# Zoe187419/ATE_replication_causalML

Measured on AMD Instinct MI355X. Metric: rows/sec for DML-ATE cross-fit, N=1e7 p=500, 1/2/4/8 MI355X; ATE/SE parity, higher is better.
Workload: dtype bf16; 1 GPU; model=DML-PLR 5-fold cross-fit, CV-LASSO nuisances (100 lambdas, inner 4-fold CV), global_batch=10000000, seq_len=500, N=10000000, p=500, folds=5, parallelism=dp1, dgp=tutorial, n_kept=10000000, layout=blocked64+bytes8

## Files before the change

ate_replication_causalml_amd/_native.py:

```python
from __future__ import annotations

import ctypes
import os
from pathlib import Path

_LIBDIR = Path(__file__).resolve().parent / "_lib"
_hip = None
_cpu = None


class NativeMissing(RuntimeError):
    pass


class NativeError(RuntimeError):

    def __init__(self, name: str, status: int, detail: str):
        self.entry, self.status = name, status
        super().__init__(f"{name} failed with status {status}: {detail}")


HIP_ERRORS = {
    1: "hipErrorInvalidValue", 2: "hipErrorOutOfMemory", 3: "hipErrorNotInitialized",
    4: "hipErrorDeinitialized", 9: "hipErrorInvalidConfiguration",
    13: "hipErrorInvalidSymbol", 17: "hipErrorInvalidDevicePointer",
    21: "hipErrorInvalidMemcpyDirection", 35: "hipErrorInsufficientDriver",
    52: "hipErrorMissingConfiguration", 53: "hipErrorPriorLaunchFailure",
    98: "hipErrorInvalidDeviceFunction", 100: "hipErrorNoDevice", 101: "hipErrorInvalidDevice",
    200: "hipErrorInvalidImage", 201: "hipErrorInvalidContext", 209: "hipErrorNoBinaryForGpu",
    218: "hipErrorInvalidKernelFile", 400: "hipErrorInvalidHandle", 500: "hipErrorNotFound",
    600: "hipErrorNotReady", 700: "hipErrorIllegalAddress", 701: "hipErrorLaunchOutOfResources",
    702: "hipErrorLaunchTimeOut", 710: "hipErrorAssert", 719: "hipErrorLaunchFailure",
    720: "hipErrorCooperativeLaunchTooLarge", 801: "hipErrorNotSupported",
    900: "hipErrorStreamCaptureUnsupported", 901: "hipErrorStreamCaptureInvalidated",
    907: "hipErrorCapturedEvent", 999: "hipErrorUnknown",
}


def describe_status(rc: int) -> str:
    if rc < 0:
        return "rejected by the entry point's own argument check (no kernel launched)"
    return f"{HIP_ERRORS.get(rc, 'hipError?')} ({rc})"


c_void_p = ctypes.c_void_p
c_int = ctypes.c_int
c_int64 = ctypes.c_int64
c_uint64 = ctypes.c_uint64
c_double = ctypes.c_double

_SIGS = {
    "ate_gram_bf16": "pliipipipipppp",
    "ate_gram_bf16_pair": "pllipippipippippiip",
    "ate_gram_bf16_tri": "pllippipippipp",
    "ate_gram_pair_bal": "",
    "ate_last_error": "pi",
    "ate_last_stale_error": "pi",
    "ate_clear_errors": "",
    "ate_debug_bad_launch": "ip",
    "ate_check_kernel_resources": "pi",
    "ate_gram_f32": "plippipipippppp",
    "ate_gram_f64": "plippipipippppp",
    "ate_gram_tile_sizes": "pppp",
    "ate_chol_solve": "pipiipdpppppp",
    "ate_chol_solve_k": "pipipidppppp",
    "ate_spd_solve_batched": "ppiippp",
    "ate_predict": "ipllppiidipp",
    "ate_irls_update": "ipllppiiiiippppipp",
    "ate_irls_check": "piidippp",
    "ate_naive": "ippplpppp",
    "ate_clip_propensity": "pplpp",
    "ate_aipw": "ppppppldpppp",
    "ate_dml_moments": "ppplppp",
    "ate_dml_finalize": "pipp",
    "ate_boot_multinomial": "ppluiipp",
    "ate_boot_poisson": "ppluiilipp",
    "ate_enet_isa_selftest": "pp",
    "ate_enet_prepare": "piipipiipipipppppppp",
    "ate_enet_path": "pipiippppidddipppppippp",
    "ate_enet_coef": "ppiiiipppppppp",
    "ate_enet_cvloss_gauss": "pippiipppiiipp",
    "ate_cv_select": "pppiipippppip",
    "ate_enet_pick": "ppiiipppip",
    "ate_dml_resid_moments": "ipllpipipiiiiiippp",
    "ate_dml_resid_exact": "pllpipipiiiiiiippp",
    "ate_irm_score_moments": "ipllpipiipiiiiidippp",
    "ate_irm_score_moments_multi": "ipllpipiipipiiiiiidippp",
    "ate_irm_score_multi_smax": "",
    "ate_irm_scores": "ipllpipiipiiiiidipp",
    "ate_irm_sens_moments": "ipllpipiipiiiiidippp",
    "ate_irm_target_moments": "ipllpipiipiiiiidippp",
    "ate_iivm_moments": "ipllpipiipiiiiiiidippp",
    "ate_group_boot": "pppliiuippp",
    "ate_group_boot_scratch": "iii",
    "ate_cate_moments": "ppplpiiippp",
    "ate_cate_moments_scratch": "iii",
    "ate_cate_boot": "ppplppiiiuippp",
    "ate_cate_boot_scratch": "iiii",
    "ate_policy_pair_hist": "ppppppliiipp",
    "ate_policy_pair_hist_scratch": "i",
    "ate_policy_search": "ppiilppp",
    "ate_lognet_path": "iplpiipipipdddippippppppppp",
    "ate_lognet_cvloss": "iplpiippipppipp",
    "ate_dgp_fill": "iplllllp" + "uiipppp",
    "ate_sel_block_rows": "",
    "ate_sel_gen_count": "upilllpp",
    "ate_sel_gen_flags": "upillpp",
    "ate_sel_gen_mark": "upiplllpiplp",
    "ate_forest_fit": "pppppi" + "pppppppp" + "ip",
    "ate_forest_predict": "ppiiipppppippip",
    "ate_forest_pack": "pippppppp",
    "ate_forest_scratch_bytes": "ii",
    "ate_forest_exact_scratch_bytes": "iiii",
    "ate_forest_fit_exact": "piiipppippppippppppppp",
    "ate_forest_predict16": "ppiiipppppppippip",
    "ate_bin_matrix": "plipppp",
    "ate_panel_xtv": "iplpipplipp",
    "ate_select_compact": "plppddpppp" + "p",
    "ate_gbdt_run": "ppp",
    "ate_lv_boot": "ppp",
    "ate_lv_classify": "pipiippp",
    "ate_lv_decide": "ppipipipippppp" + "iipip",
    "ate_lv_partition": "ppipippppipp",
    "ate_lv_scatter": "pppppippp",
    "ate_lv_children": "pippppp",
    "ate_lv_transpose": "piipip",
    "ate_gbdt_bin_panel": "pilpipppilpppl" + "p",
    "ate_gbdt_slab_entries": "liii",
    "ate_gbdt_slab2_entries": "li",
    "ate_gbdt_pair_root": "pppplllp",
    "ate_gbdt_apply": "plliipppp" + "p",
    "ate_panel_xv": "iplpipiplpp",
    "ate_col_moments": "pllipppp",
    "ate_standardize": "pllippp",
    "ate_interactions": "pllipl" + "p",
    "ate_scan_parts": "l",
    "ate_gbdt_limits": "p",
    "ate_excl_scan_i32": "plpppp",
    "ate_excl_scan_i64": "plpppp",
}
_RESTYPE = {"ate_forest_scratch_bytes": ctypes.c_int64,
            "ate_forest_exact_scratch_bytes": ctypes.c_int64, "ate_gbdt_slab_entries": ctypes.c_int64,
            "ate_gbdt_slab2_entries": ctypes.c_int64,
            "ate_scan_parts": ctypes.c_int64, "ate_group_boot_scratch": ctypes.c_int64,
            "ate_cate_moments_scratch": ctypes.c_int64,
            "ate_cate_boot_scratch": ctypes.c_int64,
            "ate_policy_pair_hist_scratch": ctypes.c_int64}
_CT = {"p": c_void_p, "i": c_int, "l": c_int64, "u": c_uint64, "d": c_double}


def _load(path: Path, sigs: dict):
    lib = ctypes.CDLL(str(path), mode=ctypes.RTLD_GLOBAL)
    for name, sig in sigs.items():
        if hasattr(lib, name):
            f = getattr(lib, name)
            f.restype = _RESTYPE.get(name, c_int)
            f.argtypes = [_CT[ch] for ch in sig]
    return lib


def hip_available() -> bool:
    return (_LIBDIR / "libatehip.so").exists()


def hip_library_path() -> Path:
    debug = os.environ.get("ATE_DEBUG", "0") not in ("", "0")
    return Path(os.environ["ATE_HIP_LIB"]) if os.environ.get("ATE_HIP_LIB") else \
        _LIBDIR / ("libatehip_debug.so" if debug else "libatehip.so")


def hip():
    global _hip
    if _hip is None:
        import torch
        debug = os.environ.get("ATE_DEBUG", "0") not in ("", "0")
        p = hip_library_path()
        if not p.exists():
            raise NativeMissing(
                f"{p} not found: build it with `python -m ate_replication_causalml_amd._build` "
                "(hipcc --offload-arch=gfx950). GPU ops have no fallback.")
        _hip = _load(p, _SIGS)
        if debug:
            _check_kernel_resources(_hip)
    return _hip


_resource_report = None


def _check_kernel_resources(lib):
    global _resource_report
    buf = ctypes.create_string_buffer(1 << 14)
    bad = lib.ate_check_kernel_resources(buf, len(buf))
    _resource_report = buf.value.decode(errors="replace")
    if bad > 0:
        raise NativeError("ate_check_kernel_resources", bad,
                          "kernels that cannot launch as registered:\n" + "\n".join(
                              l for l in _resource_report.splitlines() if "FAIL" in l))


def kernel_resource_report() -> str | None:
    return _resource_report


def _native_message(lib, fn: str) -> tuple[int, str]:
    buf = ctypes.create_string_buffer(512)
    code = getattr(lib, fn)(buf, len(buf))
    return code, buf.value.decode(errors="replace")


def cpu():
    global _cpu
    if _cpu is None:
        p = _LIBDIR / "libatecpu.so"
        if not p.exists():
            from ._build import build_cpu
            build_cpu()
        _cpu = _load(p, {})
    return _cpu


def check(rc: int, name: str = "native call"):
    if rc != 0:
        raise RuntimeError(f"{name} failed with code {rc}")


def call(name: str, *args):
    lib = hip()
    rc = getattr(lib, name)(*args)
    if rc != 0:
        raise NativeError(name, rc, status_detail(lib, rc))
    return rc


def status_detail(lib, rc: int) -> str:
    detail = describe_status(rc)
    if rc > 0 and hasattr(lib, "ate_last_error"):
        code, msg = _native_message(lib, "ate_last_error")
        if code == rc and msg:
            detail = msg
        scode, smsg = _native_message(lib, "ate_last_stale_error")
        if scode and smsg:
            detail += f" [stale, cleared before the launch: {smsg}]"
        lib.ate_clear_errors()
    return detail


def loaded_libraries():
    out = []
    try:
        with open(f"/proc/{os.getpid()}/maps") as f:
            for line in f:
                if str(_LIBDIR) in line:
                    out.append(line.split()[-1])
    except OSError:
        pass
    return sorted(set(out))
```

ate_replication_causalml_amd/estimators/lasso.py:

```python
from __future__ import annotations

import numpy as np
import torch

from .. import _native
from ..ops import stats as S
from ..ops.devconst import const
from ..ops.enet import cv_enet_gaussian
from ..ops.gram import gram
from ..ops.linalg import chol_solve, chol_solve_active
from ..ops.panel import build_panel, dtype_code
from ..parallel import rng
from ..reference.estimators import lambda_interp
from ..result import AteResult
from ..utils.graphs import estimator_graphs
from .common import as_np, read_result, resolve_device


def _fold_ids(n, K, seed, stream, dist):
    return dist.fold_ids(K, seed, stream) if dist is not None else rng.fold_ids(n, K, seed, stream)


def _sharded_gram(pan, dist):
    G = gram(pan)
    if dist is None:
        return G, None
    dist.sum_(G)
    return G, global_seg_counts(pan, dist.comm)


def _lasso_w_panel(Y, W, X, seed, nfolds, fold_stream, device, dtype, dist=None):
    dev = resolve_device(device)
    Xn = np.column_stack([as_np(X), as_np(W)])
    fid = _fold_ids(Xn.shape[0], nfolds, seed, fold_stream, dist)
    return build_panel(Xn, None, as_np(Y), folds=fid, dtype=dtype, device=dev)


def _lasso_w_cv(pan, pf_w, G, counts=None):
    pf = np.r_[np.ones(len(pan.xcols) - 1), pf_w]
    return cv_enet_gaussian(G, pan, pan.xcols, [pan.cols["Y"]], penalty_factor=pf,
                            seg_counts=counts)


def _lasso_w_body(pan, pf_w, dist=None, counts=None):
    G = gram(pan)
    if dist is not None:
        dist.sum_(G)
    cv = _lasso_w_cv(pan, pf_w, G, None if counts is None else np.asarray(counts))
    lam = cv.lambdas[0].gather(0, cv.sel[0, 1:2].long())
    fnp = cv.fold_npass.min().double().reshape(1) if cv.fold_npass is not None else \
        torch.zeros(1, dtype=torch.float64, device=lam.device)
    return torch.cat([cv.coef_1se[0, -1:].double(), lam.double(), fnp])


def _lasso_w(Y, W, X, pf_w, seed, nfolds, fold_stream, method, device, dtype, dist, graph):
    pan = _lasso_w_panel(Y, W, X, seed, nfolds, fold_stream, device, dtype, dist)
    if graph and (dist is None or dist.capturable) and pan.data.is_cuda:
        counts = None if dist is None else tuple(global_seg_counts(pan, dist.comm).tolist())
        out, g = estimator_graphs.run("lasso_w", _lasso_w_body, (pan,), float(pf_w), dist,
                                      counts)
        v = out.cpu().numpy()
        if v[2] < 0:
            from ..utils.guards import NumericalError
            raise NumericalError("CV fold path timed out waiting for its full-data lambda "
                                 "sequence; selection is invalid")
        return AteResult.make(method, float(v[0]), None, lambda_1se=float(v[1]), hipgraph=g)
    G, counts = _sharded_gram(pan, dist)
    cv = _lasso_w_cv(pan, pf_w, G, counts).check()
    return AteResult.make(method, float(cv.coef_1se[0, -1]), None,
                          lambda_1se=float(cv.lambdas[0, int(cv.sel[0, 1])]))


def lasso_single(Y, W, X, seed=1991, nfolds=10, fold_stream=5, method="Single-equation LASSO",
                 device=None, dtype="f64", dist=None, graph=True):
    return _lasso_w(Y, W, X, 0.0, seed, nfolds, fold_stream, method, device, dtype, dist, graph)


def lasso_usual(Y, W, X, seed=1991, nfolds=10, fold_stream=6, method="Usual LASSO", device=None,
                dtype="f64", dist=None, graph=True):
    return _lasso_w(Y, W, X, 1.0, seed, nfolds, fold_stream, method, device, dtype, dist, graph)


def interaction_expand(x: torch.Tensor) -> torch.Tensor:
    from ..ops.prep import interactions
    return interactions(x)


def _interp_at(lams: torch.Tensor, nlam: torch.Tensor, path: torch.Tensor, s: torch.Tensor):
    L = lams.numel()
    k = nlam.long().clamp(min=1)
    ar = torch.arange(L, device=lams.device)
    valid = ar < k
    lam0 = lams[0]
    lamk = lams.gather(0, (k - 1).reshape(1))[0]
    den = lam0 - lamk
    single = den == 0
    dsafe = torch.where(single, torch.ones_like(den), den)
    sfrac = ((lam0 - s) / dsafe).clamp(0.0, 1.0)
    ln = torch.where(valid, (lam0 - lams) / dsafe, torch.full_like(lams, 2.0))
    left = ((ln <= sfrac) & valid).sum().clamp(min=1) - 1
    ln_l = ln.gather(0, left.reshape(1))[0]
    exact = (ln_l == sfrac) | single | (left + 1 >= k)
    right = torch.where(exact, left, left + 1)
    ln_r = ln.gather(0, right.reshape(1))[0]
    gap = ln_l - ln_r
    frac = torch.where(exact | (gap.abs() < np.finfo(float).eps), torch.ones_like(sfrac),
                       (sfrac - ln_r) / torch.where(gap == 0, torch.ones_like(gap), gap))
    return (path.index_select(0, left.reshape(1))[0] * frac
            + path.index_select(0, right.reshape(1))[0] * (1 - frac))


def _belloni_body(panw, pany, panpost, compat):
    cws = cv_enet_gaussian(gram(panw), panw, panw.xcols, [panw.cols["Y"]])
    cys = cv_enet_gaussian(gram(pany), pany, pany.xcols, [pany.cols["Y"]])
    q = len(panw.xcols)
    s = cws.lambdas[0].gather(0, cws.sel[0, 0:1].long())[0]
    bw = _interp_at(cws.lambdas[0], cws.nlam[0], cws.coef_path[0].double(), s)[1:]
    if compat == "reference":
        by = _interp_at(cys.lambdas[0], cys.nlam[0], cys.coef_path[0].double(), s)[1:]
        pos = (bw > 0) | (by > 0)
        keep = torch.cat([pos[1:], torch.zeros(1, dtype=torch.bool, device=pos.device)])
    else:
        sy = cys.lambdas[0].gather(0, cys.sel[0, 0:1].long())[0]
        by = _interp_at(cys.lambdas[0], cys.nlam[0], cys.coef_path[0].double(), sy)[1:]
        keep = (bw != 0) | (by != 0)
    G = gram(panpost)[0]
    dev = G.device
    xc = const(panpost.xcols[:q], torch.int32, dev)
    ki = keep.long()
    nsel = ki.sum()
    pos = torch.where(keep, ki.cumsum(0), 1 + nsel + (1 - ki).cumsum(0))
    wpos = (1 + nsel).reshape(1)
    dest = torch.cat([const([0], torch.int64, dev), pos, wpos])
    src = torch.cat([const([panpost.cols["one"]], torch.int32, dev), xc,
                     const([panpost.xcols[q]], torch.int32, dev)])
    cols = torch.empty(q + 2, dtype=torch.int32, device=dev).index_copy(0, dest, src)
    kact = (2 + nsel).to(torch.int32)
    r = chol_solve_active(G, cols, kact, panpost.cols["Y"])
    b_w = r.beta.gather(0, wpos)[0]
    se = torch.sqrt(r.aux[1] / (panpost.n - r.aux[0]) * r.invdiag.gather(0, wpos)[0])
    fnp = torch.stack([cws.fold_npass.min(), cys.fold_npass.min()]).min().double() \
        if cws.fold_npass is not None else torch.zeros((), dtype=torch.float64, device=dev)
    return torch.stack([b_w.double(), se.double(), nsel.double(), r.aux[0].double(), fnp])


def belloni(Y, W, X, seed=1991, nfolds=10, compat="reference", method="Belloni et.al",
            device=None, dtype="f64", dist=None, graph=True):
    dev = resolve_device(device)
    Yn, Wn = as_np(Y), as_np(W)
    xint = interaction_expand(torch.as_tensor(as_np(X), device=dev))
    n, q = xint.shape
    if graph and dist is None and dev.type == "cuda":
        panw = build_panel(xint, None, Wn, folds=_fold_ids(n, nfolds, seed, 8, None), dtype=dtype,
                           device=dev)
        pany = build_panel(xint, None, Yn, folds=_fold_ids(n, nfolds, seed, 9, None), dtype=dtype,
                           device=dev)
        post = torch.cat([xint, torch.as_tensor(Wn, dtype=torch.float64, device=dev)[:, None]], 1)
        panpost = build_panel(post, None, Yn, dtype=dtype, device=dev)
        out, g = estimator_graphs.run("belloni", _belloni_body, (panw, pany, panpost), compat)
        v = out.cpu().numpy()
        if v[4] < 0:
            from ..utils.guards import NumericalError
            raise NumericalError("CV fold path timed out waiting for its full-data lambda "
                                 "sequence; selection is invalid")
        return AteResult.make(method, float(v[0]), float(v[1]), n_selected=int(round(v[2])),
                              rank=int(round(v[3])), hipgraph=g)
    fits = []
    for target, stream in ((Wn, 8), (Yn, 9)):
        fid = _fold_ids(n, nfolds, seed, stream, dist)
        pan = build_panel(xint, None, target, folds=fid, dtype=dtype, device=dev)
        G, counts = _sharded_gram(pan, dist)
        fits.append((pan, G, cv_enet_gaussian(G, pan, pan.xcols, [pan.cols["Y"]],
                                              seg_counts=counts).check()))
    (_, _, cw), (_, _, cy) = fits
    s = float(cw.lambdas[0, int(cw.sel[0, 0])])
    lw = cw.lambdas[0, :int(cw.nlam[0])].cpu().numpy()
    ly = cy.lambdas[0, :int(cy.nlam[0])].cpu().numpy()
    pw = cw.coef_path[0, :len(lw)].cpu().numpy()
    py = cy.coef_path[0, :len(ly)].cpu().numpy()

    def coef_at(lams, path, s_):
        l, r, f = lambda_interp(lams, s_)
        return path[l] * f + path[r] * (1 - f)

    bw = coef_at(lw, pw, s)[1:]
    by = coef_at(ly, py, s if compat == "reference" else float(cy.lambdas[0, int(cy.sel[0, 0])]))[1:]
    if compat == "reference":
        union = []
        for v in np.concatenate([np.flatnonzero(bw > 0) + 1, np.flatnonzero(by > 0) + 1]):
            if int(v) not in union:
                union.append(int(v))
        cols = [v - 2 for v in union if v - 1 >= 1]
    else:
        cols = sorted(set(np.flatnonzero(bw != 0)) | set(np.flatnonzero(by != 0)))
    sel_x = torch.cat([xint[:, torch.as_tensor(cols, dtype=torch.long, device=xint.device)],
                       torch.as_tensor(Wn, dtype=torch.float64, device=xint.device)[:, None]], 1)
    pan = build_panel(sel_x, None, Yn, dtype=dtype, device=dev)
    G = gram(pan)[0]
    if dist is not None:
        dist.sum_(G)
    dcols = [pan.cols["one"], *pan.xcols]
    r = chol_solve(G, dcols, pan.cols["Y"])
    n_all = dist.n_total if dist is not None else pan.n
    se = torch.sqrt(r.aux[1] / (n_all - r.aux[0]) * r.invdiag[-1])
    return read_result(torch.stack([r.beta[-1], se]), method, n_selected=len(cols),
                       rank=int(r.aux[0]))


def global_seg_counts(pan, comm):
    c = torch.as_tensor(np.asarray(pan.seg_nreal, dtype=np.float64))
    if comm is not None and comm.world_size > 1:
        dev = pan.device
        t = c.to(dev)
        comm.all_reduce_(t)
        c = t.cpu()
    return c.numpy()


EXACT_BLOCK = 16384


def dml_residual_terms(pan, coef: torch.Tensor, rows: int = 1 << 20) -> torch.Tensor:
    K = coef.shape[0]
    Xc = pan.colmajor()
    dev = Xc.device
    bf = pan.dtype == torch.bfloat16
    xc = torch.as_tensor(pan.xcols, dtype=torch.long, device=dev)
    out = []
    for k in range(K):
        r0, r1 = (int(v) for v in pan.seg_bounds[k])
        for a in range(r0, r1, rows):
            b = min(r1, a + rows)
            blk = Xc[:, a:b]
            valid = (blk[pan.cols["one"]] != 0).double()
            xs = blk.index_select(0, xc).double()
            y = blk[pan.cols["Y_hi"]].double() + blk[pan.cols["Y_lo"]].double() if bf else \
                blk[pan.cols["Y"]].double()
            w = blk[pan.cols["W_hi"]].double() + blk[pan.cols["W_lo"]].double() if bf else \
                blk[pan.cols["W"]].double()
            yr = y - (coef[k, 0, 0] + coef[k, 0, 1:].double() @ xs)
            wr = w - (coef[k, 1, 0] + coef[k, 1, 1:].double() @ xs)
            yr, wr = yr * valid, wr * valid
            w2 = wr * wr
            out.append(torch.stack([wr * yr, w2, yr * yr * w2, yr * w2 * wr, w2 * w2,
                                    valid, yr * yr], 1))
    return torch.cat(out)


_TRI: dict = {}


def _tri_index(P: int, device):
    key = (P, str(device))
    t = _TRI.get(key)
    if t is None:
        i, j = np.triu_indices(P)
        t = (torch.as_tensor(i * P + j, dtype=torch.int64).to(device),
             torch.as_tensor(j * P + i, dtype=torch.int64).to(device))
        _TRI[key] = t
    return t


def allreduce_sym_(comm, t: torch.Tensor) -> torch.Tensor:
    P = t.shape[-1]
    up, lo = _tri_index(P, t.device)
    v = t.view(-1, P * P)
    buf = v.index_select(1, up)
    comm.all_reduce_(buf)
    v.index_copy_(1, up, buf)
    v.index_copy_(1, lo, buf)
    return t


def dml_phases(pan, folds: int, lambda_rule="min", comm=None, seg_counts=None, G=None,
               shard_paths=True, exact=False):
    from ..utils.graphs import Collective
    dist = comm is not None and comm.world_size > 1
    if dist and seg_counts is None:
        seg_counts = global_seg_counts(pan, comm)
    K = folds
    full_sets = [[s for s in range(K) if s != k] for k in range(K)]
    ycols = [pan.cols["Y"], pan.cols["W"]]
    sharded = dist and shard_paths
    mine = [k for k in range(K) if k % comm.world_size == comm.rank] if sharded else list(range(K))
    p1 = len(pan.xcols) + 1

    n_rows = int(np.asarray(seg_counts if seg_counts is not None else pan.seg_nreal).sum())
    if exact:
        from ..ops.gram import check_exact_range
        check_exact_range(pan, n_rows, comm=comm if dist else None)

    def phase_gram(_):
        if exact:
            return {"GX": gram(pan, stage="tiles", exact=True, n_total=n_rows, checked=True)}
        return {"G": gram(pan, stage="tiles") if G is None else G}

    def phase_gram_reduce(st):
        if exact:
            return {"GX": gram(pan, stage="reduce", exact=True)}
        return st if G is not None else {"G": gram(pan, stage="reduce", out=st["G"])}

    def phase_from_limbs(st):
        from ..ops.exact import from_limbs
        return {**st, "G": from_limbs(st["GX"])}

    native_exact = pan.data.is_cuda and pan.dtype == torch.bfloat16

    def phase_terms(st):
        from ..ops.exact import column_amax
        if native_exact:
            part = _exact_resid(pan, st["coef"], 1, None)
            return {**st, "amax": part.view(-1, 7).amax(0)}
        terms = dml_residual_terms(pan, st["coef"])
        return {**st, "terms": terms, "amax": column_amax(terms)}

    def phase_limbs(st):
        from ..ops.exact import _scale_exp, sum_limbs
        if native_exact:
            sh = _scale_exp(st["amax"], n_rows).contiguous()
            part = _exact_resid(pan, st["coef"], 2, sh).view(torch.int64).view(-1, 14).sum(0)
            return {**st, "limbs": torch.stack([part[:7], part[7:]])}
        return {**st, "limbs": sum_limbs(st["terms"], st["amax"], n_rows)}

    def phase_mom_exact(st):
        from ..ops.exact import finish_limbs
        return {**st, "mom": finish_limbs(st["limbs"], st["amax"], n_rows)}

    def fit(st):
        if not mine:
            return None
        cv = cv_enet_gaussian(st["G"], pan, pan.xcols, ycols,
                              full_sets=[full_sets[k] for k in mine], seg_counts=seg_counts)
        return cv

    def pick(cv):
        return (cv.coef_min if lambda_rule == "min" else cv.coef_1se).reshape(
            len(mine), 2, -1).contiguous()

    def phase_fit(st):
        cv = fit(st)
        coef = pick(cv)
        return {**st, "cv": cv, "mom": dml_residual_moments(pan, coef)}

    def phase_fit_sharded(st):
        cv = fit(st)
        coef = torch.zeros((K, 2, p1), dtype=torch.float64, device=pan.device)
        if cv is not None:
            coef.index_copy_(0, const(mine, torch.int64, pan.device), pick(cv).double())
        return {**st, "cv": cv, "coef": coef}

    def phase_resid(st):
        return {**st, "mom": dml_residual_moments(pan, st["coef"])}

    def phase_final(st):
        return {**st, "res": S.dml_finalize(st["mom"], "plr")}

    cap = bool(getattr(comm, "capturable", False))

    def reduce(name, op="sum"):
        def f(st):
            (comm.all_reduce_ if op == "sum" else comm.all_reduce_max_)(st[name])
            return st
        return Collective(f, capturable=cap)

    def reduce_sym(name):
        _tri_index(pan.P, pan.device)

        def f(st):
            allreduce_sym_(comm, st[name])
            return st
        return Collective(f, capturable=cap)

    if exact:
        phases = [phase_gram, phase_gram_reduce]
        if dist:
            phases.append(reduce("GX"))
        phases.append(phase_from_limbs)
        if sharded:
            phases += [phase_fit_sharded, reduce("coef")]
        else:
            def phase_fit_coef(st):
                cv = fit(st)
                return {**st, "cv": cv, "coef": pick(cv).double()}
            phases.append(phase_fit_coef)
        phases.append(phase_terms)
        if dist:
            phases.append(reduce("amax", "max"))
        phases.append(phase_limbs)
        if dist:
            phases.append(reduce("limbs"))
        phases += [phase_mom_exact, phase_final]
        return phases
    phases = [phase_gram, phase_gram_reduce]
    if dist:
        phases.append(reduce_sym("G"))
    if sharded:
        phases += [phase_fit_sharded, reduce("coef"), phase_resid]
    else:
        phases.append(phase_fit)
    if dist:
        phases.append(reduce("mom"))
    phases.append(phase_final)
    return phases


def dml_crossfit_panel(pan, folds: int, lambda_rule="min", G=None, comm=None, seg_counts=None,
                       exact=False):
    st = None
    for ph in dml_phases(pan, folds, lambda_rule, comm, seg_counts, G, exact=exact):
        st = ph(st)
    return st["res"], st["mom"], st.get("cv")


def micro_fold_map(K: int, s: int) -> np.ndarray:
    a, b = np.divmod(np.arange(K * K), K)
    return (a + s * b) % K


def median_aggregate(theta: torch.Tensor, se: torch.Tensor, how: str = "median"):
    def med(v):
        v = torch.sort(v).values
        n = v.shape[0]
        return v[n // 2] if n % 2 else 0.5 * (v[n // 2 - 1] + v[n // 2])
    if how == "mean":
        t = theta.mean()
        return torch.stack([t, torch.sqrt((se * se + (theta - t) ** 2).mean())])
    t = med(theta)
    return torch.stack([t, torch.sqrt(med(se * se + (theta - t) ** 2))])


def dml_repeated_phases(pan, folds: int, repeats: int, lambda_rule="min", comm=None,
                        seg_counts=None, aggregate="median"):
    from ..utils.graphs import Collective
    K, Sn = folds, repeats
    if pan.nseg != K * K:
        raise ValueError(f"repeated cross-fitting needs K*K = {K * K} micro-segments, the panel "
                         f"has {pan.nseg}")
    if not 1 <= Sn <= K:
        raise ValueError(f"repeats must be in 1..{K} (distinct partitions of K*K micro-segments)")
    dist = comm is not None and comm.world_size > 1
    if seg_counts is None:
        seg_counts = global_seg_counts(pan, comm) if dist else np.asarray(pan.seg_nreal)
    counts = np.asarray(seg_counts, dtype=np.float64)
    dev = pan.device
    maps = [micro_fold_map(K, s) for s in range(Sn)]
    M = [const(np.eye(K)[m].T.copy(), torch.float64, dev) for m in maps]
    fold_counts = [np.bincount(m, weights=counts, minlength=K) for m in maps]
    mi = [const(m, torch.int64, dev) for m in maps]
    full_sets = [[j for j in range(K) if j != k] for k in range(K)]
    ycols = [pan.cols["Y"], pan.cols["W"]]
    P = pan.P
    cap = bool(getattr(comm, "capturable", False))

    def phase_gram(_):
        return {"G": gram(pan, stage="tiles")}

    def phase_gram_reduce(st):
        return {"G": gram(pan, stage="reduce", out=st["G"])}

    Mall = torch.cat(M)
    sets_all = [[s * K + j for j in fs] for s in range(Sn) for fs in full_sets]
    counts_all = np.concatenate(fold_counts)

    def phase_paths(st):
        Gs = (Mall @ st["G"].view(K * K, P * P)).view(Sn * K, P, P)
        cv = cv_enet_gaussian(Gs, pan, pan.xcols, ycols, full_sets=sets_all,
                              seg_counts=counts_all)
        coef = (cv.coef_min if lambda_rule == "min" else cv.coef_1se).reshape(Sn, K, 2, -1)
        return {**st, "coef": coef}

    def phase_split(s):
        def f(st):
            coef_m = st["coef"][s].double().index_select(0, mi[s]).contiguous()
            return {**st, f"mom{s}": dml_residual_moments(pan, coef_m)}
        return f

    def phase_final(st):
        res = torch.stack([S.dml_finalize(st[f"mom{s}"], "plr") for s in range(Sn)])
        return {**st, "splits": res, "res": median_aggregate(res[:, 0], res[:, 1], aggregate)}

    def reduce(name):
        def f(st):
            comm.all_reduce_(st[name])
            return st
        return Collective(f, capturable=cap)

    def reduce_sym(name):
        _tri_index(P, dev)

        def f(st):
            allreduce_sym_(comm, st[name])
            return st
        return Collective(f, capturable=cap)

    phases = [phase_gram, phase_gram_reduce]
    if dist:
        phases.append(reduce_sym("G"))
    phases.append(phase_paths)
    for s in range(Sn):
        phases.append(phase_split(s))
        if dist:
            phases.append(reduce(f"mom{s}"))
    phases.append(phase_final)
    return phases


def dml_repeated_panel(pan, folds: int, repeats: int, lambda_rule="min", comm=None,
                       seg_counts=None, aggregate="median"):
    st = None
    for ph in dml_repeated_phases(pan, folds, repeats, lambda_rule, comm, seg_counts, aggregate):
        st = ph(st)
    return st["res"], st["splits"]


def _exact_resid(pan, coef: torch.Tensor, mode: int, sh) -> torch.Tensor:
    K = coef.shape[0]
    dev = pan.device
    xc = const(pan.xcols, torch.int32, dev)
    segs = const(np.asarray(pan.seg_bounds[:K], dtype=np.int64), torch.int64, dev)
    nbx = 512
    part = torch.empty(K * nbx * (7 if mode == 1 else 14), dtype=torch.float64, device=dev)
    cs, bs = pan.strides()
    c = coef.double().contiguous()
    _native.call("ate_dml_resid_exact", pan.data.data_ptr(), cs, bs, xc.data_ptr(), len(pan.xcols),
                 segs.data_ptr(), K, c.data_ptr(), pan.cols["Y_hi"], pan.cols["Y_lo"],
                 pan.cols["W_hi"], pan.cols["W_lo"], pan.cols["one"], nbx, mode,
                 None if sh is None else sh.data_ptr(), part.data_ptr(),
                 torch.cuda.current_stream().cuda_stream)
    return part


def dml_residual_moments(pan, coef: torch.Tensor) -> torch.Tensor:
    K = coef.shape[0]
    p = len(pan.xcols)
    if not pan.data.is_cuda:
        X = pan.colmajor().double()
        moms = torch.zeros(7, dtype=torch.float64)
        for k in range(K):
            r0, r1 = pan.seg_bounds[k]
            Xs = X[:, r0:r1]
            v = Xs[pan.cols["one"]] != 0
            xs = Xs[pan.xcols]
            yv, wv = Xs[pan.cols["Y"]], Xs[pan.cols["W"]]
            yr = yv - (coef[k, 0, 0] + coef[k, 0, 1:] @ xs)
            wr = wv - (coef[k, 1, 0] + coef[k, 1, 1:] @ xs)
            moms += S.dml_moments(yr[v], wr[v])
        return moms
    dev = pan.device
    xc = const(pan.xcols, torch.int32, dev)
    segs = const(np.asarray(pan.seg_bounds[:K], dtype=np.int64), torch.int64, dev)
    bf = pan.dtype == torch.bfloat16
    nbx = 512 if bf else 256
    part = torch.empty(K * nbx * 7, dtype=torch.float64, device=dev)
    mom = torch.empty(7, dtype=torch.float64, device=dev)
    bf = pan.dtype == torch.bfloat16
    y0, y1 = (pan.cols["Y_hi"], pan.cols["Y_lo"]) if bf else (pan.cols["Y"], -1)
    w0, w1 = (pan.cols["W_hi"], pan.cols["W_lo"]) if bf else (pan.cols["W"], -1)
    cs, bs = pan.strides()
    _native.call("ate_dml_resid_moments", dtype_code(pan.data), pan.data.data_ptr(), cs, bs,
                 xc.data_ptr(), p, segs.data_ptr(), K, coef.data_ptr(), y0, y1, w0, w1,
                 pan.cols["one"], nbx, part.data_ptr(), mom.data_ptr(),
                 torch.cuda.current_stream().cuda_stream)
    return mom


def _dml_body(pan, folds, lambda_rule, dist=None, counts=None):
    comm = dist.comm if dist is not None else None
    return dml_crossfit_panel(pan, folds, lambda_rule, comm=comm,
                              seg_counts=None if counts is None else np.asarray(counts))[0]


def _dml_graphed(pan, folds, lambda_rule, dist=None):
    counts = None
    if dist is not None and dist.world > 1:
        counts = tuple(global_seg_counts(pan, dist.comm).tolist())
    return estimator_graphs.run("dml_plr", _dml_body, (pan,), folds, lambda_rule, dist, counts)


def _dml_repeated_body(pan, folds, repeats, lambda_rule, aggregate):
    st = None
    for ph in dml_repeated_phases(pan, folds, repeats, lambda_rule, aggregate=aggregate):
        st = ph(st)
    return torch.cat([st["res"], st["splits"].reshape(-1)])


def dml_plr_lasso_repeated(Y, W, X, folds=5, repeats=3, seed=1991, lambda_rule="min",
                           aggregate="median", method="DML cross-fit (LASSO, repeated)",
                           device=None, dtype="f64", graph=True):
    dev = resolve_device(device)
    Yn, Wn, Xn = as_np(Y), as_np(W), as_np(X)
    micro = rng.fold_ids(len(Yn), folds * folds, seed, 0)
    pan = build_panel(Xn, Wn, Yn, folds=micro, dtype=dtype, device=dev)
    if graph and pan.data.is_cuda:
        out, g = estimator_graphs.run("dml_repeated", _dml_repeated_body, (pan,), folds, repeats,
                                      lambda_rule, aggregate)
    else:
        out, g = _dml_repeated_body(pan, folds, repeats, lambda_rule, aggregate), False
    v = out.detach().double().cpu().numpy()
    return AteResult.make(method, v[0], v[1], n=len(Yn), repeats=repeats, aggregate=aggregate,
                          splits=v[2:].reshape(repeats, 2).tolist(), hipgraph=g)


def dml_plr_lasso(Y, W, X, folds=5, seed=1991, lambda_rule="min", method="DML cross-fit (LASSO)",
                  device=None, dtype="f64", dist=None, graph=True):
    dev = resolve_device(device)
    Yn, Wn, Xn = as_np(Y), as_np(W), as_np(X)
    fid = _fold_ids(len(Yn), folds, seed, 0, dist)
    pan = build_panel(Xn, Wn, Yn, folds=fid, dtype=dtype, device=dev)
    if graph and (dist is None or dist.capturable) and pan.data.is_cuda:
        res, g = _dml_graphed(pan, folds, lambda_rule, dist)
        return read_result(res, method, n=dist.n_total if dist is not None else len(Yn),
                           hipgraph=g)
    res, mom, _ = dml_crossfit_panel(pan, folds, lambda_rule,
                                     comm=dist.comm if dist is not None else None)
    return read_result(res, method, n=dist.n_total if dist is not None else len(Yn))
```

ate_replication_causalml_amd/ops/enet.py:

```python
from __future__ import annotations

from dataclasses import dataclass

import numpy as np
import torch

from .. import _native
from ..reference import glmnet as ref
from .devconst import const, const_bytes


def _stream():
    return torch.cuda.current_stream().cuda_stream


@dataclass
class EnetCvResult:
    lambdas: torch.Tensor
    nlam: torch.Tensor
    cvm: torch.Tensor
    cvsd: torch.Tensor
    sel: torch.Tensor
    coef_path: torch.Tensor
    coef_min: torch.Tensor
    coef_1se: torch.Tensor
    full_keys: list
    npass: torch.Tensor
    fold_npass: torch.Tensor | None = None
    fold_nlam: torch.Tensor | None = None

    def check(self):
        bad = [] if self.fold_npass is None else \
            np.flatnonzero(self.fold_npass.cpu().numpy() < 0).tolist()
        if bad:
            from ..utils.guards import NumericalError
            raise NumericalError(f"CV fold path(s) {bad} timed out waiting for their "
                                 "full-data lambda sequence; selection is invalid")
        return self


def poison_if_truncated(fold_npass: torch.Tensor, *ts):
    bad = (fold_npass < 0).any()
    nan = torch.full((), float("nan"), dtype=torch.float64, device=fold_npass.device)
    return [torch.where(bad, nan, t) for t in ts]


def _zeroed(dev, *specs):
    sizes = [int(np.prod(sh)) * torch.empty((), dtype=dt).element_size() for sh, dt in specs]
    offs = np.concatenate([[0], np.cumsum([(b + 255) // 256 * 256 for b in sizes])])
    buf = torch.zeros(int(offs[-1]), dtype=torch.uint8, device=dev)
    return [buf[int(o):int(o) + b].view(dt).view(sh)
            for (sh, dt), o, b in zip(specs, offs[:-1], sizes)]


def _rescale_vp(vp, p):
    vp = np.ones(p) if vp is None else np.maximum(np.asarray(vp, float), 0)
    return vp * p / vp.sum()


def _cv_tables(nseg, full_sets, ycols, nreal, nlambda, full_y):
    ny = len(ycols)
    if full_sets is None:
        full_sets = [list(range(nseg))]
    tsets, tindex = [], {}

    def tid(segs):
        key = tuple(sorted(segs))
        if key not in tindex:
            tindex[key] = len(tsets)
            tsets.append(key)
        return tindex[key]

    full_t = [tid(fs) for fs in full_sets]
    fold_t, fold_hold = [], []
    for fs in full_sets:
        for s in fs:
            fold_t.append(tid([q for q in fs if q != s]))
            fold_hold.append(s)
    K = len(full_sets[0])
    assert all(len(fs) == K for fs in full_sets), "full sets must have equal fold counts"
    masks = np.zeros((len(tsets), nseg), dtype=np.uint8)
    for i, ts in enumerate(tsets):
        masks[i, list(ts)] = 1
    if full_y is None:
        ys_of = [list(range(ny))] * len(full_sets)
    else:
        if len(full_y) != len(full_sets) or any(not 0 <= int(y) < ny for y in full_y):
            raise ValueError("full_y needs one index into ycols per full set")
        ys_of = [[int(y)] for y in full_y]
    full_keys = [(f, y) for f in range(len(full_sets)) for y in ys_of[f]]
    full_probs = [(full_t[f], y, -1, nlambda) for f, y in full_keys]
    src_of = {key: i for i, key in enumerate(full_keys)}
    fold_probs, fold_ycol, fold_holds = [], [], []
    fold_index = np.zeros((len(full_probs), K), dtype=np.int32)
    nfold = np.zeros((len(full_probs), K))
    for f in range(len(full_sets)):
        for k in range(K):
            for y in ys_of[f]:
                src = src_of[(f, y)]
                fold_index[src, k] = len(fold_probs)
                nfold[src, k] = nreal[fold_hold[f * K + k]]
                fold_probs.append((fold_t[f * K + k], y, src, 0))
                fold_ycol.append(ycols[y])
                fold_holds.append(fold_hold[f * K + k])
    perm = np.argsort([fp[0] for fp in fold_probs], kind="stable")
    inv = np.empty_like(perm)
    inv[perm] = np.arange(len(perm))
    fold_probs = [fold_probs[i] for i in perm]
    fold_ycol = [fold_ycol[i] for i in perm]
    fold_holds = [fold_holds[i] for i in perm]
    fold_index = inv[fold_index].astype(np.int32)
    return (full_sets, masks, full_keys, full_probs, fold_probs, fold_ycol, fold_holds,
            fold_index, nfold)


def cv_problem_count(nseg, full_sets=None, ny=1, full_y=None) -> int:
    t = _cv_tables(nseg, full_sets, list(range(ny)), np.ones(nseg), 1, full_y)
    return len(t[3]) + len(t[4])


MAX_PATH_PROBLEMS = 256


def default_lambda_min_ratio(n_train_min, p) -> float:
    return 1e-4 if n_train_min > p else 1e-2


def cv_enet_gaussian(G: torch.Tensor, panel, xcols, ycols, full_sets=None, penalty_factor=None,
                     alpha=1.0, nlambda=100, lambda_min_ratio=None, thresh=1e-7,
                     maxit=100000, seg_counts=None, full_y=None) -> EnetCvResult:
    nseg = G.shape[0]
    P = G.shape[1]
    p = len(xcols)
    ny = len(ycols)
    nreal = np.asarray(panel.seg_nreal if seg_counts is None else seg_counts, dtype=np.float64)
    (full_sets, masks, full_keys, full_probs, fold_probs, fold_ycol, fold_holds, fold_index,
     nfold) = _cv_tables(nseg, full_sets, ycols, nreal, nlambda, full_y)
    n_full = [nreal[list(fs)].sum() for fs in full_sets]
    if lambda_min_ratio is None:
        lambda_min_ratio = default_lambda_min_ratio(min(n_full), p)
    vp = _rescale_vp(penalty_factor, p)
    L = nlambda
    if G.is_cuda:
        return _cv_gpu(G, P, nseg, masks, xcols, ycols, p, ny, vp, panel.cols["one"], full_probs,
                       fold_probs, fold_ycol, fold_holds, fold_index, nfold, alpha,
                       lambda_min_ratio, thresh, maxit, L, full_keys, panel.dtype)
    return _cv_cpu(G, masks, xcols, ycols, p, ny, vp, panel.cols["one"], full_probs, fold_probs,
                   fold_ycol, fold_holds, fold_index, nfold, alpha, lambda_min_ratio, thresh, maxit,
                   L, full_keys)


_PROB_DT = np.dtype([("train", "<i4"), ("y", "<i4"), ("src", "<i4"), ("nlam", "<i4")])


def _probs_tensor(probs, dev):
    return const_bytes(np.array(probs, dtype=_PROB_DT), dev)


def _cv_gpu(G, P, nseg, masks, xcols, ycols, p, ny, vp, one, full_probs, fold_probs, fold_ycol,
            fold_holds, fold_index, nfold, alpha, flmin, thresh, maxit, L, full_keys,
            panel_dtype):
    dev = G.device
    s = _stream()
    f64 = dict(dtype=torch.float64, device=dev)
    nt = masks.shape[0]
    masks_t = const(masks, torch.uint8, dev)
    xc = const(xcols, torch.int32, dev)
    yc = const(ycols, torch.int32, dev)
    c_f32 = int(panel_dtype != torch.float64)
    ldc = (p + 63) // 64 * 64
    nf = len(full_probs)
    probs_all = list(full_probs) + list(fold_probs)
    nq = len(probs_all)
    i32 = torch.int32
    C, apath, rsq, nlam, npass, progress = _zeroed(
        dev, ((nt, p, ldc), torch.float32 if c_f32 else torch.float64), ((nq, L, p), torch.float64),
        ((nq, L), torch.float64), ((nq,), i32), ((nq,), i32), ((nq,), i32))
    g = torch.empty((nt, ny, p), **f64)
    xm = torch.empty((nt, p), **f64)
    xs = torch.empty((nt, p), **f64)
    ju = torch.empty((nt, p), dtype=torch.uint8, device=dev)
    ym = torch.empty((nt, ny), **f64)
    ys = torch.empty((nt, ny), **f64)
    nobs = torch.empty(nt, **f64)
    _native.call("ate_enet_prepare", G.data_ptr(), nseg, P, masks_t.data_ptr(), nt, xc.data_ptr(),
                 p, one, yc.data_ptr(), ny, C.data_ptr(), c_f32, g.data_ptr(), xm.data_ptr(),
                 xs.data_ptr(), ju.data_ptr(), ym.data_ptr(), ys.data_ptr(), nobs.data_ptr(), s)
    vp_t = const(np.asarray(vp, dtype=np.float64), torch.float64, dev)
    pr = _probs_tensor(probs_all, dev)
    lams = torch.full((nq, L), float("nan"), **f64)
    lampub = torch.empty((nq, L), **f64)
    _native.call("ate_enet_path", C.data_ptr(), c_f32, g.data_ptr(), p, ny, ju.data_ptr(),
                 ys.data_ptr(), vp_t.data_ptr(), pr.data_ptr(), nq, alpha, flmin, thresh,
                 maxit, apath.data_ptr(), lams.data_ptr(), rsq.data_ptr(), nlam.data_ptr(),
                 npass.data_ptr(), L, progress.data_ptr(), lampub.data_ptr(), s)
    coef = torch.empty((nq, L, p + 1), **f64)
    _native.call("ate_enet_coef", apath.data_ptr(), pr.data_ptr(), nq, p, ny, L,
                 nlam.data_ptr(), xm.data_ptr(), xs.data_ptr(), ju.data_ptr(), ym.data_ptr(),
                 ys.data_ptr(), coef.data_ptr(), s)
    hold = const([0] * nf + list(fold_holds), torch.int32, dev)
    ycol_p = const([0] * nf + list(fold_ycol), torch.int32, dev)
    cvraw = torch.empty((nq, L), **f64)
    _native.call("ate_enet_cvloss_gauss", G.data_ptr(), P, hold.data_ptr(), xc.data_ptr(), p, one,
                 ycol_p.data_ptr(), coef.data_ptr(), nlam.data_ptr(), L, nf, nq - nf,
                 cvraw.data_ptr(), s)
    fidx = const(fold_index + nf, torch.int32, dev)
    nfold_t = const(nfold, torch.float64, dev)
    cvm = torch.empty((nf, L), **f64)
    cvsd = torch.empty((nf, L), **f64)
    sel = torch.empty((nf, 2), dtype=torch.int32, device=dev)
    K = fold_index.shape[1]
    fold_npass = npass[nf:]
    _native.call("ate_cv_select", cvraw.data_ptr(), fidx.data_ptr(), nfold_t.data_ptr(), K, nf,
                 nlam.data_ptr(), L, cvm.data_ptr(), cvsd.data_ptr(), sel.data_ptr(),
                 fold_npass.data_ptr(), nq - nf, s)
    cmin = torch.empty((nf, p + 1), **f64)
    c1se = torch.empty((nf, p + 1), **f64)
    _native.call("ate_enet_pick", coef.data_ptr(), sel.data_ptr(), p, L, nf, cmin.data_ptr(),
                 c1se.data_ptr(), fold_npass.data_ptr(), nq - nf, s)
    return EnetCvResult(lams[:nf], nlam[:nf], cvm, cvsd, sel, coef[:nf], cmin, c1se, full_keys,
                        npass[:nf], fold_npass, nlam[nf:])


def _cv_cpu(G, masks, xcols, ycols, p, ny, vp, one, full_probs, fold_probs, fold_ycol, fold_holds,
            fold_index, nfold, alpha, flmin, thresh, maxit, L, full_keys):
    Gn = G.double().cpu().numpy()
    nt = masks.shape[0]
    stats = []
    for t in range(nt):
        Gt = np.tensordot(masks[t].astype(float), Gn, axes=1)
        n = Gt[one, one]
        sx = Gt[one, xcols] / n
        vx = np.diag(Gt)[xcols] / n - sx * sx
        ju = vx > 0
        xs = np.where(ju, np.sqrt(np.maximum(vx, 0)), 1.0)
        Cm = (Gt[np.ix_(xcols, xcols)] / n - np.outer(sx, sx)) / np.outer(xs, xs)
        Cm[~ju, :] = 0
        Cm[:, ~ju] = 0
        Cm[np.flatnonzero(~ju), np.flatnonzero(~ju)] = 1.0
        gs, ymv, ysv = [], [], []
        for yc in ycols:
            my = Gt[one, yc] / n
            vy = Gt[yc, yc] / n - my * my
            sy = np.sqrt(vy) if vy > 0 else 1.0
            gj = np.where(ju, (Gt[xcols, yc] / n - sx * my) / (xs * sy), 0.0)
            gs.append(gj)
            ymv.append(my)
            ysv.append(sy)
        stats.append(dict(C=Cm, g=gs, xm=sx, xs=xs, ju=ju, ym=ymv, ys=ysv, n=n))

    def run(probs, src_paths):
        res = []
        for (t, y, src, nlam_req) in probs:
            st = stats[t]
            lam = None if src < 0 else src_paths[src].lambdas
            path = ref._elnet_core(st["C"], st["g"][y], np.ones(p), st["xm"], st["xs"], st["ym"][y],
                                   st["ys"][y], st["ju"], alpha, vp, lam, nlam_req or L, flmin,
                                   thresh, maxit)
            res.append(path)
        return res

    full = run(full_probs, None)
    folds = run(fold_probs, full)
    nf = len(full_probs)
    K = fold_index.shape[1]
    lams = np.full((nf, L), np.nan)
    nlam = np.zeros(nf, dtype=np.int32)
    coef = np.full((nf, L, p + 1), np.nan)
    for f, path in enumerate(full):
        m = len(path.lambdas)
        lams[f, :m] = path.lambdas
        nlam[f] = m
        coef[f, :m, 0] = path.a0
        coef[f, :m, 1:] = path.beta
    cvraw = np.full((len(fold_probs), L), np.nan)
    for q, path in enumerate(folds):
        Gh = Gn[fold_holds[q]]
        yc = fold_ycol[q]
        n = Gh[one, one]
        for m in range(len(path.lambdas)):
            a0, b = path.a0[m], path.beta[m]
            Gxx = Gh[np.ix_(xcols, xcols)]
            sse = (Gh[yc, yc] - 2 * a0 * Gh[one, yc] - 2 * b @ Gh[xcols, yc] + n * a0 * a0
                   + 2 * a0 * b @ Gh[xcols, one] + b @ Gxx @ b)
            cvraw[q, m] = sse / n
    cvm = np.full((nf, L), np.nan)
    cvsd = np.full((nf, L), np.nan)
    sel = np.zeros((nf, 2), dtype=np.int32)
    for f in range(nf):
        m = nlam[f]
        raw = cvraw[fold_index[f]][:, :m]
        cm, cs, i0, i1 = ref.cv_select(lams[f, :m], raw, nfold[f])
        cvm[f, :m], cvsd[f, :m] = cm, cs
        sel[f] = (i0, i1)
    cmin = np.stack([coef[f, sel[f, 0]] for f in range(nf)])
    c1se = np.stack([coef[f, sel[f, 1]] for f in range(nf)])
    t = torch.from_numpy
    return EnetCvResult(t(lams), t(nlam), t(cvm), t(cvsd), t(sel), t(coef), t(cmin), t(c1se),
                        full_keys, t(np.array([pth.npasses for pth in full])),
                        fold_nlam=t(np.array([len(pth.lambdas) for pth in folds], dtype=np.int32)))
```

csrc/common.hpp:

```cpp
#pragma once
#include <hip/hip_runtime.h>
#include <stdint.h>
#include <stdio.h>

#include <vector>

#define ATE_API extern "C" __attribute__((visibility("default")))

namespace ate {

constexpr int WAVE = 64;

typedef __attribute__((ext_vector_type(8))) __bf16 bf16x8;
typedef __attribute__((ext_vector_type(4))) float f32x4;
typedef __attribute__((ext_vector_type(16))) float f32x16;
typedef unsigned short bf16_t;

__device__ __forceinline__ float bf16_to_f32(bf16_t h) {
  return __uint_as_float(((uint32_t)h) << 16);
}
__host__ __device__ inline bf16_t f32_to_bf16_rne(float f) {
#ifdef __HIP_DEVICE_COMPILE__
  uint32_t u = __float_as_uint(f);
#else
  uint32_t u; __builtin_memcpy(&u, &f, 4);
#endif
  u += 0x7FFFu + ((u >> 16) & 1u);
  return (bf16_t)(u >> 16);
}

struct u32x4 { uint32_t x, y, z, w; };

__host__ __device__ inline u32x4 philox4x32(uint32_t c0, uint32_t c1, uint32_t c2, uint32_t c3,
                                            uint32_t k0, uint32_t k1) {
  for (int r = 0; r < 10; ++r) {
    uint64_t p0 = (uint64_t)0xD2511F53u * c0;
    uint64_t p1 = (uint64_t)0xCD9E8D57u * c2;
    uint32_t hi0 = (uint32_t)(p0 >> 32), lo0 = (uint32_t)p0;
    uint32_t hi1 = (uint32_t)(p1 >> 32), lo1 = (uint32_t)p1;
    uint32_t n0 = hi1 ^ c1 ^ k0;
    uint32_t n2 = hi0 ^ c3 ^ k1;
    c0 = n0; c1 = lo1; c2 = n2; c3 = lo0;
    k0 += 0x9E3779B9u; k1 += 0xBB67AE85u;
  }
  return {c0, c1, c2, c3};
}

enum : uint32_t { P_FOLD = 1, P_BOOT = 2, P_RF_BOOT = 3, P_RF_MTRY = 4, P_DGP = 5,
                  P_SUBSAMPLE = 6, P_GBDT = 7, P_SAMPLE_ROWS = 8, P_MULT = 9 };

__host__ __device__ inline u32x4 rand4(uint64_t seed, uint32_t purpose, uint32_t stream,
                                       uint64_t index) {
  return philox4x32((uint32_t)index, (uint32_t)(index >> 32), purpose, stream,
                    (uint32_t)seed, (uint32_t)(seed >> 32));
}
__host__ __device__ inline uint32_t rand_below(uint64_t seed, uint32_t purpose, uint32_t stream,
                                               uint64_t index, uint32_t n) {
  u32x4 r = rand4(seed, purpose, stream, index);
  return (uint32_t)(((uint64_t)r.x * (uint64_t)n) >> 32);
}
__host__ __device__ inline float rand_uniform(uint64_t seed, uint32_t purpose, uint32_t stream,
                                              uint64_t index) {
  u32x4 r = rand4(seed, purpose, stream, index);
  return (float)(r.x >> 8) * (1.0f / 16777216.0f);
}

template <typename T>
__device__ __forceinline__ T wave_sum(T v) {
#pragma unroll
  for (int o = 32; o > 0; o >>= 1) v += __shfl_xor(v, o, 64);
  return v;
}
template <typename T>
__device__ __forceinline__ T wave_max(T v) {
#pragma unroll
  for (int o = 32; o > 0; o >>= 1) { T u = __shfl_xor(v, o, 64); v = v > u ? v : u; }
  return v;
}

template <int NV>
__device__ inline void block_sum(double (&v)[NV], double* smem ) {
  const int lane = threadIdx.x & 63, wid = threadIdx.x >> 6, nw = blockDim.x >> 6;
#pragma unroll
  for (int k = 0; k < NV; ++k) v[k] = wave_sum(v[k]);
  if (lane == 0)
#pragma unroll
    for (int k = 0; k < NV; ++k) smem[wid * NV + k] = v[k];
  __syncthreads();
  if (threadIdx.x == 0) {
#pragma unroll
    for (int k = 0; k < NV; ++k) {
      double s = 0.0;
      for (int w = 0; w < nw; ++w) s += smem[w * NV + k];
      v[k] = s;
    }
  }
  __syncthreads();
}

inline int grid_for(int64_t n, int block, int cap = 2048) {
  int64_t g = (n + block - 1) / block;
  if (g < 1) g = 1;
  return (int)(g > cap ? cap : g);
}

}

#ifdef ATE_DEVICE_ASSERT
#define ATE_DASSERT(cond)                                                          \
  do {                                                                             \
    if (!(cond)) {                                                                 \
      printf("ATE_DASSERT failed %s:%d: %s\n", __FILE__, __LINE__, #cond);         \
      __builtin_trap();                                                            \
    }                                                                              \
  } while (0)
#else
#define ATE_DASSERT(cond) do { } while (0)
#endif

namespace ate {
struct LaunchError {
  int code = 0;
  bool pending = false;
  char msg[512] = {0};
};
inline thread_local LaunchError g_launch_error, g_stale_error;

inline void record_error(LaunchError& slot, hipError_t e, const char* what, const char* func,
                         const char* file, int line) {
  slot.code = (int)e;
  snprintf(slot.msg, sizeof(slot.msg), "%s (%d): %s; %s in %s at %s:%d", hipGetErrorName(e),
           (int)e, hipGetErrorString(e), what, func, file, line);
}
inline void launch_pre(const char* func, const char* file, int line) {
  const hipError_t e = hipGetLastError();
  if (e != hipSuccess)
    record_error(g_stale_error, e, "pending before a launch (an earlier HIP call's)", func,
                 file, line);
}
inline void launch_post(const char* func, const char* file, int line) {
  const hipError_t e = hipGetLastError();
  if (e != hipSuccess && !g_launch_error.pending) {
    record_error(g_launch_error, e, "kernel launch failed", func, file, line);
    g_launch_error.pending = true;
  }
}
inline int take_launch_error() {
  if (!g_launch_error.pending) return 0;
  g_launch_error.pending = false;
  return g_launch_error.code;
}
}

namespace ate {
struct KernelShape {
  const void* fn;
  const char* name;
  int threads, dyn_lds;
};
inline std::vector<KernelShape>& kernel_shapes() {
  static std::vector<KernelShape> v;
  return v;
}
struct KernelShapeReg {
  KernelShapeReg(const void* f, const char* n, int t, int d) { kernel_shapes().push_back({f, n, t, d}); }
};
}
#define ATE_CAT2(a, b) a##b
#define ATE_CAT(a, b) ATE_CAT2(a, b)
#define ATE_KERNEL_SHAPE(name, threads, dyn_lds, ...)                                   \
  static ate::KernelShapeReg ATE_CAT(ate_kshape_, __LINE__)((const void*)(__VA_ARGS__), \
                                                              name, threads, dyn_lds);

#define ATE_LAUNCH(...)                                   \
  do {                                                    \
    ate::launch_pre(__func__, __FILE__, __LINE__);        \
    hipLaunchKernelGGL(__VA_ARGS__);                      \
    ate::launch_post(__func__, __FILE__, __LINE__);       \
  } while (0)

#define ATE_CHECK_LAUNCH()                                \
  do {                                                    \
    const int e_ = ate::take_launch_error();              \
    if (e_ != 0) return e_;                               \
  } while (0)
```

csrc/dml.hip:

```cpp
#include "common.hpp"

using namespace ate;

template <typename T>
__device__ __forceinline__ double ld_col(const T* X, int64_t ld, int c, int64_t i) {
  return (double)X[(int64_t)c * ld + i];
}
template <>
__device__ __forceinline__ double ld_col<bf16_t>(const bf16_t* X, int64_t ld, int c, int64_t i) {
  return (double)bf16_to_f32(X[(int64_t)c * ld + i]);
}

struct Seg { int64_t r0, r1; };

template <typename C>
__device__ int compact_support(C* cy, C* cw, int* xc, int p, int* wcnt ) {
  const int lane = threadIdx.x & 63, wid = threadIdx.x >> 6, nw = blockDim.x >> 6;
  int base = 0;
  for (int j0 = 0; j0 < p; j0 += blockDim.x) {
    const int j = j0 + threadIdx.x;
    const bool keep = j < p && (cy[1 + j] != C(0) || cw[1 + j] != C(0));
    C vy = j < p ? cy[1 + j] : C(0), vw = j < p ? cw[1 + j] : C(0);
    const int c = j < p ? xc[j] : 0;
    const uint64_t m = __ballot(keep);
    if (lane == 0) wcnt[wid] = __popcll(m);
    __syncthreads();
    int off = base;
    for (int w = 0; w < wid; ++w) off += wcnt[w];
    int tot = base;
    for (int w = 0; w < nw; ++w) tot += wcnt[w];
    const int pos = off + __popcll(m & ((1ull << lane) - 1ull));
    __syncthreads();
    if (keep) { cy[1 + pos] = vy; cw[1 + pos] = vw; xc[pos] = c; }
    __syncthreads();
    base = tot;
  }
  return base;
}

template <typename T, int RPT>
__global__ __launch_bounds__(256) void dml_resid_kernel(
    const T* __restrict__ X, int64_t ld, const int* __restrict__ xcols, int p,
    const Seg* __restrict__ segs, int nseg, const double* __restrict__ coef ,
    int y0, int y1, int w0, int w1, int vcol, double* __restrict__ partial) {
  extern __shared__ __attribute__((aligned(16))) double sh[];
  double* cy = sh;
  double* cw = sh + (p + 1);
  int* xc = (int*)(sh + 2 * (p + 1));
  __shared__ double red[16 * 7];
  __shared__ int wcnt[16];
  double v[7] = {0, 0, 0, 0, 0, 0, 0};
  for (int j = threadIdx.x; j < p; j += blockDim.x) xc[j] = xcols[j];
  const int k = blockIdx.y;
  ATE_DASSERT(k < nseg && y0 >= 0 && w0 >= 0 && vcol >= 0);
  for (int j = threadIdx.x; j <= p; j += blockDim.x) {
    cy[j] = coef[((int64_t)k * 2 + 0) * (p + 1) + j];
    cw[j] = coef[((int64_t)k * 2 + 1) * (p + 1) + j];
  }
  __syncthreads();
  p = compact_support(cy, cw, xc, p, wcnt);
  const Seg sg = segs[k];
  ATE_DASSERT(sg.r0 >= 0 && sg.r0 <= sg.r1 && sg.r1 <= ld);
  for (int64_t base = sg.r0 + (int64_t)blockIdx.x * 256 * RPT; base < sg.r1;
       base += (int64_t)gridDim.x * 256 * RPT) {
    double py[RPT], pw[RPT];
    int64_t ii[RPT];
#pragma unroll
    for (int r = 0; r < RPT; ++r) {
      ii[r] = base + r * 256 + threadIdx.x;
      py[r] = cy[0];
      pw[r] = cw[0];
    }
    for (int j = 0; j < p; ++j) {
      const double by = cy[1 + j], bw = cw[1 + j];
      const int c = xc[j];
#pragma unroll
      for (int r = 0; r < RPT; ++r) {
        double x = ii[r] < sg.r1 ? ld_col(X, ld, c, ii[r]) : 0.0;
        py[r] += by * x;
        pw[r] += bw * x;
      }
    }
#pragma unroll
    for (int r = 0; r < RPT; ++r) {
      if (ii[r] >= sg.r1) continue;
      if (ld_col(X, ld, vcol, ii[r]) == 0.0) continue;
      double y = ld_col(X, ld, y0, ii[r]) + (y1 >= 0 ? ld_col(X, ld, y1, ii[r]) : 0.0);
      double w = ld_col(X, ld, w0, ii[r]) + (w1 >= 0 ? ld_col(X, ld, w1, ii[r]) : 0.0);
      double yr = y - py[r], wr = w - pw[r], w2 = wr * wr;
      v[0] += wr * yr; v[1] += w2; v[2] += yr * yr * w2; v[3] += yr * w2 * wr; v[4] += w2 * w2;
      v[5] += 1.0; v[6] += yr * yr;
    }
  }
  block_sum<7>(v, red);
  if (threadIdx.x == 0) {
    double* out = partial + ((int64_t)blockIdx.y * gridDim.x + blockIdx.x) * 7;
#pragma unroll
    for (int q = 0; q < 7; ++q) out[q] = v[q];
  }
}

__global__ __launch_bounds__(256) void sum7_kernel(const double* __restrict__ partial, int nb,
                                                   double* __restrict__ out) {
  __shared__ double red[16 * 7];
  double v[7] = {0, 0, 0, 0, 0, 0, 0};
  for (int b = threadIdx.x; b < nb; b += 256)
#pragma unroll
    for (int q = 0; q < 7; ++q) v[q] += partial[(int64_t)b * 7 + q];
  block_sum<7>(v, red);
  if (threadIdx.x == 0)
#pragma unroll
    for (int q = 0; q < 7; ++q) out[q] = v[q];
}

template <typename T>
static int dml_resid_t(const void* X, int64_t ld, const void* xcols, int p, const void* segs,
                       int nseg, const void* coef, int y0, int y1, int w0, int w1, int vcol,
                       int nbx, void* partial, void* moments, hipStream_t s) {
  size_t sh = (size_t)2 * (p + 1) * sizeof(double) + (size_t)p * sizeof(int);
  dim3 grid(nbx, nseg);
  ATE_LAUNCH((dml_resid_kernel<T, 4>), grid, dim3(256), sh, s, (const T*)X, ld,
                     (const int*)xcols, p, (const Seg*)segs, nseg, (const double*)coef, y0, y1,
                     w0, w1, vcol, (double*)partial);
  ATE_CHECK_LAUNCH();
  ATE_LAUNCH(sum7_kernel, dim3(1), dim3(256), 0, s, (const double*)partial, nbx * nseg,
                     (double*)moments);
  ATE_CHECK_LAUNCH();
  return 0;
}

__global__ __launch_bounds__(256) void dml_resid_bf16_kernel(
    const bf16_t* __restrict__ X, int64_t cs, int64_t bs, const int* __restrict__ xcols, int p,
    const Seg* __restrict__ segs, int nseg, const double* __restrict__ coef,
    int y0, int y1, int w0, int w1, int vcol, double* __restrict__ partial, int mode,
    const int64_t* __restrict__ sh) {
  extern __shared__ __attribute__((aligned(16))) float shf[];
  float* cy = shf;
  float* cw = shf + (p + 1);
  int* xc = (int*)(shf + 2 * (p + 1));
  __shared__ double red[16 * 7];
  __shared__ int wcnt[16];
  const int k = blockIdx.y;
  for (int j = threadIdx.x; j < p; j += blockDim.x) xc[j] = xcols[j];
  for (int j = threadIdx.x; j <= p; j += blockDim.x) {
    cy[j] = (float)coef[((int64_t)k * 2 + 0) * (p + 1) + j];
    cw[j] = (float)coef[((int64_t)k * 2 + 1) * (p + 1) + j];
  }
  __syncthreads();
  p = compact_support(cy, cw, xc, p, wcnt);
  double v[7] = {0, 0, 0, 0, 0, 0, 0};
  long long lh[7] = {0, 0, 0, 0, 0, 0, 0}, ll[7] = {0, 0, 0, 0, 0, 0, 0};
  double scale[7];
#pragma unroll
  for (int q = 0; q < 7; ++q) scale[q] = mode == 2 ? ldexp(1.0, (int)sh[q]) : 1.0;
  const Seg sg = segs[k];
  ATE_DASSERT(k < nseg && sg.r0 >= 0 && sg.r0 <= sg.r1 && (sg.r0 & 7) == 0 && mode >= 0 &&
              mode <= 2 && y0 >= 0 && w0 >= 0 && vcol >= 0);
  auto ld8 = [&](int c, int64_t i, float (&o)[8]) {
    ATE_DASSERT((i & 7) == 0 && c >= 0);
    const uint4 u = *reinterpret_cast<const uint4*>(X + (int64_t)c * cs + (i >> 6) * bs + (i & 63));
    const uint32_t w[4] = {u.x, u.y, u.z, u.w};
#pragma unroll
    for (int q = 0; q < 4; ++q) {
      o[2 * q] = __uint_as_float(w[q] << 16);
      o[2 * q + 1] = __uint_as_float(w[q] & 0xFFFF0000u);
    }
  };
  for (int64_t i = sg.r0 + ((int64_t)blockIdx.x * 256 + threadIdx.x) * 8; i < sg.r1;
       i += (int64_t)gridDim.x * 256 * 8) {
    float py[8], pw[8];
#pragma unroll
    for (int r = 0; r < 8; ++r) { py[r] = cy[0]; pw[r] = cw[0]; }
#pragma unroll 4
    for (int j = 0; j < p; ++j) {
      float x[8];
      ld8(xc[j], i, x);
      const float by = cy[1 + j], bw = cw[1 + j];
#pragma unroll
      for (int r = 0; r < 8; ++r) { py[r] += by * x[r]; pw[r] += bw * x[r]; }
    }
    float vv[8], ya[8], yb[8], wa[8], wb[8];
    ld8(vcol, i, vv);
    ld8(y0, i, ya);
    ld8(w0, i, wa);
    if (y1 >= 0) ld8(y1, i, yb); else { for (int r = 0; r < 8; ++r) yb[r] = 0.f; }
    if (w1 >= 0) ld8(w1, i, wb); else { for (int r = 0; r < 8; ++r) wb[r] = 0.f; }
#pragma unroll
    for (int r = 0; r < 8; ++r) {
      if (vv[r] == 0.f) continue;
      const double yr = ((double)ya[r] + (double)yb[r]) - (double)py[r];
      const double wr = ((double)wa[r] + (double)wb[r]) - (double)pw[r];
      const double w2 = wr * wr;
      if (mode == 0) {
        v[0] += wr * yr; v[1] += w2; v[2] += yr * yr * w2; v[3] += yr * w2 * wr; v[4] += w2 * w2;
        v[5] += 1.0; v[6] += yr * yr;
        continue;
      }
      const double t[7] = {wr * yr, w2, yr * yr * w2, yr * w2 * wr, w2 * w2, 1.0, yr * yr};
#pragma unroll
      for (int q = 0; q < 7; ++q) {
        if (mode == 1) {
          v[q] = fmax(v[q], fabs(t[q]));
        } else {
          const double x = t[q] * scale[q];
          const double h = floor(x);
          lh[q] += (long long)h;
          ll[q] += (long long)rint((x - h) * 4294967296.0);
        }
      }
    }
  }
  const int64_t blk = (int64_t)blockIdx.y * gridDim.x + blockIdx.x;
  if (mode == 0) {
    block_sum<7>(v, red);
    if (threadIdx.x == 0) {
      double* out = partial + blk * 7;
#pragma unroll
      for (int q = 0; q < 7; ++q) out[q] = v[q];
    }
    return;
  }
  __shared__ long long xr[4][14];
  const int lane = threadIdx.x & 63, wid = threadIdx.x >> 6;
#pragma unroll
  for (int q = 0; q < 7; ++q) {
    for (int o = 32; o > 0; o >>= 1) {
      if (mode == 1) {
        v[q] = fmax(v[q], __shfl_xor(v[q], o, 64));
      } else {
        lh[q] += __shfl_xor(lh[q], o, 64);
        ll[q] += __shfl_xor(ll[q], o, 64);
      }
    }
  }
  if (lane == 0) {
#pragma unroll
    for (int q = 0; q < 7; ++q) {
      xr[wid][q] = mode == 1 ? __double_as_longlong(v[q]) : lh[q];
      xr[wid][7 + q] = ll[q];
    }
  }
  __syncthreads();
  if (threadIdx.x < 14) {
    const int q = threadIdx.x;
    if (mode == 1) {
      if (q < 7) {
        double m = 0.0;
        for (int w = 0; w < 4; ++w) m = fmax(m, __longlong_as_double(xr[w][q]));
        partial[blk * 7 + q] = m;
      }
    } else {
      long long a = 0;
      for (int w = 0; w < 4; ++w) a += xr[w][q];
      reinterpret_cast<long long*>(partial)[blk * 14 + q] = a;
    }
  }
}

ATE_API int ate_dml_resid_moments(int dtype, const void* X, int64_t cs, int64_t bs,
                                  const void* xcols, int p,
                                  const void* segs, int nseg, const void* coef, int y0, int y1,
                                  int w0, int w1, int vcol, int nbx, void* partial, void* moments,
                                  void* stream) {
  hipStream_t s = (hipStream_t)stream;
  if (dtype != 3 && bs != 64) return -1;
  const int64_t ld = cs;
  if (dtype == 1)
    return dml_resid_t<float>(X, ld, xcols, p, segs, nseg, coef, y0, y1, w0, w1, vcol, nbx,
                              partial, moments, s);
  if (dtype == 2)
    return dml_resid_t<double>(X, ld, xcols, p, segs, nseg, coef, y0, y1, w0, w1, vcol, nbx,
                               partial, moments, s);
  if (dtype == 3) {
    size_t sh = (size_t)2 * (p + 1) * sizeof(float) + (size_t)p * sizeof(int);
    dim3 grid(nbx, nseg);
    ATE_LAUNCH(dml_resid_bf16_kernel, grid, dim3(256), sh, s, (const bf16_t*)X, cs, bs,
                       (const int*)xcols, p, (const Seg*)segs, nseg, (const double*)coef, y0, y1,
                       w0, w1, vcol, (double*)partial, 0, (const int64_t*)nullptr);
    ATE_CHECK_LAUNCH();
    ATE_LAUNCH(sum7_kernel, dim3(1), dim3(256), 0, s, (const double*)partial, nbx * nseg,
                       (double*)moments);
    ATE_CHECK_LAUNCH();
    return 0;
  }
  return -1;
}

ATE_API int ate_dml_resid_exact(const void* X, int64_t cs, int64_t bs, const void* xcols, int p,
                                const void* segs, int nseg, const void* coef, int y0, int y1,
                                int w0, int w1, int vcol, int nbx, int mode, const void* sh,
                                void* partial, void* stream) {
  if (mode < 1 || mode > 2) return -1;
  size_t shm = (size_t)2 * (p + 1) * sizeof(float) + (size_t)p * sizeof(int);
  dim3 grid(nbx, nseg);
  ATE_LAUNCH(dml_resid_bf16_kernel, grid, dim3(256), shm, (hipStream_t)stream,
                     (const bf16_t*)X, cs, bs, (const int*)xcols, p, (const Seg*)segs, nseg,
                     (const double*)coef, y0, y1, w0, w1, vcol, (double*)partial, mode,
                     (const int64_t*)sh);
  ATE_CHECK_LAUNCH();
  return 0;
}
```

csrc/enet.hip:

```cpp
#include <cstdlib>

#include <utility>

#include "common.hpp"

#include <type_traits>

using namespace ate;

__device__ __forceinline__ double seg_sum(const double* __restrict__ G, int nseg, int P,
                                          const unsigned char* __restrict__ mk, int a, int b) {
  double acc = 0.0;
  for (int q = 0; q < nseg; ++q)
    if (mk[q]) acc += G[((int64_t)q * P + a) * P + b];
  return acc;
}

__global__ __launch_bounds__(256) void enet_prep_stats_kernel(
    const double* __restrict__ G, int nseg, int P, const unsigned char* __restrict__ masks,
    const int* __restrict__ xcols, int p, int ones_col, const int* __restrict__ ycols, int ny,
    double* __restrict__ xm, double* __restrict__ xs, unsigned char* __restrict__ ju,
    double* __restrict__ ym, double* __restrict__ ys, double* __restrict__ nobs) {
  const int s = blockIdx.y;
  const unsigned char* mk = masks + (int64_t)s * nseg;
  const double n = seg_sum(G, nseg, P, mk, ones_col, ones_col);
  const int e = blockIdx.x * blockDim.x + threadIdx.x;
  if (e < p) {
    const int j = e;
    const double mj = seg_sum(G, nseg, P, mk, ones_col, xcols[j]) / n;
    const double vj = seg_sum(G, nseg, P, mk, xcols[j], xcols[j]) / n - mj * mj;
    xm[(int64_t)s * p + j] = mj;
    xs[(int64_t)s * p + j] = vj > 0 ? sqrt(vj) : 1.0;
    ju[(int64_t)s * p + j] = vj > 0 ? 1 : 0;
    if (j == 0) nobs[s] = n;
  } else if (e < p + ny) {
    const int y = e - p;
    const double my = seg_sum(G, nseg, P, mk, ones_col, ycols[y]) / n;
    const double vy = seg_sum(G, nseg, P, mk, ycols[y], ycols[y]) / n - my * my;
    ym[(int64_t)s * ny + y] = my;
    ys[(int64_t)s * ny + y] = vy > 0 ? sqrt(vy) : 1.0;
  }
}

template <typename CT>
__global__ __launch_bounds__(256) void enet_prepare_kernel(
    const double* __restrict__ G, int nseg, int P, const unsigned char* __restrict__ masks,
    const int* __restrict__ xcols, int p, int ldc, const int* __restrict__ ycols, int ny,
    const double* __restrict__ xm, const double* __restrict__ xs,
    const unsigned char* __restrict__ ju, const double* __restrict__ ym,
    const double* __restrict__ ys, const double* __restrict__ nobs, CT* __restrict__ C,
    double* __restrict__ g) {
  const int s = blockIdx.y;
  const unsigned char* mk = masks + (int64_t)s * nseg;
  const double n = nobs[s];
  const int64_t total = (int64_t)p * p + (int64_t)ny * p;
  for (int64_t e = blockIdx.x * (int64_t)blockDim.x + threadIdx.x; e < total;
       e += (int64_t)gridDim.x * blockDim.x) {
    if (e < (int64_t)p * p) {
      const int j = (int)(e / p), k = (int)(e % p);
      const bool okj = ju[(int64_t)s * p + j], okk = ju[(int64_t)s * p + k];
      double cjk;
      if (!okj || !okk) {
        cjk = (j == k) ? 1.0 : 0.0;
      } else {
        const double mj = xm[(int64_t)s * p + j], mk2 = xm[(int64_t)s * p + k];
        cjk = (seg_sum(G, nseg, P, mk, xcols[j], xcols[k]) / n - mj * mk2) /
              (xs[(int64_t)s * p + j] * xs[(int64_t)s * p + k]);
      }
      C[((int64_t)s * p + j) * ldc + k] = (CT)cjk;
    } else {
      const int64_t r = e - (int64_t)p * p;
      const int y = (int)(r / p), j = (int)(r % p);
      double gj = 0.0;
      if (ju[(int64_t)s * p + j]) {
        const double mj = xm[(int64_t)s * p + j], my = ym[(int64_t)s * ny + y];
        gj = (seg_sum(G, nseg, P, mk, xcols[j], ycols[y]) / n - mj * my) /
             (xs[(int64_t)s * p + j] * ys[(int64_t)s * ny + y]);
      }
      g[((int64_t)s * ny + y) * p + j] = gj;
    }
  }
}

ATE_API int ate_enet_prepare(const void* G, int nseg, int P, const void* masks, int ntrain,
                             const void* xcols, int p, int ones_col, const void* ycols, int ny,
                             void* C, int c_f32, void* g, void* xm, void* xs, void* ju, void* ym,
                             void* ys, void* nobs, void* stream) {
  hipStream_t st = (hipStream_t)stream;
  ATE_LAUNCH(enet_prep_stats_kernel, dim3((p + ny + 255) / 256, ntrain), dim3(256), 0, st,
                     (const double*)G, nseg, P, (const unsigned char*)masks, (const int*)xcols,
                     p, ones_col, (const int*)ycols, ny, (double*)xm, (double*)xs,
                     (unsigned char*)ju, (double*)ym, (double*)ys, (double*)nobs);
  ATE_CHECK_LAUNCH();
  const int64_t total = (int64_t)p * p + (int64_t)ny * p;
  dim3 grid(grid_for(total, 256, 512), ntrain);
  const int ldc = (p + 63) / 64 * 64;
  if (c_f32)
    ATE_LAUNCH(enet_prepare_kernel<float>, grid, dim3(256), 0, st, (const double*)G, nseg,
                       P, (const unsigned char*)masks, (const int*)xcols, p, ldc,
                       (const int*)ycols, ny, (const double*)xm, (const double*)xs,
                       (const unsigned char*)ju, (const double*)ym, (const double*)ys,
                       (const double*)nobs, (float*)C, (double*)g);
  else
    ATE_LAUNCH(enet_prepare_kernel<double>, grid, dim3(256), 0, st, (const double*)G, nseg,
                       P, (const unsigned char*)masks, (const int*)xcols, p, ldc,
                       (const int*)ycols, ny, (const double*)xm, (const double*)xs,
                       (const unsigned char*)ju, (const double*)ym, (const double*)ys,
                       (const double*)nobs, (double*)C, (double*)g);
  ATE_CHECK_LAUNCH();
  return 0;
}

struct EnetProblem {
  int train;
  int y;
  int ulam_src;
  int nlam_req;
};

constexpr double BIGL = 9.9e35;
constexpr int PMAX = 512;

#ifdef ENET_PROF
__device__ unsigned long long enet_prof[256][32];
#define PROF_T(var) const unsigned long long var = wall_clock64()
#define PROF_ADD(k, v) do { if (tid == 0) sprof[0][k] += (unsigned long long)(v); } while (0)
#else
#define PROF_T(var)
#define PROF_ADD(k, v) do { } while (0)
#endif

template <typename CT> struct VecT;
template <> struct VecT<float> { typedef float4 type; };
template <> struct VecT<double> { typedef double2 type; };
__device__ __forceinline__ float vdot(float4 a, float4 b) {
  return a.x * b.x + a.y * b.y + a.z * b.z + a.w * b.w;
}
__device__ __forceinline__ double vdot(double2 a, double2 b) { return a.x * b.x + a.y * b.y; }

__device__ __forceinline__ void glds16f(const float* src, float* dst) {
  __builtin_amdgcn_global_load_lds(src, (__attribute__((address_space(3))) void*)dst, 16, 0, 0);
}
__device__ __forceinline__ void glds16f(const double*, float*) {}

__device__ __forceinline__ double readlane_d(double v, int i) {
  int lo = __builtin_amdgcn_readlane(__double2loint(v), i);
  int hi = __builtin_amdgcn_readlane(__double2hiint(v), i);
  return __hiloint2double(hi, lo);
}

__device__ __forceinline__ void select_lane(int i, int lane, double& a, double b, double& c, double d) {
  int a0 = __double2loint(a), a1 = __double2hiint(a), c0 = __double2loint(c), c1 = __double2hiint(c);
  asm volatile(
      "v_cmp_eq_u32_e32 vcc, %4, %5\n\t"
      "v_cndmask_b32_e32 %0, %0, %6, vcc\n\t"
      "v_cndmask_b32_e32 %1, %1, %7, vcc\n\t"
      "v_cndmask_b32_e32 %2, %2, %8, vcc\n\t"
      "v_cndmask_b32_e32 %3, %3, %9, vcc"
      : "+v"(a0), "+v"(a1), "+v"(c0), "+v"(c1)
      : "i"(i), "v"(lane), "v"(__double2loint(b)), "v"(__double2hiint(b)), "v"(__double2loint(d)),
        "v"(__double2hiint(d))
      : "vcc");
  a = __hiloint2double(a1, a0);
  c = __hiloint2double(c1, c0);
}

__device__ __forceinline__ void select_lane1(int i, int lane, double& a, double b) {
  int a0 = __double2loint(a), a1 = __double2hiint(a);
  asm volatile(
      "v_cmp_eq_u32_e32 vcc, %2, %3\n\t"
      "v_cndmask_b32_e32 %0, %0, %4, vcc\n\t"
      "v_cndmask_b32_e32 %1, %1, %5, vcc"
      : "+v"(a0), "+v"(a1)
      : "i"(i), "v"(lane), "v"(__double2loint(b)), "v"(__double2hiint(b))
      : "vcc");
  a = __hiloint2double(a1, a0);
}

template <int C>
__device__ __forceinline__ void fmac_bcast(double& u, double d, double nc) {
  asm volatile("s_nop 1\n\tv_fmac_f64_dpp %0, %1, %2 row_newbcast:%3 row_mask:0xf bank_mask:0xf"
               : "+v"(u)
               : "v"(d), "v"(nc), "i"(C));
}
template <int R>
__device__ __forceinline__ double row_replicate(double x) {
  unsigned w[2] = {(unsigned)__double2loint(x), (unsigned)__double2hiint(x)};
#pragma unroll
  for (int h = 0; h < 2; ++h) {
    const auto p = __builtin_amdgcn_permlane32_swap(w[h], w[h], false, false);
    const unsigned a = R < 2 ? p[0] : p[1];
    const auto q = __builtin_amdgcn_permlane16_swap(a, a, false, false);
    w[h] = (R & 1) ? q[1] : q[0];
  }
  return __hiloint2double((int)w[1], (int)w[0]);
}

__device__ __forceinline__ double clamp_hw(double u, double lo, double hi) {
  double r;
  asm("v_max_f64 %0, %1, %2\n\tv_min_f64 %0, %0, %3" : "=&v"(r) : "v"(u), "v"(lo), "v"(hi));
  return r;
}

__device__ __forceinline__ double lasso_step_hw(double u, double a, double lo, double hi) {
  double t, c;
  asm("v_add_f64 %0, %2, -%3\n\t"
      "v_max_f64 %1, %2, %4\n\t"
      "v_min_f64 %1, %1, %5\n\t"
      "v_add_f64 %1, %0, -%1"
      : "=&v"(t), "=&v"(c)
      : "v"(u), "v"(a), "v"(lo), "v"(hi));
  return c;
}

template <class F, int... C>
__device__ __forceinline__ void static_for_impl(F&& f, std::integer_sequence<int, C...>) {
  (f(std::integral_constant<int, C>{}), ...);
}
template <int N, class F>
__device__ __forceinline__ void static_for(F&& f) {
  static_for_impl(f, std::make_integer_sequence<int, N>{});
}

__global__ void enet_isa_selftest_kernel(double* out) {
  const int l = threadIdx.x;
  const double x = (double)l;
  out[l] = row_replicate<0>(x);
  out[64 + l] = row_replicate<1>(x);
  out[128 + l] = row_replicate<2>(x);
  out[192 + l] = row_replicate<3>(x);
  double u = 1.0;
  fmac_bcast<5>(u, x, 2.0);
  out[256 + l] = u;
}

ATE_API int ate_enet_isa_selftest(void* out, void* stream) {
  ATE_LAUNCH(enet_isa_selftest_kernel, dim3(1), dim3(64), 0, (hipStream_t)stream,
                     (double*)out);
  ATE_CHECK_LAUNCH();
  return 0;
}

#ifndef ENET_NW
#define ENET_NW 8
#endif
constexpr int NW = ENET_NW, NTH = NW * 64, NP = NW - 1;
static_assert(NW >= 3, "phase B uses wave 1 for block tn and waves 2.. for snapshots");
static_assert(NW >= PMAX / 64, "one pull wave per 64-column block: NW >= PMAX / 64");
#ifndef ENET_SETPRIO
#define ENET_SETPRIO 0
#endif
#ifndef ENET_BALLOT_ONLY
#define ENET_BALLOT_ONLY 0
#endif
#ifndef ENET_PULL_DENSE
#define ENET_PULL_DENSE 12
#endif
#ifndef ENET_ROWWALK
#define ENET_ROWWALK 0
#endif
#ifndef ENET_MODE_S
#define ENET_MODE_S 1
#endif
#ifndef ENET_S_ENTER
#define ENET_S_ENTER 40
#endif
#ifndef ENET_S_FETCH
#define ENET_S_FETCH 8
#endif
constexpr int S_UNION = 112 * 1024;
constexpr int S_CAP = S_UNION / (PMAX * 4);
#ifndef ENET_DENSE_MIN
#define ENET_DENSE_MIN 28
#endif

#define LDS_AS __attribute__((address_space(3)))
struct PassS {
  double dlx, rsq;
};
__device__ __noinline__ PassS enet_pass_s(bool full, int T, int ldc, double ab, double dem,
                                          const float* __restrict__ Cf, LDS_AS double* sg,
                                          LDS_AS double* sa, const LDS_AS double* svp,
                                          LDS_AS int* sflag, LDS_AS int* sslot,
                                          LDS_AS float* sccache, LDS_AS int* sever_n,
                                          LDS_AS int* sncache,
                                          LDS_AS unsigned long long* sprof_row) {
  const int lane = threadIdx.x & 63;
#ifdef ENET_PROF
  const long long tps0_ = clock64();
  unsigned long long nit_ = 0, nfetch_ = 0;
#endif
  double gS[8], aS[8], tS[8];
  int slS[8];
  int flb = 0;
#pragma unroll
  for (int s8 = 0; s8 < 8; ++s8) {
    const int k = s8 * 64 + lane;
    const bool in = s8 < T;
    gS[s8] = in ? sg[k] : 0.0;
    aS[s8] = in ? sa[k] : 0.0;
    tS[s8] = in ? svp[k] * ab : 0.0;
    slS[s8] = in ? sslot[k] : -1;
    const int f = in ? sflag[k] : 0;
    if ((f & 1) && (full || (f & 2))) flb |= 1 << s8;
    if (f & 2) flb |= 1 << (8 + s8);
  }
  int ncache = __builtin_amdgcn_readfirstlane(*sncache);
  int ever_n = __builtin_amdgcn_readfirstlane(*sever_n);
  double dlx = 0.0, rsq_add = 0.0;
#ifdef ENET_PROF
  const long long tpl0_ = clock64();
#endif
  static_for<8>([&](auto s_tag) __attribute__((always_inline)) {
    constexpr int SJ = decltype(s_tag)::value;
    if (SJ >= T) return;
    uint64_t live = ~0ull;
    for (;;) {
      const bool c = ((flb >> SJ) & 1) & ((aS[SJ] != 0.0) | (fabs(gS[SJ] + aS[SJ]) > tS[SJ]));
      const uint64_t cm = __builtin_amdgcn_ballot_w64(c) & live;
      if (!cm) break;
      const int lj = __ffsll((unsigned long long)cm) - 1;
      live = lj == 63 ? 0ull : (~0ull << (lj + 1));
#ifdef ENET_PROF
      ++nit_;
#endif
      const int j = SJ * 64 + lj;
      const double gj = readlane_d(gS[SJ], lj);
      const double aj = readlane_d(aS[SJ], lj);
      const double tj = readlane_d(tS[SJ], lj);
      int slj = __builtin_amdgcn_readlane(slS[SJ], lj);
      const double uj = gj + aj;
      double an = copysign(fmax(fabs(uj) - tj, 0.0), uj);
      if (dem != 0.0) an = an / (1.0 + svp[j] * dem);
      const double d = an - aj;
      if (__builtin_amdgcn_readfirstlane((int)(d == 0.0))) continue;
      float cv[8];
      if (slj < 0 && ncache < S_CAP) {
#ifdef ENET_PROF
        ++nfetch_;
#endif
        slj = ncache++;
        const float* Cj = Cf + (int64_t)j * ldc;
        LDS_AS float* dst = sccache + slj * PMAX;
#pragma unroll
        for (int s8 = 0; s8 < 8; ++s8) {
          const int k = s8 * 64 + lane;
          const float v = k < ldc ? Cj[k] : 0.f;
          cv[s8] = v;
          dst[(s8 >> 2) * 256 + lane * 4 + (s8 & 3)] = v;
        }
        if (lane == 0) sslot[j] = slj;
        if (lane == lj) slS[SJ] = slj;
      } else if (slj >= 0) {
        const LDS_AS float* src = sccache + slj * PMAX + lane * 4;
#pragma unroll
        for (int e = 0; e < 4; ++e) {
          cv[e] = src[e];
          cv[4 + e] = src[256 + e];
        }
      } else {
        const float* Cj = Cf + (int64_t)j * ldc;
#pragma unroll
        for (int s8 = 0; s8 < 8; ++s8) cv[s8] = s8 * 64 + lane < ldc ? Cj[s8 * 64 + lane] : 0.f;
      }
#pragma unroll
      for (int s8 = 0; s8 < 8; ++s8) gS[s8] = __builtin_fma(-(double)cv[s8], d, gS[s8]);
      const int evj = __builtin_amdgcn_readlane(flb, lj);
      if (!((evj >> (8 + SJ)) & 1)) ++ever_n;
      if (lane == lj) {
        flb |= 1 << (8 + SJ);
        aS[SJ] = an;
      }
      rsq_add += d * (2.0 * gj - d);
      dlx = fmax(dlx, d * d);
    }
  });
#ifdef ENET_PROF
  if (lane == 0) sprof_row[23] += (unsigned long long)(clock64() - tpl0_);
#endif
#pragma unroll
  for (int s8 = 0; s8 < 8; ++s8) {
    if (s8 < T) {
      const int k = s8 * 64 + lane;
      sg[k] = gS[s8];
      sa[k] = aS[s8];
      if ((flb >> (8 + s8)) & 1) sflag[k] |= 2;
    }
  }
  if (lane == 0) {
    *sever_n = ever_n;
    *sncache = ncache;
  }
#ifdef ENET_PROF
  if (lane == 0) {
    sprof_row[19] += 1ull;
    sprof_row[20] += nit_;
    sprof_row[21] += (unsigned long long)(clock64() - tps0_);
    sprof_row[22] += nfetch_;
  }
#endif
  return PassS{dlx, rsq_add};
}

constexpr int FOLD_LEAD = 2;

__device__ __noinline__ double lambda0_extrap(double l1, double l2) {
#pragma clang fp contract(off)
  return exp(2.0 * log(l1) - log(l2));
}

template <typename CT, bool LASSO>
__global__ __launch_bounds__(NTH) void enet_path_kernel(
    const CT* __restrict__ C, const double* __restrict__ gin, int p, int ny,
    const unsigned char* __restrict__ ju_s, const double* __restrict__ ys_s,
    const double* __restrict__ vp_in, const EnetProblem* __restrict__ probs, int nprob,
    double alpha, double flmin, double thr, int maxit,
    double* __restrict__ apath, double* __restrict__ lams, double* __restrict__ rsqs,
    int* __restrict__ nlam_out, int* __restrict__ npass_out, int L, int* __restrict__ progress,
    long spin_max, double* __restrict__ lampub) {
  constexpr int TMAX = PMAX / 64;
  __shared__ double sg[PMAX], sa[PMAX], svp[PMAX], sdc[PMAX];
  __shared__ __attribute__((aligned(16))) unsigned char s_union[S_UNION];
  double(&sds)[TMAX][PMAX] = *reinterpret_cast<double(*)[TMAX][PMAX]>(s_union);
  float(&sCn2)[2][64 * 64] = *reinterpret_cast<float(*)[2][64 * 64]>(s_union + 32768);
  float(&sCorr)[64 * 64] = *reinterpret_cast<float(*)[64 * 64]>(s_union + 65536);
  float* const sccache = reinterpret_cast<float*>(s_union);
  __shared__ int sslot[PMAX];
  __shared__ int sever_n;
  __shared__ int sncache;
  __shared__ int spub, sarr;
  __shared__ int sfetch0;
  __shared__ int sflag[PMAX];
  __shared__ double spart2[2][NW][64];
  __shared__ __attribute__((aligned(16))) float sred[NW][256];
  __shared__ __attribute__((aligned(16))) float sdw[NW][64];
  __shared__ int srow[NW][64];
  __shared__ float scorr2[2][NP][64];
  __shared__ int scorr_ok[2];
#ifdef ENET_PROF
  __shared__ unsigned long long sprof[NW][32];
  for (int e = threadIdx.x; e < NW * 32; e += blockDim.x) (&sprof[0][0])[e] = 0ull;
#endif
  __shared__ __attribute__((aligned(16))) CT sdelta[PMAX];
  __shared__ int slist[PMAX];
  constexpr int PER = (PMAX + NP - 1) / NP + 1;
  __shared__ int slist2[NP * PER];
  __shared__ __attribute__((aligned(16))) CT sdelta2[NP * PER];
  __shared__ int scl[64];
  __shared__ CT scd[64];
  __shared__ __attribute__((aligned(16))) float sdall[64];
  __shared__ int svis[8], snv, sblk_any[8], svis_id[8];
  __shared__ double sdl;
  __shared__ double srsq;
  __shared__ int snl_final;
  __shared__ int sany;
  __shared__ int schg;
  __shared__ double slam;
  __shared__ int savail;
  __shared__ int snpass_ring[4];
  int q;
  {
    int bid = blockIdx.x, nwg = gridDim.x;
    int xcd = bid & 7, qq = nwg >> 3, r = nwg & 7;
    q = ((xcd < r) ? xcd * (qq + 1) : r * (qq + 1) + (xcd - r) * qq) + (bid >> 3);
  }
  if (q >= nprob) return;
  const EnetProblem pr = probs[q];
  if (pr.ulam_src < -1) return;
  const int tid = threadIdx.x, lane = tid & 63, wid = tid >> 6;
#if ENET_SETPRIO
  if (ENET_SETPRIO == 2 || wid == 0) __builtin_amdgcn_s_setprio(3);
#endif
  const int T = (p + 63) >> 6;
  const int ldc = T * 64;
  const int cw = ldc / NW;
  const CT* Cq = C + (int64_t)pr.train * p * ldc;
  const double ysq = ys_s[(int64_t)pr.train * ny + pr.y];
  for (int k = tid; k < T * 64; k += NTH) {
    bool in = k < p;
    sg[k] = in ? gin[((int64_t)pr.train * ny + pr.y) * p + k] : 0.0;
    sa[k] = 0.0;
    svp[k] = in ? vp_in[k] : 0.0;
    sdc[k] = 0.0;
    sflag[k] = (in && ju_s[(int64_t)pr.train * p + k]) ? 1 : 0;
  }
  for (int e = tid; e < TMAX * PMAX; e += NTH) (&sds[0][0])[e] = 0.0;
  for (int k = tid; k < PMAX; k += NTH) sslot[k] = -1;
  if (tid < 8) svis_id[tid] = tid;
  if (tid == 0) { sever_n = 0; sncache = 0; spub = 0; sarr = 0; sfetch0 = 0; }
  __syncthreads();
  const int nlam = pr.ulam_src >= 0 ? L : pr.nlam_req;
  const double alf = pr.ulam_src >= 0 ? 1.0 : pow(flmin, 1.0 / (double)(nlam - 1));
  double alm = 0.0, rsq = 0.0, rsq_prev = 0.0;
  int npass = 0, m_out = 0;
  double ab = 0.0, dem = 0.0;
  double rsq_l = 0.0;
  typedef typename VecT<CT>::type V;
  constexpr int W = sizeof(V) / sizeof(CT);
  float dg_lo[32], dg_hi[32];
  int cpar = 0;

  auto pull_block = [&](int jb, int tb) __attribute__((always_inline)) -> float {
    ATE_DASSERT(jb >= 0 && jb < T && tb >= 0 && tb < T && jb != tb);
    const int grp = lane >> 4, c4 = (lane & 15) * 4;
    const int j = jb * 64 + lane;
    const double ddj = sdc[j] - sds[tb][j];
    const uint64_t nzb = __builtin_amdgcn_ballot_w64(ddj != 0.0);
    if (!nzb) return 0.f;
    const int n = __popcll(nzb);
    const float* Cf = reinterpret_cast<const float*>(Cq) + tb * 64 + c4;
    float* dw = sdw[wid];
    float4 a = make_float4(0.f, 0.f, 0.f, 0.f);
    auto fma4 = [&](float4 w, float d) __attribute__((always_inline)) {
      a.x += w.x * d;
      a.y += w.y * d;
      a.z += w.z * d;
      a.w += w.w * d;
    };
    if (n >= ENET_PULL_DENSE) {
      const int r0 = jb * 64 + grp * 16;
      float4 v[16];
#pragma unroll
      for (int u = 0; u < 16; ++u) {
        const int r = min(r0 + u, p - 1);
        v[u] = *reinterpret_cast<const float4*>(Cf + (int64_t)r * ldc);
      }
      dw[lane] = (float)ddj;
      __builtin_amdgcn_fence(__ATOMIC_RELEASE, "wavefront");
      __builtin_amdgcn_wave_barrier();
      __builtin_amdgcn_fence(__ATOMIC_ACQUIRE, "wavefront");
#pragma unroll
      for (int k = 0; k < 4; ++k) {
        const float4 d4 = *reinterpret_cast<const float4*>(dw + grp * 16 + 4 * k);
        fma4(v[4 * k + 0], d4.x);
        fma4(v[4 * k + 1], d4.y);
        fma4(v[4 * k + 2], d4.z);
        fma4(v[4 * k + 3], d4.w);
      }
    } else {
      int* rw = srow[wid];
      const int pos = __popcll(nzb & ((1ull << lane) - 1ull));
      if (ddj != 0.0) {
        rw[pos] = j;
        dw[pos] = (float)ddj;
      }
      __builtin_amdgcn_fence(__ATOMIC_RELEASE, "wavefront");
      __builtin_amdgcn_wave_barrier();
      __builtin_amdgcn_fence(__ATOMIC_ACQUIRE, "wavefront");
      constexpr int NS = (ENET_PULL_DENSE + 3) / 4;
      float4 v[NS];
      float dv[NS];
#pragma unroll
      for (int u = 0; u < NS; ++u) {
        if (4 * u < n) {
          const int idx = 4 * u + grp;
          const bool ok = idx < n;
          const int ix = ok ? idx : 0;
          v[u] = *reinterpret_cast<const float4*>(Cf + (int64_t)rw[ix] * ldc);
          dv[u] = ok ? dw[ix] : 0.f;
        }
      }
#pragma unroll
      for (int u = 0; u < NS; ++u)
        if (4 * u < n) fma4(v[u], dv[u]);
    }
    float* red = sred[wid];
    *reinterpret_cast<float4*>(red + grp * 64 + c4) = a;
    __builtin_amdgcn_fence(__ATOMIC_RELEASE, "wavefront");
    __builtin_amdgcn_wave_barrier();
    __builtin_amdgcn_fence(__ATOMIC_ACQUIRE, "wavefront");
    return (red[lane] + red[64 + lane]) + (red[128 + lane] + red[192 + lane]);
  };

  auto pull = [&](int t) __attribute__((always_inline)) {
    const int c0 = wid * cw;
    int cnt = 0;
    if constexpr (sizeof(CT) != 4) {
      for (int base = c0; base < c0 + cw; base += 64) {
        const int j = base + lane;
        const bool inq = j < c0 + cw;
        const double dj = inq ? sdc[j] - sds[t][j] : 0.0;
        const bool nz = dj != 0.0;
        const uint64_t bal = __ballot(nz);
        const int pos = cnt + __popcll(bal & ((1ull << lane) - 1ull));
        if (nz) { slist[c0 + pos] = j; sdelta[c0 + pos] = (CT)dj; }
        cnt += __popcll(bal);
      }
    }
    CT acc = 0;
    if constexpr (sizeof(CT) == 4) {
      const int jb = wid + (wid >= t ? 1 : 0);
      if (jb < T) acc = pull_block(jb, t);
    } else {
      const CT* colt = Cq + t * 64 + lane;
      int e = 0;
      for (; e + 16 <= cnt; e += 16) {
        CT v[16];
#pragma unroll
        for (int u = 0; u < 16; ++u) v[u] = colt[(int64_t)slist[c0 + e + u] * ldc];
#pragma unroll
        for (int u = 0; u < 16; ++u) acc += v[u] * sdelta[c0 + e + u];
      }
      for (; e < cnt; ++e) acc += colt[(int64_t)slist[c0 + e] * ldc] * sdelta[c0 + e];
    }
#ifdef ENET_PROF
    if (sizeof(CT) != 4 && lane == 0) sprof[wid][5] += (unsigned long long)cnt;
#endif
    if constexpr (sizeof(CT) == 4) {
      for (int pc = wid; pc < 16; pc += NW) {
        const int i = pc * 4 + (lane >> 4);
        const int r = min(t * 64 + i, p - 1);
        glds16f(Cq + (int64_t)r * ldc + t * 64 + (lane & 15) * 4, &sCn2[cpar][0] + pc * 256);
      }
    } else {
      for (int i = wid; i < 64; i += NW) {
        const int r = t * 64 + i;
        sCn2[cpar][i * 64 + lane] = r < p ? (float)Cq[(int64_t)r * ldc + t * 64 + lane] : 0.f;
      }
    }
    spart2[0][wid][lane] = (double)acc;
    __syncthreads();
    if (tid < 64) {
      const int k = t * 64 + tid;
      double sp = 0.0;
#pragma unroll
      for (int w = 0; w < NW; ++w) sp += spart2[0][w][tid];
      sg[k] -= sp;
    }
    for (int j = tid; j < ldc; j += NTH) sds[t][j] = sdc[j];
    __syncthreads();
  };

  auto pull_rest = [&](int t, int tn, int vpar) __attribute__((always_inline)) {
    ATE_DASSERT(t >= 0 && t < T && tn >= 0 && tn < T);
    const int my = wid - 1;
    CT acc = 0;
    if constexpr (sizeof(CT) == 4) {
      for (int pc = my; pc < 32; pc += NP) {
        const int blk = pc < 16 ? tn : t;
        const int i = (pc & 15) * 4 + (lane >> 4);
        const int r = min(blk * 64 + i, p - 1);
        const CT* src = Cq + (int64_t)r * ldc + tn * 64 + (lane & 15) * 4;
        float* dst = (pc < 16 ? &sCn2[cpar ^ 1][0] : sCorr) + (pc & 15) * 256;
        glds16f(src, dst);
      }
      const int jb = my + (my >= tn ? 1 : 0);
      if (jb < T) acc = pull_block(jb, tn);
    } else {
      const int base0 = my * PER;
      double dvv[TMAX];
#pragma unroll
      for (int c = 0; c < TMAX; ++c) {
        const int j = c * 64 + lane;
        dvv[c] = c < T ? sdc[j] - sds[tn][j] : 0.0;
      }
      uint64_t bals[TMAX];
      int pref[TMAX];
      int tot = 0;
#pragma unroll
      for (int c = 0; c < TMAX; ++c) {
        bals[c] = __builtin_amdgcn_ballot_w64(dvv[c] != 0.0);
        pref[c] = tot;
        tot += __popcll(bals[c]);
      }
      const int share = (tot + NP - 1) / NP;
      const int lo = my * share, hi = min(tot, lo + share);
      ATE_DASSERT(hi - lo <= PER);
      const uint64_t ltmask = (1ull << lane) - 1ull;
#pragma unroll
      for (int c = 0; c < TMAX; ++c) {
        const int pos = pref[c] + __popcll(bals[c] & ltmask);
        if (((bals[c] >> lane) & 1ull) && pos >= lo && pos < hi) {
          slist2[base0 + pos - lo] = c * 64 + lane;
          sdelta2[base0 + pos - lo] = (CT)dvv[c];
        }
      }
      const int cnt = max(0, hi - lo);
      const CT* colt = Cq + tn * 64 + lane;
      int e = 0;
      for (; e + 16 <= cnt; e += 16) {
        CT v[16];
#pragma unroll
        for (int u = 0; u < 16; ++u) v[u] = colt[(int64_t)slist2[base0 + e + u] * ldc];
#pragma unroll
        for (int u = 0; u < 16; ++u) acc += v[u] * sdelta2[base0 + e + u];
      }
      for (; e < cnt; ++e) acc += colt[(int64_t)slist2[base0 + e] * ldc] * sdelta2[base0 + e];
    }
    spart2[vpar][wid][lane] = (double)acc;
    if constexpr (sizeof(CT) == 4) return;
    constexpr int NR = (64 + NP - 1) / NP;
    float dr[NR];
#pragma unroll
    for (int ii = 0; ii < NR; ++ii) {
      const int i = my + NP * ii;
      const int r = tn * 64 + i;
      dr[ii] = (i < 64 && r < p) ? (float)Cq[(int64_t)r * ldc + tn * 64 + lane] : 0.f;
    }
#pragma unroll
    for (int ii = 0; ii < NR; ++ii) {
      const int i = my + NP * ii;
      if (i < 64) sCn2[cpar ^ 1][i * 64 + lane] = dr[ii];
    }
  };

  int ready = -1;
  int nvis = 0;
  int narr = 0;
  auto wait_ge = [&](int* c, int target) __attribute__((always_inline)) {
    while (__hip_atomic_load(c, __ATOMIC_RELAXED, __HIP_MEMORY_SCOPE_WORKGROUP) < target)
      __builtin_amdgcn_s_sleep(1);
    __builtin_amdgcn_fence(__ATOMIC_ACQUIRE, "workgroup");
  };
  auto pending_sum = [&](int par) __attribute__((always_inline)) -> double {
    double c0 = spart2[par][0][lane];
    if constexpr (sizeof(CT) == 4) {
      float cs = 0.f;
      if (scorr_ok[par]) {
#pragma unroll
        for (int w = 0; w < NP; ++w) cs += scorr2[par][w][lane];
      }
      c0 = (double)cs;
    }
    double sp = c0;
#pragma unroll
    for (int w = 1; w < NW; ++w) sp += spart2[par][w][lane];
    return sp;
  };
  bool modeS = sizeof(CT) == 4 && ENET_MODE_S != 0;
  auto pass = [&](bool full) __attribute__((always_inline)) -> double {
    if (modeS) {
      if (wid == 0) {
        const PassS r = enet_pass_s(
            full, T, ldc, ab, dem, reinterpret_cast<const float*>(Cq), (LDS_AS double*)sg,
            (LDS_AS double*)sa, (const LDS_AS double*)svp, (LDS_AS int*)sflag,
            (LDS_AS int*)sslot, (LDS_AS float*)sccache, (LDS_AS int*)&sever_n,
            (LDS_AS int*)&sncache,
#ifdef ENET_PROF
            (LDS_AS unsigned long long*)&sprof[0][0]
#else
            nullptr
#endif
        );
        if (lane == 0) {
          sdl = r.dlx;
          rsq_l += r.rsq;
        }
      }
      __syncthreads();
      const double r = sdl;
      __syncthreads();
      return r;
    }
    double dlx_l = 0.0;
    int nv = T;
    if (!full) {
      for (int t = wid; t < T; t += NW) {
        const bool a = (sflag[t * 64 + lane] & 3) == 3;
        const uint64_t b = __builtin_amdgcn_ballot_w64(a);
        if (lane == 0) sblk_any[t] = b != 0;
      }
      __syncthreads();
      if (tid == 0) {
        int c = 0;
        for (int t = 0; t < T; ++t)
          if (sblk_any[t]) svis[c++] = t;
        snv = c;
      }
      __syncthreads();
      nv = snv;
    }
    const int* vl = full ? svis_id : svis;
    if (nv == 0) {
      PROF_ADD(13, 1ull);
      return 0.0;
    }
    PROF_T(tp0_);
    PROF_ADD(12, 1ull);
    if (ready != vl[0]) pull(vl[0]);
    ready = -1;
    PROF_T(tp1_);
    PROF_ADD(0, tp1_ - tp0_);
    PROF_ADD(8, tp1_ - tp0_);
    for (int v = 0; v < nv; ++v) {
      const int t = vl[v];
      const int vpar = v & 1;
      const int tn = v + 1 < nv ? vl[v + 1] : (t != 0 ? 0 : -1);
      if (v + 1 == nv) ready = tn;
      const int k = t * 64 + lane;
      PROF_T(ta_);
      double gt = 0.0, at = 0.0, dblk = 0.0;
      CT corr = 0;
      int nc = 0;
      uint64_t chm = 0;
      int fl = 0;
      double dc0 = 0.0, ds0 = 0.0;
      if (wid == 0) {
#ifdef ENET_PROF
        const long long tv0_ = clock64();
#endif
#pragma unroll
        for (int i = 0; i < 32; ++i) {
          dg_lo[i] = sCn2[cpar][i * 64 + lane];
          dg_hi[i] = sCn2[cpar][(i + 32) * 64 + lane];
        }
        dc0 = sdc[k];
        gt = sg[k];
        at = sa[k];
        const double vpt = svp[k];
        fl = sflag[k];
        const int par = vpar ^ 1;
        double pend[NW];
#pragma unroll
        for (int w = 0; w < NW; ++w) pend[w] = spart2[par][w][lane];
        const bool cok = sizeof(CT) == 4 && scorr_ok[par];
        const bool elig = (fl & 1) && (full || (fl & 2));
        const double thr_l = vpt * ab;
        const double rden = (LASSO || dem == 0.0) ? 1.0 : 1.0 / (1.0 + vpt * dem);
#ifdef ENET_PROF
        const long long tw0_ = clock64();
#endif
        if (v > 0) wait_ge(&sarr, NP * narr);
#ifdef ENET_PROF
        const long long tw1_ = clock64();
        if (lane == 0) {
          sprof[wid][24] += (unsigned long long)(tw0_ - tv0_);
          sprof[wid][25] += (unsigned long long)(tw1_ - tw0_);
        }
#endif
        ds0 = sds[t][k];
        if (v > 0) {
          double c0 = pend[0];
          if constexpr (sizeof(CT) == 4) {
            float cs = 0.f;
            if (cok) {
#pragma unroll
              for (int w = 0; w < NP; ++w) cs += scorr2[par][w][lane];
            }
            c0 = (double)cs;
          }
          double sp = c0;
#pragma unroll
          for (int w = 1; w < NW; ++w) sp += pend[w];
          gt = gt - sp;
        }
        double gbef = 0.0;
        const double thr0 = elig ? (at != 0.0 ? -1.0 : thr_l) : __builtin_inf();
        uint64_t live = ~0ull, moved = 0ull;
        double anv = at;
        double u = gt + at;
#ifdef ENET_PROF
        unsigned long long nupd_ = 0;
#endif
        __builtin_amdgcn_s_waitcnt(0x0F70);
#ifdef ENET_PROF
        const long long tloop0_ = clock64();
        if (lane == 0) sprof[wid][17] += (unsigned long long)(tloop0_ - tv0_);
        if (lane == 0) sprof[wid][26] += (unsigned long long)(tloop0_ - tw1_);
#endif
        auto step = [&]() __attribute__((always_inline)) -> bool {
#pragma clang fp contract(off)
          const double au = fabs(u);
          const uint64_t msk = __builtin_amdgcn_ballot_w64(au > thr0) & live;
          const double an = __dmul_rn(copysign(fmax(au - thr_l, 0.0), u), rden);
          const double dd = an - at;
          asm volatile("" : : "v"(dd));
          if (!msk) return false;
          const int i = __ffsll((unsigned long long)msk) - 1;
          const float clo = dg_lo[i & 31], chi = dg_hi[i & 31];
          const float ci = i < 32 ? clo : chi;
          const double d = readlane_d(dd, i);
          const bool me = lane == i;
          gbef = me ? gt : gbef;
          const double cd = (double)ci * d;
          u -= cd;
          gt -= cd;
          __builtin_amdgcn_sched_barrier(0);
          live = i == 63 ? 0ull : (~0ull << (i + 1));
          moved |= 1ull << i;
          anv = me ? an : anv;
#ifdef ENET_PROF
          if (lane == 0) ++nupd_;
#endif
          return true;
        };
        auto step_known = [&](int i) __attribute__((always_inline)) {
#pragma clang fp contract(off)
          const double au = fabs(u);
          const double an = __dmul_rn(copysign(fmax(au - thr_l, 0.0), u), rden);
          const double dd = an - at;
          const float clo = dg_lo[i & 31], chi = dg_hi[i & 31];
          const float ci = i < 32 ? clo : chi;
          const double d = readlane_d(dd, i);
          const bool me = lane == i;
          gbef = me ? gt : gbef;
          const double cd = (double)ci * d;
          u -= cd;
          gt -= cd;
          __builtin_amdgcn_sched_barrier(0);
          anv = me ? an : anv;
#ifdef ENET_PROF
          if (lane == 0) ++nupd_;
#endif
        };
        const uint64_t em = __builtin_amdgcn_ballot_w64(elig);
        const uint64_t nzm = __builtin_amdgcn_ballot_w64(elig && at != 0.0);
        const int ncand = full ? __popcll(nzm) : __popcll(em);
        auto dense_walk = [&](auto lasso_tag) __attribute__((always_inline)) {
          constexpr bool LW = decltype(lasso_tag)::value;
          const double thr_e = elig ? thr_l : __builtin_inf();
          if constexpr (LW) {
            const double a0v = at;
            double usnap = u;
#if ENET_ROWWALK
            const int row = lane >> 4;
            auto row_pass = [&](auto r_tag) __attribute__((always_inline)) {
              constexpr int R = decltype(r_tag)::value;
              if (row == R) {
                asm volatile("s_nop 4");
                static_for<16>([&](auto c_tag) __attribute__((always_inline)) {
                  constexpr int C = decltype(c_tag)::value, I = R * 16 + C;
                  const double dd = lasso_step_hw(u, a0v, -thr_e, thr_e);
                  const float ci = I < 32 ? dg_lo[I] : dg_hi[I - 32];
                  select_lane1(I, lane, usnap, u);
                  fmac_bcast<C>(u, dd, -(double)ci);
                });
              }
              const double cls = fmin(fmax(usnap, -thr_e), thr_e);
              const double rep = row_replicate<R>((usnap - a0v) - cls);
              if (row != R) {
                asm volatile("s_nop 4");
                static_for<16>([&](auto c_tag) __attribute__((always_inline)) {
                  constexpr int C = decltype(c_tag)::value, I = R * 16 + C;
                  const float ci = I < 32 ? dg_lo[I] : dg_hi[I - 32];
                  fmac_bcast<C>(u, rep, -(double)ci);
                });
              }
            };
            row_pass(std::integral_constant<int, 0>{});
            row_pass(std::integral_constant<int, 1>{});
            row_pass(std::integral_constant<int, 2>{});
            row_pass(std::integral_constant<int, 3>{});
#else
#pragma unroll
            for (int i = 0; i < 64; ++i) {
              const double cl = fmin(fmax(u, -thr_e), thr_e);
              const double dd = (u - a0v) - cl;
              const float ci = i < 32 ? dg_lo[i] : dg_hi[i - 32];
              const double d = readlane_d(dd, i);
              select_lane1(i, lane, usnap, u);
              u = __builtin_fma(-(double)ci, d, u);
            }
#endif
            {
              const double cl = fmin(fmax(usnap, -thr_e), thr_e);
              gbef = usnap - a0v;
              anv = usnap - cl;
            }
            gt = u - a0v;
          } else {
#pragma unroll
            for (int i = 0; i < 64; ++i) {
#pragma clang fp contract(off)
              const double au = fabs(u);
              const double sv = copysign(fmax(au - thr_e, 0.0), u);
              const double an = __dmul_rn(sv, rden);
              const double dd = an - at;
              const float ci = i < 32 ? dg_lo[i] : dg_hi[i - 32];
              const double d = readlane_d(dd, i);
              select_lane(i, lane, gbef, gt, anv, an);
              const double cd = (double)ci * d;
              u -= cd;
              gt -= cd;
            }
          }
#ifdef ENET_PROF
          if (lane == 0) nupd_ += 64;
#endif
        };
        if (!ENET_BALLOT_ONLY && ncand >= ENET_DENSE_MIN) {
          moved = ~0ull;
          if (LASSO || dem == 0.0) dense_walk(std::true_type{});
          else if constexpr (!LASSO) dense_walk(std::false_type{});
        } else if (full || ENET_BALLOT_ONLY) {
          while (step() && step()) {
          }
        } else {
          uint64_t rem = em;
          moved = rem;
          while (rem) {
            const int i = __ffsll((unsigned long long)rem) - 1;
            rem &= rem - 1ull;
            step_known(i);
            if (!rem) break;
            const int i2 = __ffsll((unsigned long long)rem) - 1;
            rem &= rem - 1ull;
            step_known(i2);
          }
        }
#ifdef ENET_PROF
        if (lane == 0) sprof[wid][15] += (unsigned long long)(clock64() - tloop0_);
        const long long tpost0_ = clock64();
#endif
        if ((moved >> lane) & 1ull) {
          const double dn = anv - at;
          if (dn != 0.0) {
            dblk = dn;
            at = anv;
          }
        }
#ifdef ENET_PROF
        if (lane == 0) {
          const unsigned long long tl_ = wall_clock64() - ta_;
          sprof[wid][6] += tl_;
          sprof[wid][7] += nupd_;

          sprof[wid][14] += 1ull;
        }
#endif
        if (dblk != 0.0) {
          rsq_l += dblk * (2.0 * gbef - dblk);
          dlx_l = fmax(dlx_l, dblk * dblk);
          fl |= 2;
        }
        if (sizeof(CT) != 4 && tn >= 0) {
          const bool ch = dblk != 0.0;
          const uint64_t bal = __builtin_amdgcn_ballot_w64(ch);
          const int pos = __popcll(bal & ((1ull << lane) - 1ull));
          if (ch) { scl[pos] = k; scd[pos] = (CT)dblk; }
          nc = __popcll(bal);
          chm = bal;
          const CT* colt = Cq + tn * 64 + lane;
          int e = 0;
          for (; e + 16 <= nc; e += 16) {
            CT w[16];
#pragma unroll
            for (int u = 0; u < 16; ++u) w[u] = colt[(int64_t)scl[e + u] * ldc];
#pragma unroll
            for (int u = 0; u < 16; ++u) corr += w[u] * scd[e + u];
          }
          for (; e < nc; ++e) corr += colt[(int64_t)scl[e] * ldc] * scd[e];
        }
        if constexpr (sizeof(CT) != 4) {
          spart2[vpar][0][lane] = (double)corr;
        } else if (tn >= 0) {
          sdall[lane] = (float)dblk;
          const uint64_t chg = __builtin_amdgcn_ballot_w64(dblk != 0.0);
          if (lane == 0) schg = chg != 0ull;
        }
#ifdef ENET_PROF
        if (lane == 0) sprof[wid][2] += (unsigned long long)(wall_clock64() - ta_);
        if (lane == 0) sprof[wid][28] += (unsigned long long)(clock64() - tpost0_);
#endif
      } else if (tn >= 0) {
        wait_ge(&spub, nvis);
        wait_ge(&sarr, NP * narr);
        pull_rest(t, tn, vpar);
#ifdef ENET_PROF
        if (wid == 1 && lane == 0)
          sprof[wid][4] += (unsigned long long)(wall_clock64() - ta_);
        if (wid == NW - 1 && lane == 0)
          sprof[wid][18] += (unsigned long long)(wall_clock64() - ta_);
#endif
      }
#ifdef ENET_PROF
      const long long tsb_ = clock64();
#endif
      __syncthreads();
#ifdef ENET_PROF
      if (wid == 0 && lane == 0) sprof[0][27] += (unsigned long long)(clock64() - tsb_);
#endif
      PROF_T(tb_);
      PROF_ADD(1, tb_ - ta_);
      PROF_ADD(3, 1);
      const double dnew = dc0 + dblk;
      if (wid == 0) {
        sg[k] = gt;
        sa[k] = at;
        sflag[k] = fl;
        sdc[k] = dnew;
        sds[t][k] = ds0 + dblk;
        if (tn >= 0) {
          sds[tn][k] = dnew;
          if constexpr (sizeof(CT) == 4) {
            if (lane == 0) scorr_ok[vpar] = schg;
          }
        }
        __builtin_amdgcn_fence(__ATOMIC_RELEASE, "workgroup");
        if (lane == 0) __hip_atomic_store(&spub, nvis + 1, __ATOMIC_RELAXED, __HIP_MEMORY_SCOPE_WORKGROUP);
#ifdef ENET_PROF
        if (lane == 0) sprof[wid][9] += (unsigned long long)(wall_clock64() - tb_);
#endif
      } else if (tn >= 0) {
        const int my = wid - 1;
        if (sizeof(CT) == 4 && schg) {
          constexpr int RPW = (64 + NP - 1) / NP;
          float cv[RPW], dv[RPW];
#pragma unroll
          for (int j = 0; j < RPW; ++j) {
            const int r = my + NP * j;
            cv[j] = r < 64 ? sCorr[r * 64 + lane] : 0.f;
            dv[j] = r < 64 ? sdall[r] : 0.f;
          }
          float a = 0.f;
#pragma unroll
          for (int j = 0; j < RPW; ++j) a = __builtin_fmaf(cv[j], dv[j], a);
          scorr2[vpar][my][lane] = a;
        }
        for (int j = my * 64 + lane; j < ldc; j += NP * 64)
          if ((j >> 6) != t) sds[tn][j] = sdc[j];
        __builtin_amdgcn_fence(__ATOMIC_RELEASE, "workgroup");
        if (lane == 0) __hip_atomic_fetch_add(&sarr, 1, __ATOMIC_RELAXED, __HIP_MEMORY_SCOPE_WORKGROUP);
#ifdef ENET_PROF
        if (wid == 1 && lane == 0) sprof[wid][16] += (unsigned long long)(wall_clock64() - tb_);
#endif
      }
      if (tn >= 0) {
        cpar ^= 1;
        ++narr;
      }
      ++nvis;
      PROF_T(tc_);
      PROF_ADD(0, tc_ - tb_);
    }
    if (ready >= 0) {
      if (wid == 0) {
        wait_ge(&sarr, NP * narr);
        const int kr = ready * 64 + lane;
        sg[kr] = sg[kr] - pending_sum((nv - 1) & 1);
      }
    }
    __syncthreads();
    const double dlx = wave_max(dlx_l);
    if (tid == 0) sdl = dlx;
    __syncthreads();
    return sdl;
  };

  auto publish = [&](int v) {
    asm volatile("s_waitcnt vmcnt(0)" ::: "memory");
    __builtin_amdgcn_fence(__ATOMIC_RELEASE, "agent");
    asm volatile("s_waitcnt vmcnt(0)" ::: "memory");
    __hip_atomic_store(progress + q, v, __ATOMIC_RELAXED, __HIP_MEMORY_SCOPE_AGENT);
  };
#ifdef ENET_PROF
  const long long kc0_ = clock64();
  const unsigned long long kw0_ = wall_clock64();
#endif
  const bool is_fold = pr.ulam_src >= 0;
  bool timed_out = false;
  int vseen = 0;
  double lam_lo = 0.0, lam_hi = 0.0;
  bool lam_reg = false;
  for (int m = 0; m < nlam; ++m) {
#ifdef ENET_PROF
    const unsigned long long tlam0_ = wall_clock64();
#endif
    if (is_fold) {
      if (wid == 0) {
        const int need = m <= FOLD_LEAD + 1 ? 2 : m - FOLD_LEAD + 1;
        int v = vseen;
        if (v < need) {
          if (lane == 0) {
            for (long spin = 0;; ++spin) {
              v = __hip_atomic_load(progress + pr.ulam_src, __ATOMIC_RELAXED, __HIP_MEMORY_SCOPE_AGENT);
              if (v >= need) break;
              if (spin > spin_max) { v = -1; break; }
              __builtin_amdgcn_s_sleep(2);
            }
          }
          v = __builtin_amdgcn_readfirstlane(v);
          __builtin_amdgcn_fence(__ATOMIC_ACQUIRE, "agent");
          asm volatile("s_waitcnt vmcnt(0)" ::: "memory");
          if (v > 0) vseen = v;
          if (v >= 2 && v < (1 << 30) && !lam_reg && L <= 128) {
            const double* lp = lampub + (int64_t)pr.ulam_src * L;
            lam_lo = lane < L ? lp[lane] : 0.0;
            lam_hi = 64 + lane < L ? lp[64 + lane] : 0.0;
            lam_reg = true;
          }
        }
        int avail = 0;
        double lv = 0.0;
        if (v < 0) {
          timed_out = true;
        } else if (v >= (1 << 30)) {
          if (lane == 0) {
            int nl = __hip_atomic_load(nlam_out + pr.ulam_src, __ATOMIC_RELAXED, __HIP_MEMORY_SCOPE_AGENT);
            avail = m < nl;
            if (avail) lv = __hip_atomic_load(lams + (int64_t)pr.ulam_src * L + m, __ATOMIC_RELAXED,
                                              __HIP_MEMORY_SCOPE_AGENT);
          }
        } else if (lam_reg) {
          avail = 1;
          lv = readlane_d(m < 64 ? lam_lo : lam_hi, m & 63);
        } else {
          avail = 1;
          if (lane == 0)
            lv = __hip_atomic_load(lampub + (int64_t)pr.ulam_src * L + m, __ATOMIC_RELAXED,
                                   __HIP_MEMORY_SCOPE_AGENT);
        }
        if (lane == 0) {
          savail = avail;
          slam = lv;
        }
      }
      __syncthreads();
      const int avail = savail;
      alm = slam / ysq;
      if (!avail) break;
    } else if (m == 0) {
      alm = BIGL;
    } else if (m == 1) {
      if (!modeS) {
        for (int t = 0; t < T; ++t) pull(t);
        ready = -1;
      }
      double mx = 0.0;
      for (int k = lane; k < p; k += 64)
        if ((sflag[k] & 1) && svp[k] > 0.0) mx = fmax(mx, fabs(sg[k]) / svp[k]);
      mx = wave_max(mx);
      alm = alf * mx / fmax(alpha, 1e-3);
      if (tid == 0 && L >= 3) {
        double* lp = lampub + (int64_t)q * L;
        double x = alm, x2 = alm;
        lp[1] = x * ysq;
        for (int mm = 2; mm < L; ++mm) {
          x *= alf;
          lp[mm] = x * ysq;
          if (mm == 2) x2 = x;
        }
        lp[0] = lambda0_extrap(lp[1], x2 * ysq);
        publish(2);
      }
    } else {
      alm *= alf;
    }
    ab = alm * alpha;
    dem = LASSO ? 0.0 : alm * (1.0 - alpha);
    const int fetched = sncache - sfetch0;
    __syncthreads();
    if (tid == 0) sfetch0 = sncache;
    if (modeS && (sever_n > ENET_S_ENTER || fetched > ENET_S_FETCH)) {
      modeS = false;
      for (int e = tid; e < TMAX * PMAX; e += NTH) (&sds[0][0])[e] = 0.0;
      ready = -1;
      __syncthreads();
    }
#ifdef ENET_PROF
    const unsigned long long tpass0_ = wall_clock64();
    if (tid == 0) sprof[0][29] += tpass0_ - tlam0_;
#endif
    while (npass < maxit) {
      ++npass;
      double dl = pass(true);
      if (dl < thr) break;
      while (npass < maxit) {
        ++npass;
        dl = pass(false);
        if (dl < thr) break;
      }
    }
#ifdef ENET_PROF
    const unsigned long long tpend_ = wall_clock64();
    if (tid == 0) sprof[0][5] += tpend_ - tpass0_;
#endif
    double* ap = apath + ((int64_t)q * L + m) * p;
    for (int k = tid; k < p; k += NTH) ap[k] = sa[k];
    rsq = wave_sum(rsq_l);
    if (tid == 0) srsq = rsq;
    __syncthreads();
    const double rsq_all = srsq;
    if (tid == 0) {
      lams[(int64_t)q * L + m] = alm * ysq;
      rsqs[(int64_t)q * L + m] = rsq_all;
      if (!is_fold && m == 2)
        lams[(int64_t)q * L] = lambda0_extrap(lams[(int64_t)q * L + 1], alm * ysq);
      if (!is_fold && m >= 2)
        __hip_atomic_store(progress + q, m + 1, __ATOMIC_RELAXED, __HIP_MEMORY_SCOPE_AGENT);
    }
    m_out = m + 1;
    if (tid == 0) snpass_ring[m & 3] = npass;
    if (pr.ulam_src < 0 && m >= 4 && m > 0) {
      if (rsq_all - rsq_prev < 1e-5 * rsq_all || rsq_all > 0.999) break;
    }
    rsq_prev = rsq_all;
#ifdef ENET_PROF
    if (tid == 0) sprof[0][30] += wall_clock64() - tpend_;
#endif
  }
  if (is_fold) {
    if (tid == 0) {
      int v = 0;
      for (long spin = 0;; ++spin) {
        v = __hip_atomic_load(progress + pr.ulam_src, __ATOMIC_RELAXED, __HIP_MEMORY_SCOPE_AGENT);
        if (v >= (1 << 30)) break;
        if (spin > spin_max) { v = -1; break; }
        __builtin_amdgcn_s_sleep(2);
      }
      __builtin_amdgcn_fence(__ATOMIC_ACQUIRE, "agent");
      asm volatile("s_waitcnt vmcnt(0)" ::: "memory");
      if (v < 0) timed_out = true;
      snl_final = v < 0 ? m_out
                     : __hip_atomic_load(nlam_out + pr.ulam_src, __ATOMIC_RELAXED, __HIP_MEMORY_SCOPE_AGENT);
    }
    __syncthreads();
    const int nl = snl_final;
    if (m_out > nl) {
      ATE_DASSERT(m_out - nl <= FOLD_LEAD + 1);
      for (int mm = nl; mm < m_out; ++mm) {
        double* ap = apath + ((int64_t)q * L + mm) * p;
        for (int k = tid; k < p; k += NTH) ap[k] = 0.0;
        if (tid == 0) {
          lams[(int64_t)q * L + mm] = __builtin_nan("");
          rsqs[(int64_t)q * L + mm] = 0.0;
        }
      }
      npass = nl > 0 ? snpass_ring[(nl - 1) & 3] : 0;
      m_out = nl;
    }
  }
#ifdef ENET_PROF
  __syncthreads();
  if (tid < 32) {
    unsigned long long acc = 0;
    for (int w = 0; w < NW; ++w) acc += sprof[w][tid];
    if (tid == 10) acc = (unsigned long long)(clock64() - kc0_);
    if (tid == 11) acc = wall_clock64() - kw0_;
    atomicAdd(&enet_prof[q][tid], acc);
  }
#endif
  if (tid == 0) {
    nlam_out[q] = m_out;
    npass_out[q] = timed_out ? -1 : npass;
    if (!is_fold) publish(1 << 30);
  }
}

#ifdef ENET_PROF
extern "C" __attribute__((visibility("default"))) int ate_enet_prof_read(void* host) {
  return (int)hipMemcpyFromSymbol(host, HIP_SYMBOL(enet_prof), sizeof(enet_prof));
}
extern "C" __attribute__((visibility("default"))) int ate_enet_prof_reset() {
  static unsigned long long z[256][32];
  return (int)hipMemcpyToSymbol(HIP_SYMBOL(enet_prof), z, sizeof(z));
}
#endif

ATE_KERNEL_SHAPE("enet_path_kernel<float, lasso>", NTH, 0, enet_path_kernel<float, true>)
ATE_KERNEL_SHAPE("enet_path_kernel<float, enet>", NTH, 0, enet_path_kernel<float, false>)
ATE_KERNEL_SHAPE("enet_path_kernel<double, lasso>", NTH, 0, enet_path_kernel<double, true>)
ATE_KERNEL_SHAPE("enet_path_kernel<double, enet>", NTH, 0, enet_path_kernel<double, false>)

ATE_API int ate_enet_path(const void* C, int c_f32, const void* g, int p, int ny, const void* ju,
                          const void* ys, const void* vp, const void* probs, int nprob,
                          double alpha, double flmin, double thr, int maxit, void* apath,
                          void* lams, void* rsqs, void* nlam_out, void* npass_out, int L,
                          void* progress, void* lampub, void* stream) {
  if (p > PMAX) return -2;
  if (nprob > 256) return -3;
  hipStream_t s = (hipStream_t)stream;
  const int nwg = (nprob + 7) / 8 * 8;
  const char* sm = getenv("ATE_ENET_SPIN_MAX");
  const long spin_max = sm ? atol(sm) : (1l << 26);
#define LAUNCH_C(CTT, LS)                                                                      \
  ATE_LAUNCH((enet_path_kernel<CTT, LS>), dim3(nwg), dim3(NTH), 0, s, (const CTT*)C,   \
                     (const double*)g, p, ny, (const unsigned char*)ju, (const double*)ys,     \
                     (const double*)vp, (const EnetProblem*)probs, nprob, alpha, flmin, thr,   \
                     maxit, (double*)apath, (double*)lams, (double*)rsqs, (int*)nlam_out,     \
                     (int*)npass_out, L, (int*)progress, spin_max, (double*)lampub)
  const bool lasso = alpha == 1.0;
  if (c_f32 && lasso) LAUNCH_C(float, true);
  else if (c_f32) LAUNCH_C(float, false);
  else if (lasso) LAUNCH_C(double, true);
  else LAUNCH_C(double, false);
#undef LAUNCH_C
  ATE_CHECK_LAUNCH();
  return 0;
}

__global__ void enet_coef_kernel(const double* __restrict__ apath, const EnetProblem* __restrict__ probs,
                                 int nprob, int p, int ny, int L, const int* __restrict__ nlam_out,
                                 const double* __restrict__ xm, const double* __restrict__ xs,
                                 const unsigned char* __restrict__ ju, const double* __restrict__ ym,
                                 const double* __restrict__ ys, double* __restrict__ coef) {
  const int q = blockIdx.y, m = blockIdx.x;
  if (q >= nprob || m >= L) return;
  const EnetProblem pr = probs[q];
  double* out = coef + ((int64_t)q * L + m) * (p + 1);
  if (m >= nlam_out[q]) {
    for (int j = threadIdx.x; j <= p; j += blockDim.x) out[j] = NAN;
    return;
  }
  const double* a = apath + ((int64_t)q * L + m) * p;
  const double ysq = ys[(int64_t)pr.train * ny + pr.y], ymq = ym[(int64_t)pr.train * ny + pr.y];
  __shared__ double smem[16];
  double acc[1] = {0.0};
  for (int j = threadIdx.x; j < p; j += blockDim.x) {
    int64_t sj = (int64_t)pr.train * p + j;
    double b = ju[sj] ? a[j] * ysq / xs[sj] : 0.0;
    out[1 + j] = b;
    acc[0] += b * xm[sj];
  }
  block_sum<1>(acc, smem);
  if (threadIdx.x == 0) out[0] = ymq - acc[0];
}

ATE_API int ate_enet_coef(const void* apath, const void* probs, int nprob, int p, int ny, int L,
                          const void* nlam_out, const void* xm, const void* xs, const void* ju,
                          const void* ym, const void* ys, void* coef, void* stream) {
  ATE_LAUNCH(enet_coef_kernel, dim3(L, nprob), dim3(128), 0, (hipStream_t)stream,
                     (const double*)apath, (const EnetProblem*)probs, nprob, p, ny, L,
                     (const int*)nlam_out, (const double*)xm, (const double*)xs,
                     (const unsigned char*)ju, (const double*)ym, (const double*)ys,
                     (double*)coef);
  ATE_CHECK_LAUNCH();
  return 0;
}

constexpr int CVL = 8;
constexpr int CVK = PMAX / 64;

__global__ __launch_bounds__(256) void enet_cvloss_gauss_kernel(
    const double* __restrict__ G, int P, const int* __restrict__ hold,
    const int* __restrict__ xcols, int p, int ones_col, const int* __restrict__ ycol_of_prob,
    const double* __restrict__ coef, const int* __restrict__ nlam_out, int L, int q0,
    double* __restrict__ cvraw) {
  const int q = q0 + blockIdx.x, m0 = (gridDim.y - 1 - blockIdx.y) * CVL;
  const int nl = nlam_out[q];
  const int tid = threadIdx.x, lane = tid & 63, wid = tid >> 6;
  if (m0 >= nl) {
    if (tid < CVL && m0 + tid < L) cvraw[(int64_t)q * L + m0 + tid] = NAN;
    return;
  }
  const double* Gh = G + (int64_t)hold[q] * P * P;
  const int yc = ycol_of_prob[q];
  __shared__ double sbeta[CVL][PMAX];
  __shared__ int sxc[PMAX];
  __shared__ unsigned char snz[PMAX];
  __shared__ double sred[4][3 * CVL];
  for (int e = tid; e < CVL * PMAX; e += 256) {
    const int m = e / PMAX, j = e % PMAX;
    const bool ok = j < p && m0 + m < nl;
    sbeta[m][j] = ok ? coef[((int64_t)q * L + m0 + m) * (p + 1) + 1 + j] : 0.0;
  }
  for (int j = tid; j < PMAX; j += 256) sxc[j] = j < p ? xcols[j] : xcols[0];
  __syncthreads();
  for (int j = tid; j < PMAX; j += 256) {
    bool any = false;
#pragma unroll
    for (int m = 0; m < CVL; ++m) any |= sbeta[m][j] != 0.0;
    snz[j] = any;
  }
  __syncthreads();
  double bl[CVK][CVL];
#pragma unroll
  for (int k = 0; k < CVK; ++k)
#pragma unroll
    for (int m = 0; m < CVL; ++m) bl[k][m] = sbeta[m][k * 64 + lane];
  int cl[CVK];
#pragma unroll
  for (int k = 0; k < CVK; ++k) cl[k] = sxc[k * 64 + lane];
  double quad[CVL], lin[CVL], sx[CVL];
#pragma unroll
  for (int m = 0; m < CVL; ++m) { quad[m] = 0.0; lin[m] = 0.0; sx[m] = 0.0; }
  if (wid == 0) {
#pragma unroll
    for (int k = 0; k < CVK; ++k) {
      if (k * 64 + lane >= p) continue;
      const double gy = Gh[(int64_t)cl[k] * P + yc], g1 = Gh[(int64_t)cl[k] * P + ones_col];
#pragma unroll
      for (int m = 0; m < CVL; ++m) {
        lin[m] = fma(bl[k][m], gy, lin[m]);
        sx[m] = fma(bl[k][m], g1, sx[m]);
      }
    }
  }
  auto next_row = [&](int a) {
    while (a < p && !snz[a]) a += 4;
    return a;
  };
  auto load_row = [&](int a, double* g) {
    const double* Gr = Gh + (int64_t)sxc[a] * P;
#pragma unroll
    for (int k = 0; k < CVK; ++k) g[k] = (k * 64 + lane < p) ? Gr[cl[k]] : 0.0;
  };
  double gn[CVK];
  int a = next_row(wid);
  if (a < p) load_row(a, gn);
  while (a < p) {
    double g[CVK];
#pragma unroll
    for (int k = 0; k < CVK; ++k) g[k] = gn[k];
    const int an = next_row(a + 4);
    if (an < p) load_row(an, gn);
#pragma unroll
    for (int m = 0; m < CVL; ++m) {
      double t = 0.0;
#pragma unroll
      for (int k = 0; k < CVK; ++k) t = fma(g[k], bl[k][m], t);
      quad[m] = fma(sbeta[m][a], t, quad[m]);
    }
    a = an;
  }
#pragma unroll
  for (int m = 0; m < CVL; ++m) {
    quad[m] = wave_sum(quad[m]);
    lin[m] = wave_sum(lin[m]);
    sx[m] = wave_sum(sx[m]);
  }
  if (lane == 0)
#pragma unroll
    for (int m = 0; m < CVL; ++m) {
      sred[wid][m] = quad[m];
      sred[wid][CVL + m] = lin[m];
      sred[wid][2 * CVL + m] = sx[m];
    }
  __syncthreads();
  if (tid < CVL && m0 + tid < L) {
    const int m = tid;
    if (m0 + m >= nl) {
      cvraw[(int64_t)q * L + m0 + m] = NAN;
    } else {
      const double qd = sred[0][m] + sred[1][m] + sred[2][m] + sred[3][m];
      const double ln = sred[0][CVL + m], s1 = sred[0][2 * CVL + m];
      const double a0 = coef[((int64_t)q * L + m0 + m) * (p + 1)];
      const double n = Gh[(int64_t)ones_col * P + ones_col];
      const double yy = Gh[(int64_t)yc * P + yc], sy = Gh[(int64_t)ones_col * P + yc];
      const double sse = yy - 2.0 * a0 * sy - 2.0 * ln + n * a0 * a0 + 2.0 * a0 * s1 + qd;
      cvraw[(int64_t)q * L + m0 + m] = sse / n;
    }
  }
}

ATE_API int ate_enet_cvloss_gauss(const void* G, int P, const void* hold, const void* xcols, int p,
                                  int ones_col, const void* ycol_of_prob, const void* coef,
                                  const void* nlam_out, int L, int q0, int nprob, void* cvraw,
                                  void* stream) {
  if (p > PMAX) return -1;
  if (nprob <= 0) return 0;
  ATE_LAUNCH(enet_cvloss_gauss_kernel, dim3(nprob, (L + CVL - 1) / CVL), dim3(256), 0,
                     (hipStream_t)stream, (const double*)G, P, (const int*)hold,
                     (const int*)xcols, p, ones_col, (const int*)ycol_of_prob,
                     (const double*)coef, (const int*)nlam_out, L, q0, (double*)cvraw);
  ATE_CHECK_LAUNCH();
  return 0;
}

__device__ __forceinline__ bool any_truncated(const int* fnp, int nfp) {
  bool bad = false;
  if (fnp)
    for (int i = threadIdx.x; i < nfp; i += blockDim.x) bad |= fnp[i] < 0;
  return __syncthreads_or(bad) != 0;
}

__global__ __launch_bounds__(64) void cv_select_kernel(
    const double* __restrict__ cvraw, const int* __restrict__ fold_probs,
    const double* __restrict__ nfold, int K, int nfull, const int* __restrict__ nlam_full, int L,
    double* __restrict__ cvm, double* __restrict__ cvsd, int* __restrict__ sel,
    const int* __restrict__ fnp, int nfp) {
  const int f = blockIdx.x;
  const int lane = threadIdx.x;
  if (f >= nfull) return;
  if (any_truncated(fnp, nfp)) {
    for (int m = lane; m < L; m += 64) {
      cvm[(int64_t)f * L + m] = NAN;
      cvsd[(int64_t)f * L + m] = NAN;
    }
    if (lane == 0) { sel[2 * f] = 0; sel[2 * f + 1] = 0; }
    return;
  }
  const int nl = nlam_full[f];
  double wsum = 0.0;
  for (int k = 0; k < K; ++k) wsum += nfold[f * K + k];
  double mus[4], sds[4];
  double best = INFINITY;
  int imin = 0x7fffffff;
#pragma unroll
  for (int c = 0; c < 4; ++c) {
    const int m = c * 64 + lane;
    mus[c] = INFINITY;
    sds[c] = 0.0;
    if (m >= nl) {
      if (m < L) {
        cvm[(int64_t)f * L + m] = NAN;
        cvsd[(int64_t)f * L + m] = NAN;
      }
      continue;
    }
    double mu = 0.0;
    for (int k = 0; k < K; ++k) mu += nfold[f * K + k] * cvraw[(int64_t)fold_probs[f * K + k] * L + m];
    mu /= wsum;
    double var = 0.0;
    for (int k = 0; k < K; ++k) {
      double d = cvraw[(int64_t)fold_probs[f * K + k] * L + m] - mu;
      var += nfold[f * K + k] * d * d;
    }
    const double sd = sqrt(var / wsum / (double)(K - 1));
    cvm[(int64_t)f * L + m] = mu;
    cvsd[(int64_t)f * L + m] = sd;
    mus[c] = mu;
    sds[c] = sd;
    if (mu < best) { best = mu; imin = m; }
  }
#pragma unroll
  for (int o = 32; o > 0; o >>= 1) {
    const double ob = __shfl_xor(best, o, 64);
    const int oi = __shfl_xor(imin, o, 64);
    if (ob < best || (ob == best && oi < imin)) { best = ob; imin = oi; }
  }
  if (imin == 0x7fffffff) imin = 0;
  const int oc = imin >> 6, ol = imin & 63;
  double mine = 0.0;
#pragma unroll
  for (int c = 0; c < 4; ++c)
    if (c == oc) mine = mus[c] + sds[c];
  const double thr1 = __shfl(mine, ol, 64);
  int i1 = imin;
#pragma unroll
  for (int c = 0; c < 4; ++c) {
    const uint64_t b = __ballot(c * 64 + lane < nl && mus[c] <= thr1);
    if (b) { i1 = c * 64 + __ffsll((unsigned long long)b) - 1; break; }
  }
  if (lane == 0) {
    sel[2 * f] = imin;
    sel[2 * f + 1] = i1;
  }
}

ATE_API int ate_cv_select(const void* cvraw, const void* fold_probs, const void* nfold, int K,
                          int nfull, const void* nlam_full, int L, void* cvm, void* cvsd, void* sel,
                          const void* fold_npass, int nfp, void* stream) {
  if (L > 256) return -1;
  ATE_LAUNCH(cv_select_kernel, dim3(nfull), dim3(64), 0, (hipStream_t)stream,
                     (const double*)cvraw, (const int*)fold_probs, (const double*)nfold, K, nfull,
                     (const int*)nlam_full, L, (double*)cvm, (double*)cvsd, (int*)sel,
                     (const int*)fold_npass, nfp);
  ATE_CHECK_LAUNCH();
  return 0;
}

__global__ void enet_pick_kernel(const double* __restrict__ coef, const int* __restrict__ sel,
                                 int p, int L, int nfull, double* __restrict__ out_min,
                                 double* __restrict__ out_1se, const int* __restrict__ fnp,
                                 int nfp) {
  const int f = blockIdx.x, which = blockIdx.y;
  double* out = which ? out_1se : out_min;
  const bool bad = any_truncated(fnp, nfp);
  const int m = sel[2 * f + which];
  for (int j = threadIdx.x; j <= p; j += blockDim.x)
    out[(int64_t)f * (p + 1) + j] = bad ? NAN : coef[((int64_t)f * L + m) * (p + 1) + j];
}

ATE_API int ate_enet_pick(const void* coef, const void* sel, int p, int L, int nfull,
                          void* out_min, void* out_1se, const void* fold_npass, int nfp,
                          void* stream) {
  ATE_LAUNCH(enet_pick_kernel, dim3(nfull, 2), dim3(128), 0, (hipStream_t)stream,
                     (const double*)coef, (const int*)sel, p, L, nfull, (double*)out_min,
                     (double*)out_1se, (const int*)fold_npass, nfp);
  ATE_CHECK_LAUNCH();
  return 0;
}
```

csrc/stats.hip:

```cpp
#include "common.hpp"

using namespace ate;

constexpr int RB = 256;
constexpr int RGRID = 1024;

template <int NV, class F>
__global__ __launch_bounds__(RB) void rowreduce_kernel(F f, int64_t n, double* __restrict__ partial) {
  __shared__ double smem[16 * NV];
  double v[NV];
#pragma unroll
  for (int k = 0; k < NV; ++k) v[k] = 0.0;
  for (int64_t i = blockIdx.x * (int64_t)RB + threadIdx.x; i < n; i += (int64_t)gridDim.x * RB)
    f(i, v);
  block_sum<NV>(v, smem);
  if (threadIdx.x == 0)
#pragma unroll
    for (int k = 0; k < NV; ++k) partial[blockIdx.x * NV + k] = v[k];
}

template <int NV>
__global__ void slab_sum_kernel(const double* __restrict__ partial, int nb, double* __restrict__ out) {
  int k = threadIdx.x;
  if (k >= NV) return;
  double s = 0.0;
  for (int b = 0; b < nb; ++b) s += partial[b * NV + k];
  out[k] = s;
}

template <int NV, class F>
static int rowreduce(F f, int64_t n, double* partial, double* out, hipStream_t s) {
  int nb = grid_for(n, RB, RGRID);
  ATE_LAUNCH((rowreduce_kernel<NV, F>), dim3(nb), dim3(RB), 0, s, f, n, partial);
  ATE_CHECK_LAUNCH();
  ATE_LAUNCH(slab_sum_kernel<NV>, dim3(1), dim3(64), 0, s, partial, nb, out);
  ATE_CHECK_LAUNCH();
  return 0;
}

template <typename T>
struct GroupMoments {
  const T* y; const T* w; const T* valid;
  __device__ void operator()(int64_t i, double (&v)[6]) const {
    if (valid && valid[i] == T(0)) return;
    double yi = (double)y[i];
    int g = (double)w[i] != 0.0 ? 3 : 0;
    v[g] += 1.0; v[g + 1] += yi; v[g + 2] += yi * yi;
  }
};

__global__ void naive_finalize_kernel(const double* __restrict__ m, double* __restrict__ res) {
  double n0 = m[0], n1 = m[3];
  double mu0 = m[1] / n0, mu1 = m[4] / n1;
  double v0 = (m[2] - n0 * mu0 * mu0) / (n0 - 1.0);
  double v1 = (m[5] - n1 * mu1 * mu1) / (n1 - 1.0);
  res[0] = mu1 - mu0;
  res[1] = sqrt(v0 / (n0 - 1.0) + v1 / (n1 - 1.0));
}

template <typename T>
static int naive_t(const void* y, const void* w, const void* valid, int64_t n, void* partial,
                   void* moments, void* res, hipStream_t s) {
  GroupMoments<T> f{(const T*)y, (const T*)w, (const T*)valid};
  int rc = rowreduce<6>(f, n, (double*)partial, (double*)moments, s);
  if (rc) return rc;
  ATE_LAUNCH(naive_finalize_kernel, dim3(1), dim3(1), 0, s, (const double*)moments,
                     (double*)res);
  ATE_CHECK_LAUNCH();
  return 0;
}

ATE_API int ate_naive(int dtype, const void* y, const void* w, const void* valid, int64_t n,
                      void* partial, void* moments, void* res, void* stream) {
  hipStream_t s = (hipStream_t)stream;
  if (dtype == 1) return naive_t<float>(y, w, valid, n, partial, moments, res, s);
  if (dtype == 2) return naive_t<double>(y, w, valid, n, partial, moments, res, s);
  return -1;
}

__global__ __launch_bounds__(RB) void clip_minmax_kernel(const double* __restrict__ p, const double* __restrict__ valid,
                                   int64_t n, double* __restrict__ partial) {
  __shared__ double sm[2][16];
  double mn = INFINITY, mx = -INFINITY;
  for (int64_t i = blockIdx.x * (int64_t)RB + threadIdx.x; i < n; i += (int64_t)gridDim.x * RB) {
    if (valid && valid[i] == 0.0) continue;
    double pi = p[i];
    if (pi > 0.0) mn = fmin(mn, pi);
    if (pi < 1.0) mx = fmax(mx, pi);
  }
  mn = -wave_max(-mn);
  mx = wave_max(mx);
  int lane = threadIdx.x & 63, wid = threadIdx.x >> 6;
  if (lane == 0) { sm[0][wid] = mn; sm[1][wid] = mx; }
  __syncthreads();
  if (threadIdx.x == 0) {
    for (int w = 1; w < RB / 64; ++w) { mn = fmin(mn, sm[0][w]); mx = fmax(mx, sm[1][w]); }
    partial[2 * blockIdx.x] = mn;
    partial[2 * blockIdx.x + 1] = mx;
  }
}

__global__ void clip_apply_kernel(double* __restrict__ p, int64_t n, const double* __restrict__ partial,
                                  int nb) {
  __shared__ double lim[2];
  if (threadIdx.x == 0) {
    double mn = INFINITY, mx = -INFINITY;
    for (int b = 0; b < nb; ++b) { mn = fmin(mn, partial[2 * b]); mx = fmax(mx, partial[2 * b + 1]); }
    lim[0] = mn; lim[1] = mx;
  }
  __syncthreads();
  for (int64_t i = blockIdx.x * (int64_t)blockDim.x + threadIdx.x; i < n;
       i += (int64_t)gridDim.x * blockDim.x) {
    const double p0 = p[i];
    double pi = p0;
    if (pi == 0.0 && lim[0] < INFINITY) pi = lim[0];
    if (pi == 1.0 && lim[1] > -INFINITY) pi = lim[1];
    if (pi != p0) p[i] = pi;
  }
}

ATE_API int ate_clip_propensity(void* p, const void* valid, int64_t n, void* partial, void* stream) {
  hipStream_t s = (hipStream_t)stream;
  int nb = grid_for(n, RB, RGRID);
  ATE_LAUNCH(clip_minmax_kernel, dim3(nb), dim3(RB), 0, s, (const double*)p,
                     (const double*)valid, n, (double*)partial);
  ATE_CHECK_LAUNCH();
  ATE_LAUNCH(clip_apply_kernel, dim3(grid_for(n, 256)), dim3(256), 0, s, (double*)p, n,
                     (const double*)partial, nb);
  ATE_CHECK_LAUNCH();
  return 0;
}

struct AipwMoments {
  const double *w, *y, *p, *mu0, *mu1, *valid; double sign;
  __device__ void operator()(int64_t i, double (&v)[6]) const {
    if (valid && valid[i] == 0.0) return;
    double wi = w[i], yi = y[i], pi = p[i], m0 = mu0[i], m1 = mu1[i];
    double e1 = wi * (yi - m1) / pi + sign * (1.0 - wi) * (yi - m0) / (1.0 - pi);
    if (e1 == e1) { v[0] += e1; v[1] += 1.0; }
    v[2] += m1 - m0;
    v[3] += 1.0;
    double a = wi * yi / pi - m1 * (wi - pi) / pi - ((1.0 - wi) * yi / (1.0 - pi) + m0 * (wi - pi) / (1.0 - pi));
    if (a == a) { v[4] += a; v[5] += a * a; }
  }
};

__global__ void aipw_finalize_kernel(const double* __restrict__ m, double* __restrict__ res) {
  double tau = m[0] / m[1] + m[2] / m[3];
  double n = m[3];
  double ss = m[5] - 2.0 * tau * m[4] + n * tau * tau;
  res[0] = tau;
  res[1] = sqrt(fmax(ss, 0.0)) / n;
}

ATE_API int ate_aipw(const void* w, const void* y, const void* p, const void* mu0, const void* mu1,
                     const void* valid, int64_t n, double sign, void* partial, void* moments,
                     void* res, void* stream) {
  hipStream_t s = (hipStream_t)stream;
  AipwMoments f{(const double*)w, (const double*)y, (const double*)p, (const double*)mu0,
                (const double*)mu1, (const double*)valid, sign};
  int rc = rowreduce<6>(f, n, (double*)partial, (double*)moments, s);
  if (rc) return rc;
  ATE_LAUNCH(aipw_finalize_kernel, dim3(1), dim3(1), 0, s, (const double*)moments,
                     (double*)res);
  ATE_CHECK_LAUNCH();
  return 0;
}

struct DmlMoments {
  const double *yr, *wr, *valid;
  __device__ void operator()(int64_t i, double (&v)[7]) const {
    if (valid && valid[i] == 0.0) return;
    double y = yr[i], w = wr[i], w2 = w * w;
    v[0] += w * y; v[1] += w2; v[2] += y * y * w2; v[3] += y * w2 * w; v[4] += w2 * w2;
    v[5] += 1.0; v[6] += y * y;
  }
};

__global__ void dml_finalize_kernel(const double* __restrict__ m, int mode, double* __restrict__ res) {
  double n = m[5];
  double theta = m[0] / m[1];
  double se;
  if (mode == 0) {
    double j = m[1] / n;
    double psi2 = (m[2] - 2.0 * theta * m[3] + theta * theta * m[4]) / n;
    se = sqrt(fmax(psi2, 0.0) / (j * j) / n);
  } else {
    double rss = m[6] - 2.0 * theta * m[0] + theta * theta * m[1];
    se = sqrt(fmax(rss, 0.0) / (n - 1.0) / m[1]);
  }
  res[0] = theta;
  res[1] = se;
}

ATE_API int ate_dml_moments(const void* yr, const void* wr, const void* valid, int64_t n,
                            void* partial, void* moments, void* stream) {
  DmlMoments f{(const double*)yr, (const double*)wr, (const double*)valid};
  return rowreduce<7>(f, n, (double*)partial, (double*)moments, (hipStream_t)stream);
}

ATE_API int ate_dml_finalize(const void* moments, int mode, void* res, void* stream) {
  ATE_LAUNCH(dml_finalize_kernel, dim3(1), dim3(1), 0, (hipStream_t)stream,
                     (const double*)moments, mode, (double*)res);
  ATE_CHECK_LAUNCH();
  return 0;
}

__global__ __launch_bounds__(256) void boot_multinomial_kernel(
    const double* __restrict__ e1, const double* __restrict__ e2, int64_t n, uint64_t seed,
    int b0, double* __restrict__ taus) {
  __shared__ double smem[16 * 3];
  const int b = blockIdx.x;
  double v[3] = {0.0, 0.0, 0.0};
  for (int64_t j = threadIdx.x; j < n; j += blockDim.x) {
    uint32_t r = rand_below(seed, P_BOOT, (uint32_t)(b0 + b), (uint64_t)j, (uint32_t)n);
    double a = e1[r];
    if (a == a) { v[0] += a; v[1] += 1.0; }
    v[2] += e2[r];
  }
  block_sum<3>(v, smem);
  if (threadIdx.x == 0) taus[b] = v[0] / v[1] + v[2] / (double)n;
}

__device__ __forceinline__ int poisson1(float u) {
  const float cdf[8] = {0.36787944f, 0.73575888f, 0.91969860f, 0.98101184f,
                        0.99634015f, 0.99940582f, 0.99991676f, 0.99998975f};
  int k = 0;
#pragma unroll
  for (int q = 0; q < 8; ++q) k += (u >= cdf[q]) ? 1 : 0;
  return k;
}

__global__ __launch_bounds__(256) void boot_poisson_kernel(
    const double* __restrict__ e1, const double* __restrict__ e2, int64_t n, uint64_t seed, int b0,
    int B, int64_t row_offset, double* __restrict__ partial) {
  __shared__ double red[4][64][4];
  const int nrep_pad = ((B + 63) / 64) * 64;
  const int lane = threadIdx.x & 63, wid = threadIdx.x >> 6;
  const int b = blockIdx.y * 64 + lane;
  double s1 = 0.0, sok = 0.0, s2 = 0.0, sc = 0.0;
  if (b < B) {
    for (int64_t i = blockIdx.x * 4 + wid; i < n; i += (int64_t)gridDim.x * 4) {
      u32x4 r = rand4(seed, P_BOOT, (uint32_t)(b0 + b), (uint64_t)(row_offset + i) | (1ull << 62));
      int c = poisson1((float)(r.x >> 8) * (1.0f / 16777216.0f));
      if (c) {
        double a = e1[i];
        if (a == a) { s1 += c * a; sok += c; }
        s2 += c * e2[i];
        sc += c;
      }
    }
  }
  red[wid][lane][0] = s1; red[wid][lane][1] = sok; red[wid][lane][2] = s2; red[wid][lane][3] = sc;
  __syncthreads();
  if (wid == 0) {
    for (int w = 1; w < 4; ++w) {
      s1 += red[w][lane][0]; sok += red[w][lane][1]; s2 += red[w][lane][2]; sc += red[w][lane][3];
    }
    double* out = partial + ((int64_t)blockIdx.x * nrep_pad + blockIdx.y * 64 + lane) * 4;
    out[0] = s1; out[1] = sok; out[2] = s2; out[3] = sc;
  }
}

ATE_API int ate_boot_multinomial(const void* e1, const void* e2, int64_t n, uint64_t seed, int b0,
                                 int B, void* taus, void* stream) {
  if (n > 0xFFFFFFFFll) return -1;
  ATE_LAUNCH(boot_multinomial_kernel, dim3(B), dim3(256), 0, (hipStream_t)stream,
                     (const double*)e1, (const double*)e2, n, seed, b0, (double*)taus);
  ATE_CHECK_LAUNCH();
  return 0;
}

ATE_API int ate_boot_poisson(const void* e1, const void* e2, int64_t n, uint64_t seed, int b0,
                             int B, int64_t row_offset, int nb, void* partial, void* stream) {
  dim3 grid(nb, (B + 63) / 64);
  ATE_LAUNCH(boot_poisson_kernel, grid, dim3(256), 0, (hipStream_t)stream,
                     (const double*)e1, (const double*)e2, n, seed, b0, B, row_offset,
                     (double*)partial);
  ATE_CHECK_LAUNCH();
  return 0;
}
```

Measured before the change: 2.268 billion rows/s.

## Fuse enet CV tail and DML residual finalize into last-block-done kernels

Merges the enet coefficient unscaling, CV loss, CV selection and pick steps into one kernel. A per-fold atomic counter lets the last finishing block do the select and pick. The enet prepare step also fills the lambda buffer, and some zeroing memsets are dropped. The DML residual moment kernel now does the 7-moment reduction and the finalize formula in its last block, using agent-scope stores and a fence. This removes several small kernel launches and memsets on the critical path, at the cost of atomic-counter complexity and different reduction ordering.

```diff
diff --git a/ate_replication_causalml_amd/_native.py b/ate_replication_causalml_amd/_native.py
--- a/ate_replication_causalml_amd/_native.py
+++ b/ate_replication_causalml_amd/_native.py
@@ -77,12 +77,15 @@
     "ate_boot_poisson": "ppluiilipp",
     "ate_enet_isa_selftest": "pp",
     "ate_enet_prepare": "piipipiipipipppppppp",
+    "ate_enet_prepare_fused": "piipipiipipi" + "ppppppp" + "plp",
     "ate_enet_path": "pipiippppidddipppppippp",
     "ate_enet_coef": "ppiiiipppppppp",
     "ate_enet_cvloss_gauss": "pippiipppiiipp",
     "ate_cv_select": "pppiipippppip",
     "ate_enet_pick": "ppiiipppip",
+    "ate_enet_cv_tail": "pippiipppi" + "pppppp" + "iiii" + "pppppppppppp",
     "ate_dml_resid_moments": "ipllpipipiiiiiippp",
+    "ate_dml_resid_moments_final": "ipllpipipiiiiii" + "ppppp",
     "ate_dml_resid_exact": "pllpipipiiiiiiippp",
     "ate_irm_score_moments": "ipllpipiipiiiiidippp",
     "ate_irm_score_moments_multi": "ipllpipiipipiiiiiidippp",
diff --git a/ate_replication_causalml_amd/estimators/lasso.py b/ate_replication_causalml_amd/estimators/lasso.py
--- a/ate_replication_causalml_amd/estimators/lasso.py
+++ b/ate_replication_causalml_amd/estimators/lasso.py
@@ -4,6 +4,7 @@
 import torch
 
 from .. import _native
+from ..ops import enet as enet_ops
 from ..ops import stats as S
 from ..ops.devconst import const
 from ..ops.enet import cv_enet_gaussian
@@ -337,9 +338,14 @@
         return (cv.coef_min if lambda_rule == "min" else cv.coef_1se).reshape(
             len(mine), 2, -1).contiguous()
 
+    fused_final = enet_ops.CV_FUSED and not dist and pan.data.is_cuda
+
     def phase_fit(st):
         cv = fit(st)
         coef = pick(cv)
+        if fused_final:
+            mom, res = dml_residual_moments(pan, coef, final=True)
+            return {**st, "cv": cv, "mom": mom, "res": res}
         return {**st, "cv": cv, "mom": dml_residual_moments(pan, coef)}
 
     def phase_fit_sharded(st):
@@ -353,6 +359,8 @@
         return {**st, "mom": dml_residual_moments(pan, st["coef"])}
 
     def phase_final(st):
+        if "res" in st:
+            return st
         return {**st, "res": S.dml_finalize(st["mom"], "plr")}
 
     cap = bool(getattr(comm, "capturable", False))
@@ -530,7 +538,7 @@
     return part
 
 
-def dml_residual_moments(pan, coef: torch.Tensor) -> torch.Tensor:
+def dml_residual_moments(pan, coef: torch.Tensor, final: bool = False):
     K = coef.shape[0]
     p = len(pan.xcols)
     if not pan.data.is_cuda:
@@ -557,6 +565,14 @@
     y0, y1 = (pan.cols["Y_hi"], pan.cols["Y_lo"]) if bf else (pan.cols["Y"], -1)
     w0, w1 = (pan.cols["W_hi"], pan.cols["W_lo"]) if bf else (pan.cols["W"], -1)
     cs, bs = pan.strides()
+    if final:
+        res = torch.empty(2, dtype=torch.float64, device=dev)
+        done = torch.zeros(1, dtype=torch.int32, device=dev)
+        _native.call("ate_dml_resid_moments_final", dtype_code(pan.data), pan.data.data_ptr(), cs,
+                     bs, xc.data_ptr(), p, segs.data_ptr(), K, coef.data_ptr(), y0, y1, w0, w1,
+                     pan.cols["one"], nbx, part.data_ptr(), done.data_ptr(), mom.data_ptr(),
+                     res.data_ptr(), torch.cuda.current_stream().cuda_stream)
+        return mom, res
     _native.call("ate_dml_resid_moments", dtype_code(pan.data), pan.data.data_ptr(), cs, bs,
                  xc.data_ptr(), p, segs.data_ptr(), K, coef.data_ptr(), y0, y1, w0, w1,
                  pan.cols["one"], nbx, part.data_ptr(), mom.data_ptr(),
diff --git a/ate_replication_causalml_amd/ops/enet.py b/ate_replication_causalml_amd/ops/enet.py
--- a/ate_replication_causalml_amd/ops/enet.py
+++ b/ate_replication_causalml_amd/ops/enet.py
@@ -1,5 +1,6 @@
 from __future__ import annotations
 
+import os
 from dataclasses import dataclass
 
 import numpy as np
@@ -12,6 +13,9 @@
 
 def _stream():
     return torch.cuda.current_stream().cuda_stream
+
+
+CV_FUSED = os.environ.get("ATE_CV_FUSED", "1") not in ("", "0")
 
 
 @dataclass
@@ -173,9 +177,20 @@
     probs_all = list(full_probs) + list(fold_probs)
     nq = len(probs_all)
     i32 = torch.int32
-    C, apath, rsq, nlam, npass, progress = _zeroed(
-        dev, ((nt, p, ldc), torch.float32 if c_f32 else torch.float64), ((nq, L, p), torch.float64),
-        ((nq, L), torch.float64), ((nq,), i32), ((nq,), i32), ((nq,), i32))
+    c_dt = torch.float32 if c_f32 else torch.float64
+    fused = CV_FUSED and L <= 256
+    fused_prep = fused and nseg <= 8
+    if fused:
+        zspec = [((nq, L), torch.float64), ((nq,), i32), ((nq,), i32), ((nq,), i32), ((nf,), i32)]
+        if not fused_prep:
+            zspec.append(((nt, p, ldc), c_dt))
+        rsq, nlam, npass, progress, done, *zc = _zeroed(dev, *zspec)
+        C = zc[0] if zc else torch.empty((nt, p, ldc), dtype=c_dt, device=dev)
+        apath = torch.empty((nq, L, p), **f64)
+    else:
+        C, apath, rsq, nlam, npass, progress = _zeroed(
+            dev, ((nt, p, ldc), c_dt), ((nq, L, p), torch.float64),
+            ((nq, L), torch.float64), ((nq,), i32), ((nq,), i32), ((nq,), i32))
     g = torch.empty((nt, ny, p), **f64)
     xm = torch.empty((nt, p), **f64)
     xs = torch.empty((nt, p), **f64)
@@ -183,39 +198,57 @@
     ym = torch.empty((nt, ny), **f64)
     ys = torch.empty((nt, ny), **f64)
     nobs = torch.empty(nt, **f64)
-    _native.call("ate_enet_prepare", G.data_ptr(), nseg, P, masks_t.data_ptr(), nt, xc.data_ptr(),
-                 p, one, yc.data_ptr(), ny, C.data_ptr(), c_f32, g.data_ptr(), xm.data_ptr(),
-                 xs.data_ptr(), ju.data_ptr(), ym.data_ptr(), ys.data_ptr(), nobs.data_ptr(), s)
+    if fused_prep:
+        lams = torch.empty((nq, L), **f64)
+        _native.call("ate_enet_prepare_fused", G.data_ptr(), nseg, P, masks_t.data_ptr(), nt,
+                     xc.data_ptr(), p, one, yc.data_ptr(), ny, C.data_ptr(), c_f32, g.data_ptr(),
+                     xm.data_ptr(), xs.data_ptr(), ju.data_ptr(), ym.data_ptr(), ys.data_ptr(),
+                     nobs.data_ptr(), lams.data_ptr(), nq * L, s)
+    else:
+        _native.call("ate_enet_prepare", G.data_ptr(), nseg, P, masks_t.data_ptr(), nt,
+                     xc.data_ptr(), p, one, yc.data_ptr(), ny, C.data_ptr(), c_f32, g.data_ptr(),
+                     xm.data_ptr(), xs.data_ptr(), ju.data_ptr(), ym.data_ptr(), ys.data_ptr(),
+                     nobs.data_ptr(), s)
+        lams = torch.full((nq, L), float("nan"), **f64)
     vp_t = const(np.asarray(vp, dtype=np.float64), torch.float64, dev)
     pr = _probs_tensor(probs_all, dev)
-    lams = torch.full((nq, L), float("nan"), **f64)
     lampub = torch.empty((nq, L), **f64)
     _native.call("ate_enet_path", C.data_ptr(), c_f32, g.data_ptr(), p, ny, ju.data_ptr(),
                  ys.data_ptr(), vp_t.data_ptr(), pr.data_ptr(), nq, alpha, flmin, thresh,
                  maxit, apath.data_ptr(), lams.data_ptr(), rsq.data_ptr(), nlam.data_ptr(),
                  npass.data_ptr(), L, progress.data_ptr(), lampub.data_ptr(), s)
-    coef = torch.empty((nq, L, p + 1), **f64)
-    _native.call("ate_enet_coef", apath.data_ptr(), pr.data_ptr(), nq, p, ny, L,
-                 nlam.data_ptr(), xm.data_ptr(), xs.data_ptr(), ju.data_ptr(), ym.data_ptr(),
-                 ys.data_ptr(), coef.data_ptr(), s)
     hold = const([0] * nf + list(fold_holds), torch.int32, dev)
     ycol_p = const([0] * nf + list(fold_ycol), torch.int32, dev)
     cvraw = torch.empty((nq, L), **f64)
-    _native.call("ate_enet_cvloss_gauss", G.data_ptr(), P, hold.data_ptr(), xc.data_ptr(), p, one,
-                 ycol_p.data_ptr(), coef.data_ptr(), nlam.data_ptr(), L, nf, nq - nf,
-                 cvraw.data_ptr(), s)
     fidx = const(fold_index + nf, torch.int32, dev)
     nfold_t = const(nfold, torch.float64, dev)
     cvm = torch.empty((nf, L), **f64)
     cvsd = torch.empty((nf, L), **f64)
     sel = torch.empty((nf, 2), dtype=torch.int32, device=dev)
     K = fold_index.shape[1]
+    cmin = torch.empty((nf, p + 1), **f64)
+    c1se = torch.empty((nf, p + 1), **f64)
     fold_npass = npass[nf:]
+    if fused:
+        coef = torch.empty((nf, L, p + 1), **f64)
+        _native.call("ate_enet_cv_tail", G.data_ptr(), P, hold.data_ptr(), xc.data_ptr(), p, one,
+                     ycol_p.data_ptr(), apath.data_ptr(), pr.data_ptr(), ny, nlam.data_ptr(),
+                     xm.data_ptr(), xs.data_ptr(), ju.data_ptr(), ym.data_ptr(), ys.data_ptr(), L,
+                     nf, nq - nf, K, fidx.data_ptr(), nfold_t.data_ptr(), coef.data_ptr(),
+                     cvraw.data_ptr(), cvm.data_ptr(), cvsd.data_ptr(), sel.data_ptr(),
+                     cmin.data_ptr(), c1se.data_ptr(), fold_npass.data_ptr(), done.data_ptr(), s)
+        return EnetCvResult(lams[:nf], nlam[:nf], cvm, cvsd, sel, coef, cmin, c1se, full_keys,
+                            npass[:nf], fold_npass, nlam[nf:])
+    coef = torch.empty((nq, L, p + 1), **f64)
+    _native.call("ate_enet_coef", apath.data_ptr(), pr.data_ptr(), nq, p, ny, L,
+                 nlam.data_ptr(), xm.data_ptr(), xs.data_ptr(), ju.data_ptr(), ym.data_ptr(),
+                 ys.data_ptr(), coef.data_ptr(), s)
+    _native.call("ate_enet_cvloss_gauss", G.data_ptr(), P, hold.data_ptr(), xc.data_ptr(), p, one,
+                 ycol_p.data_ptr(), coef.data_ptr(), nlam.data_ptr(), L, nf, nq - nf,
+                 cvraw.data_ptr(), s)
     _native.call("ate_cv_select", cvraw.data_ptr(), fidx.data_ptr(), nfold_t.data_ptr(), K, nf,
                  nlam.data_ptr(), L, cvm.data_ptr(), cvsd.data_ptr(), sel.data_ptr(),
                  fold_npass.data_ptr(), nq - nf, s)
-    cmin = torch.empty((nf, p + 1), **f64)
-    c1se = torch.empty((nf, p + 1), **f64)
     _native.call("ate_enet_pick", coef.data_ptr(), sel.data_ptr(), p, L, nf, cmin.data_ptr(),
                  c1se.data_ptr(), fold_npass.data_ptr(), nq - nf, s)
     return EnetCvResult(lams[:nf], nlam[:nf], cvm, cvsd, sel, coef[:nf], cmin, c1se, full_keys,
diff --git a/csrc/common.hpp b/csrc/common.hpp
--- a/csrc/common.hpp
+++ b/csrc/common.hpp
@@ -98,6 +98,13 @@
   __syncthreads();
 }
 
+template <bool AGENT>
+__device__ __forceinline__ void st_out(double* p, double v) {
+  if constexpr (AGENT) __hip_atomic_store(p, v, __ATOMIC_RELAXED, __HIP_MEMORY_SCOPE_AGENT);
+  else *p = v;
+}
+__device__ __forceinline__ void wait_stores() { asm volatile("s_waitcnt vmcnt(0)" ::: "memory"); }
+
 inline int grid_for(int64_t n, int block, int cap = 2048) {
   int64_t g = (n + block - 1) / block;
   if (g < 1) g = 1;
diff --git a/csrc/dml.hip b/csrc/dml.hip
--- a/csrc/dml.hip
+++ b/csrc/dml.hip
@@ -1,4 +1,5 @@
 #include "common.hpp"
+#include "dml_common.hpp"
 
 using namespace ate;
 
@@ -38,8 +39,8 @@
   return base;
 }
 
-template <typename T, int RPT>
-__global__ __launch_bounds__(256) void dml_resid_kernel(
+template <typename T, int RPT, bool AGENT = false>
+__device__ __forceinline__ void dml_resid_body(
     const T* __restrict__ X, int64_t ld, const int* __restrict__ xcols, int p,
     const Seg* __restrict__ segs, int nseg, const double* __restrict__ coef ,
     int y0, int y1, int w0, int w1, int vcol, double* __restrict__ partial) {
@@ -96,18 +97,23 @@
   if (threadIdx.x == 0) {
     double* out = partial + ((int64_t)blockIdx.y * gridDim.x + blockIdx.x) * 7;
 #pragma unroll
-    for (int q = 0; q < 7; ++q) out[q] = v[q];
-  }
+    for (int q = 0; q < 7; ++q) st_out<AGENT>(out + q, v[q]);
+  }
+}
+
+template <typename T, int RPT>
+__global__ __launch_bounds__(256) void dml_resid_kernel(
+    const T* __restrict__ X, int64_t ld, const int* __restrict__ xcols, int p,
+    const Seg* __restrict__ segs, int nseg, const double* __restrict__ coef ,
+    int y0, int y1, int w0, int w1, int vcol, double* __restrict__ partial) {
+  dml_resid_body<T, RPT>(X, ld, xcols, p, segs, nseg, coef, y0, y1, w0, w1, vcol, partial);
 }
 
 __global__ __launch_bounds__(256) void sum7_kernel(const double* __restrict__ partial, int nb,
                                                    double* __restrict__ out) {
   __shared__ double red[16 * 7];
   double v[7] = {0, 0, 0, 0, 0, 0, 0};
-  for (int b = threadIdx.x; b < nb; b += 256)
-#pragma unroll
-    for (int q = 0; q < 7; ++q) v[q] += partial[(int64_t)b * 7 + q];
-  block_sum<7>(v, red);
+  sum7_block(partial, nb, v, red);
   if (threadIdx.x == 0)
 #pragma unroll
     for (int q = 0; q < 7; ++q) out[q] = v[q];
@@ -129,7 +135,8 @@
   return 0;
 }
 
-__global__ __launch_bounds__(256) void dml_resid_bf16_kernel(
+template <bool AGENT = false>
+__device__ __forceinline__ void dml_resid_bf16_body(
     const bf16_t* __restrict__ X, int64_t cs, int64_t bs, const int* __restrict__ xcols, int p,
     const Seg* __restrict__ segs, int nseg, const double* __restrict__ coef,
     int y0, int y1, int w0, int w1, int vcol, double* __restrict__ partial, int mode,
@@ -216,7 +223,7 @@
     if (threadIdx.x == 0) {
       double* out = partial + blk * 7;
 #pragma unroll
-      for (int q = 0; q < 7; ++q) out[q] = v[q];
+      for (int q = 0; q < 7; ++q) st_out<AGENT>(out + q, v[q]);
     }
     return;
   }
@@ -255,6 +262,89 @@
       reinterpret_cast<long long*>(partial)[blk * 14 + q] = a;
     }
   }
+}
+
+__global__ __launch_bounds__(256) void dml_resid_bf16_kernel(
+    const bf16_t* __restrict__ X, int64_t cs, int64_t bs, const int* __restrict__ xcols, int p,
+    const Seg* __restrict__ segs, int nseg, const double* __restrict__ coef,
+    int y0, int y1, int w0, int w1, int vcol, double* __restrict__ partial, int mode,
+    const int64_t* __restrict__ sh) {
+  dml_resid_bf16_body(X, cs, bs, xcols, p, segs, nseg, coef, y0, y1, w0, w1, vcol, partial, mode,
+                      sh);
+}
+
+__device__ __forceinline__ void dml_resid_final_tail(const double* partial, int* done,
+                                                     double* __restrict__ mom,
+                                                     double* __restrict__ res) {
+  __shared__ double red[16 * 7];
+  __shared__ int slast;
+  const int nb = gridDim.x * gridDim.y;
+  if (threadIdx.x == 0) {
+    wait_stores();
+    const int old = __hip_atomic_fetch_add(done, 1, __ATOMIC_RELAXED, __HIP_MEMORY_SCOPE_AGENT);
+    ATE_DASSERT(old >= 0 && old < nb);
+    slast = old == nb - 1;
+  }
+  __syncthreads();
+  if (!slast) return;
+  __builtin_amdgcn_fence(__ATOMIC_ACQUIRE, "agent");
+  double v[7] = {0, 0, 0, 0, 0, 0, 0};
+  sum7_block(partial, nb, v, red);
+  if (threadIdx.x == 0) {
+#pragma unroll
+    for (int q = 0; q < 7; ++q) mom[q] = v[q];
+    dml_finalize_formula(v, 0, res);
+  }
+}
+
+template <typename T, int RPT>
+__global__ __launch_bounds__(256) void dml_resid_final_kernel(
+    const T* __restrict__ X, int64_t ld, const int* __restrict__ xcols, int p,
+    const Seg* __restrict__ segs, int nseg, const double* __restrict__ coef, int y0, int y1,
+    int w0, int w1, int vcol, double* partial, int* done, double* __restrict__ mom,
+    double* __restrict__ res) {
+  dml_resid_body<T, RPT, true>(X, ld, xcols, p, segs, nseg, coef, y0, y1, w0, w1, vcol, partial);
+  dml_resid_final_tail(partial, done, mom, res);
+}
+
+__global__ __launch_bounds__(256) void dml_resid_bf16_final_kernel(
+    const bf16_t* __restrict__ X, int64_t cs, int64_t bs, const int* __restrict__ xcols, int p,
+    const Seg* __restrict__ segs, int nseg, const double* __restrict__ coef, int y0, int y1,
+    int w0, int w1, int vcol, double* partial, int* done, double* __restrict__ mom,
+    double* __restrict__ res) {
+  dml_resid_bf16_body<true>(X, cs, bs, xcols, p, segs, nseg, coef, y0, y1, w0, w1, vcol, partial,
+                            0, nullptr);
+  dml_resid_final_tail(partial, done, mom, res);
+}
+
+ATE_API int ate_dml_resid_moments_final(int dtype, const void* X, int64_t cs, int64_t bs,
+                                        const void* xcols, int p, const void* segs, int nseg,
+                                        const void* coef, int y0, int y1, int w0, int w1,
+                                        int vcol, int nbx, void* partial, void* done,
+                                        void* moments, void* res, void* stream) {
+  hipStream_t s = (hipStream_t)stream;
+  if (dtype != 3 && bs != 64) return -1;
+  if (nbx < 1 || nseg < 1) return -1;
+  dim3 grid(nbx, nseg);
+  const size_t shd = (size_t)2 * (p + 1) * sizeof(double) + (size_t)p * sizeof(int);
+  if (dtype == 1) {
+    ATE_LAUNCH((dml_resid_final_kernel<float, 4>), grid, dim3(256), shd, s, (const float*)X, cs,
+               (const int*)xcols, p, (const Seg*)segs, nseg, (const double*)coef, y0, y1, w0, w1,
+               vcol, (double*)partial, (int*)done, (double*)moments, (double*)res);
+  } else if (dtype == 2) {
+    ATE_LAUNCH((dml_resid_final_kernel<double, 4>), grid, dim3(256), shd, s, (const double*)X, cs,
+               (const int*)xcols, p, (const Seg*)segs, nseg, (const double*)coef, y0, y1, w0, w1,
+               vcol, (double*)partial, (int*)done, (double*)moments, (double*)res);
+  } else if (dtype == 3) {
+    const size_t sh = (size_t)2 * (p + 1) * sizeof(float) + (size_t)p * sizeof(int);
+    ATE_LAUNCH(dml_resid_bf16_final_kernel, grid, dim3(256), sh, s, (const bf16_t*)X, cs, bs,
+               (const int*)xcols, p, (const Seg*)segs, nseg, (const double*)coef, y0, y1, w0, w1,
+               vcol, (double*)partial, (int*)done, (double*)moments, (double*)res);
+  } else {
+    return -1;
+  }
+  ATE_CHECK_LAUNCH();
+  return 0;
 }
 
 ATE_API int ate_dml_resid_moments(int dtype, const void* X, int64_t cs, int64_t bs,
diff --git a/csrc/dml_common.hpp b/csrc/dml_common.hpp
--- /dev/null
+++ b/csrc/dml_common.hpp
@@ -0,0 +1,30 @@
+#pragma once
+#include "common.hpp"
+
+namespace ate {
+
+__device__ __forceinline__ void dml_finalize_formula(const double* m, int mode, double* res) {
+  double n = m[5];
+  double theta = m[0] / m[1];
+  double se;
+  if (mode == 0) {
+    double j = m[1] / n;
+    double psi2 = (m[2] - 2.0 * theta * m[3] + theta * theta * m[4]) / n;
+    se = sqrt(fmax(psi2, 0.0) / (j * j) / n);
+  } else {
+    double rss = m[6] - 2.0 * theta * m[0] + theta * theta * m[1];
+    se = sqrt(fmax(rss, 0.0) / (n - 1.0) / m[1]);
+  }
+  res[0] = theta;
+  res[1] = se;
+}
+
+__device__ __forceinline__ void sum7_block(const double* partial, int nb, double (&v)[7],
+                                           double* red ) {
+  for (int b = threadIdx.x; b < nb; b += 256)
+#pragma unroll
+    for (int q = 0; q < 7; ++q) v[q] += partial[(int64_t)b * 7 + q];
+  block_sum<7>(v, red);
+}
+
+}
diff --git a/csrc/enet.hip b/csrc/enet.hip
--- a/csrc/enet.hip
+++ b/csrc/enet.hip
@@ -14,6 +14,16 @@
   for (int q = 0; q < nseg; ++q)
     if (mk[q]) acc += G[((int64_t)q * P + a) * P + b];
   return acc;
+}
+
+__device__ __forceinline__ void col_mean_var(double s1, double s2, double n, double& m,
+                                             double& v) {
+  m = s1 / n;
+  v = s2 / n - m * m;
+}
+__device__ __forceinline__ double std_entry(double sab, double n, double ma, double mb,
+                                            double sa, double sb) {
+  return (sab / n - ma * mb) / (sa * sb);
 }
 
 __global__ __launch_bounds__(256) void enet_prep_stats_kernel(
@@ -27,16 +37,18 @@
   const int e = blockIdx.x * blockDim.x + threadIdx.x;
   if (e < p) {
     const int j = e;
-    const double mj = seg_sum(G, nseg, P, mk, ones_col, xcols[j]) / n;
-    const double vj = seg_sum(G, nseg, P, mk, xcols[j], xcols[j]) / n - mj * mj;
+    double mj, vj;
+    col_mean_var(seg_sum(G, nseg, P, mk, ones_col, xcols[j]),
+                 seg_sum(G, nseg, P, mk, xcols[j], xcols[j]), n, mj, vj);
     xm[(int64_t)s * p + j] = mj;
     xs[(int64_t)s * p + j] = vj > 0 ? sqrt(vj) : 1.0;
     ju[(int64_t)s * p + j] = vj > 0 ? 1 : 0;
     if (j == 0) nobs[s] = n;
   } else if (e < p + ny) {
     const int y = e - p;
-    const double my = seg_sum(G, nseg, P, mk, ones_col, ycols[y]) / n;
-    const double vy = seg_sum(G, nseg, P, mk, ycols[y], ycols[y]) / n - my * my;
+    double my, vy;
+    col_mean_var(seg_sum(G, nseg, P, mk, ones_col, ycols[y]),
+                 seg_sum(G, nseg, P, mk, ycols[y], ycols[y]), n, my, vy);
     ym[(int64_t)s * ny + y] = my;
     ys[(int64_t)s * ny + y] = vy > 0 ? sqrt(vy) : 1.0;
   }
@@ -64,8 +76,8 @@
         cjk = (j == k) ? 1.0 : 0.0;
       } else {
         const double mj = xm[(int64_t)s * p + j], mk2 = xm[(int64_t)s * p + k];
-        cjk = (seg_sum(G, nseg, P, mk, xcols[j], xcols[k]) / n - mj * mk2) /
-              (xs[(int64_t)s * p + j] * xs[(int64_t)s * p + k]);
+        cjk = std_entry(seg_sum(G, nseg, P, mk, xcols[j], xcols[k]), n, mj, mk2,
+                        xs[(int64_t)s * p + j], xs[(int64_t)s * p + k]);
       }
       C[((int64_t)s * p + j) * ldc + k] = (CT)cjk;
     } else {
@@ -74,8 +86,8 @@
       double gj = 0.0;
       if (ju[(int64_t)s * p + j]) {
         const double mj = xm[(int64_t)s * p + j], my = ym[(int64_t)s * ny + y];
-        gj = (seg_sum(G, nseg, P, mk, xcols[j], ycols[y]) / n - mj * my) /
-             (xs[(int64_t)s * p + j] * ys[(int64_t)s * ny + y]);
+        gj = std_entry(seg_sum(G, nseg, P, mk, xcols[j], ycols[y]), n, mj, my,
+                       xs[(int64_t)s * p + j], ys[(int64_t)s * ny + y]);
       }
       g[((int64_t)s * ny + y) * p + j] = gj;
     }
@@ -107,6 +119,176 @@
                        (const int*)ycols, ny, (const double*)xm, (const double*)xs,
                        (const unsigned char*)ju, (const double*)ym, (const double*)ys,
                        (const double*)nobs, (double*)C, (double*)g);
+  ATE_CHECK_LAUNCH();
+  return 0;
+}
+
+constexpr int PF_TJ = 16, PF_TK = 64, PF_NC = PF_TJ + PF_TK, PF_SCH = 4, PF_SEG = 8;
+
+__device__ __forceinline__ double seg_sum_bits(const double* __restrict__ G, int nseg, int P,
+                                               unsigned bits, int a, int b) {
+  double v[PF_SEG];
+#pragma unroll
+  for (int q = 0; q < PF_SEG; ++q) v[q] = q < nseg ? G[((int64_t)q * P + a) * P + b] : 0.0;
+  double acc = 0.0;
+#pragma unroll
+  for (int q = 0; q < PF_SEG; ++q)
+    if (q < nseg && (bits >> q & 1u)) acc += v[q];
+  return acc;
+}
+
+template <typename CT>
+__global__ __launch_bounds__(256) void enet_prepare_fused_kernel(
+    const double* __restrict__ G, int nseg, int P, const unsigned char* __restrict__ masks,
+    int ntrain, const int* __restrict__ xcols, int p, int ldc, int ones_col,
+    const int* __restrict__ ycols, int ny, CT* __restrict__ C, double* __restrict__ g,
+    double* __restrict__ xm, double* __restrict__ xs, unsigned char* __restrict__ ju,
+    double* __restrict__ ym, double* __restrict__ ys, double* __restrict__ nobs,
+    double* __restrict__ lams, int64_t nlams) {
+  const int tk = blockIdx.x, tj = blockIdx.y, tid = threadIdx.x;
+  const int j0 = tj * PF_TJ, k0 = tk * PF_TK, s0 = blockIdx.z * PF_SCH;
+  const int lane = tid & 63, jr = tid >> 6;
+  ATE_DASSERT(k0 + PF_TK <= ldc && j0 < p && ones_col >= 0 && ones_col < P);
+  {
+    const int64_t nb = (int64_t)gridDim.x * gridDim.y * gridDim.z,
+                  b = ((int64_t)blockIdx.z * gridDim.y + tj) * gridDim.x + tk;
+    for (int64_t e = b * 256 + tid; e < nlams; e += nb * 256) lams[e] = __builtin_nan("");
+  }
+  __shared__ double s_n[PF_SCH], s_m[PF_SCH][PF_NC], s_s[PF_SCH][PF_NC];
+  __shared__ unsigned char s_ju[PF_SCH][PF_NC];
+  __shared__ unsigned s_mask[PF_SCH];
+  const bool inreg = nseg <= PF_SEG;
+  const int k = k0 + lane;
+  const int xk = k < p ? xcols[k] : 0;
+  ATE_DASSERT(xk >= 0 && xk < P);
+  double gv[4][PF_SEG];
+  int xj[4];
+#pragma unroll
+  for (int i = 0; i < 4; ++i) {
+    const int j = j0 + jr + 4 * i;
+    xj[i] = j < p ? xcols[j] : 0;
+    ATE_DASSERT(xj[i] >= 0 && xj[i] < P);
+#pragma unroll
+    for (int q = 0; q < PF_SEG; ++q)
+      gv[i][q] = (inreg && q < nseg && j < p && k < p)
+                     ? G[((int64_t)q * P + xj[i]) * P + xk] : 0.0;
+  }
+  auto set_sum = [&](int s, int sl, int a, int b) {
+    return inreg ? seg_sum_bits(G, nseg, P, s_mask[sl], a, b)
+                 : seg_sum(G, nseg, P, masks + (int64_t)s * nseg, a, b);
+  };
+  {
+    const int ns = ntrain - s0 < PF_SCH ? ntrain - s0 : PF_SCH;
+    ATE_DASSERT(ns >= 1);
+    if (tid < ns) {
+      const unsigned char* mk = masks + (int64_t)(s0 + tid) * nseg;
+      unsigned bits = 0;
+      if (inreg) {
+#pragma unroll
+        for (int q = 0; q < PF_SEG; ++q) bits |= (q < nseg && mk[q < nseg ? q : 0]) ? 1u << q : 0u;
+      }
+      s_mask[tid] = bits;
+      s_n[tid] = inreg ? seg_sum_bits(G, nseg, P, bits, ones_col, ones_col)
+                       : seg_sum(G, nseg, P, mk, ones_col, ones_col);
+    }
+    __syncthreads();
+    for (int e = tid; e < ns * PF_NC; e += 256) {
+      const int sl = e / PF_NC, c = e % PF_NC;
+      const int col = c < PF_TJ ? j0 + c : k0 + c - PF_TJ;
+      if (col >= p) continue;
+      const int s = s0 + sl;
+      const int xc = xcols[col];
+      ATE_DASSERT(xc >= 0 && xc < P);
+      double mj, vj;
+      col_mean_var(set_sum(s, sl, ones_col, xc), set_sum(s, sl, xc, xc), s_n[sl], mj, vj);
+      const double sd = vj > 0 ? sqrt(vj) : 1.0;
+      s_m[sl][c] = mj;
+      s_s[sl][c] = sd;
+      s_ju[sl][c] = vj > 0 ? 1 : 0;
+      if (tk == 0 && c < PF_TJ) {
+        xm[(int64_t)s * p + col] = mj;
+        xs[(int64_t)s * p + col] = sd;
+        ju[(int64_t)s * p + col] = vj > 0 ? 1 : 0;
+      }
+    }
+    if (tk == 0 && tj == 0) {
+      if (tid < ns) nobs[s0 + tid] = s_n[tid];
+      for (int e = tid; e < ns * ny; e += 256) {
+        const int sl = e / ny, y = e % ny, s = s0 + sl;
+        double my, vy;
+        col_mean_var(set_sum(s, sl, ones_col, ycols[y]), set_sum(s, sl, ycols[y], ycols[y]),
+                     s_n[sl], my, vy);
+        ym[(int64_t)s * ny + y] = my;
+        ys[(int64_t)s * ny + y] = vy > 0 ? sqrt(vy) : 1.0;
+      }
+    }
+    __syncthreads();
+#pragma unroll
+    for (int i = 0; i < 4; ++i) {
+      const int jl = jr + 4 * i, j = j0 + jl;
+      if (j >= p) continue;
+      for (int sl = 0; sl < ns; ++sl) {
+        const int s = s0 + sl;
+        double cjk = 0.0;
+        if (k < p) {
+          if (!s_ju[sl][jl] || !s_ju[sl][PF_TJ + lane]) {
+            cjk = (j == k) ? 1.0 : 0.0;
+          } else {
+            double acc = 0.0;
+            if (inreg) {
+              const unsigned bits = s_mask[sl];
+#pragma unroll
+              for (int q = 0; q < PF_SEG; ++q)
+                if (q < nseg && (bits >> q & 1u)) acc += gv[i][q];
+            } else {
+              acc = seg_sum(G, nseg, P, masks + (int64_t)s * nseg, xj[i], xk);
+            }
+            cjk = std_entry(acc, s_n[sl], s_m[sl][jl], s_m[sl][PF_TJ + lane], s_s[sl][jl],
+                            s_s[sl][PF_TJ + lane]);
+          }
+        }
+        C[((int64_t)s * p + j) * ldc + k] = (CT)cjk;
+      }
+    }
+    if (tk == 0) {
+      for (int e = tid; e < ns * ny * PF_TJ; e += 256) {
+        const int jl = e % PF_TJ, y = (e / PF_TJ) % ny, sl = e / (PF_TJ * ny);
+        const int j = j0 + jl, s = s0 + sl;
+        if (j >= p) continue;
+        double gj = 0.0;
+        if (s_ju[sl][jl]) {
+          const int yc = ycols[y];
+          ATE_DASSERT(yc >= 0 && yc < P);
+          double my, vy;
+          col_mean_var(set_sum(s, sl, ones_col, yc), set_sum(s, sl, yc, yc), s_n[sl], my, vy);
+          gj = std_entry(set_sum(s, sl, xcols[j], yc), s_n[sl], s_m[sl][jl], my, s_s[sl][jl],
+                         vy > 0 ? sqrt(vy) : 1.0);
+        }
+        g[((int64_t)s * ny + y) * p + j] = gj;
+      }
+    }
+  }
+}
+
+ATE_API int ate_enet_prepare_fused(const void* G, int nseg, int P, const void* masks, int ntrain,
+                                   const void* xcols, int p, int ones_col, const void* ycols,
+                                   int ny, void* C, int c_f32, void* g, void* xm, void* xs,
+                                   void* ju, void* ym, void* ys, void* nobs, void* lams,
+                                   int64_t nlams, void* stream) {
+  if (p < 1 || ntrain < 1 || nseg < 1 || ny < 0) return -1;
+  hipStream_t st = (hipStream_t)stream;
+  const int ldc = (p + 63) / 64 * 64;
+  dim3 grid(ldc / PF_TK, (p + PF_TJ - 1) / PF_TJ, (ntrain + PF_SCH - 1) / PF_SCH);
+  if (c_f32)
+    ATE_LAUNCH(enet_prepare_fused_kernel<float>, grid, dim3(256), 0, st, (const double*)G, nseg,
+               P, (const unsigned char*)masks, ntrain, (const int*)xcols, p, ldc, ones_col,
+               (const int*)ycols, ny, (float*)C, (double*)g, (double*)xm, (double*)xs,
+               (unsigned char*)ju, (double*)ym, (double*)ys, (double*)nobs, (double*)lams, nlams);
+  else
+    ATE_LAUNCH(enet_prepare_fused_kernel<double>, grid, dim3(256), 0, st, (const double*)G, nseg,
+               P, (const unsigned char*)masks, ntrain, (const int*)xcols, p, ldc, ones_col,
+               (const int*)ycols, ny, (double*)C, (double*)g, (double*)xm, (double*)xs,
+               (unsigned char*)ju, (double*)ym, (double*)ys, (double*)nobs, (double*)lams, nlams);
   ATE_CHECK_LAUNCH();
   return 0;
 }
@@ -1379,6 +1561,22 @@
   return 0;
 }
 
+template <class Store>
+__device__ __forceinline__ double coef_row_terms(const double* __restrict__ a, int64_t tb, int p,
+                                                 double ysq, const double* __restrict__ xm,
+                                                 const double* __restrict__ xs,
+                                                 const unsigned char* __restrict__ ju, int t0,
+                                                 int stride, Store st) {
+  double acc = 0.0;
+  for (int j = t0; j < p; j += stride) {
+    int64_t sj = tb + j;
+    double b = ju[sj] ? a[j] * ysq / xs[sj] : 0.0;
+    st(j, b);
+    acc += b * xm[sj];
+  }
+  return acc;
+}
+
 __global__ void enet_coef_kernel(const double* __restrict__ apath, const EnetProblem* __restrict__ probs,
                                  int nprob, int p, int ny, int L, const int* __restrict__ nlam_out,
                                  const double* __restrict__ xm, const double* __restrict__ xs,
@@ -1395,13 +1593,8 @@
   const double* a = apath + ((int64_t)q * L + m) * p;
   const double ysq = ys[(int64_t)pr.train * ny + pr.y], ymq = ym[(int64_t)pr.train * ny + pr.y];
   __shared__ double smem[16];
-  double acc[1] = {0.0};
-  for (int j = threadIdx.x; j < p; j += blockDim.x) {
-    int64_t sj = (int64_t)pr.train * p + j;
-    double b = ju[sj] ? a[j] * ysq / xs[sj] : 0.0;
-    out[1 + j] = b;
-    acc[0] += b * xm[sj];
-  }
+  double acc[1] = {coef_row_terms(a, (int64_t)pr.train * p, p, ysq, xm, xs, ju, threadIdx.x,
+                                  blockDim.x, [&](int j, double b) { out[1 + j] = b; })};
   block_sum<1>(acc, smem);
   if (threadIdx.x == 0) out[0] = ymq - acc[0];
 }
@@ -1420,6 +1613,101 @@
 
 constexpr int CVL = 8;
 constexpr int CVK = PMAX / 64;
+
+template <bool AGENT, class A0>
+__device__ __forceinline__ void cvloss_chunk(
+    const double* __restrict__ Gh, int P, const int* __restrict__ xcols, int p, int ones_col,
+    int yc, double (*sbeta)[PMAX], int* sxc, unsigned char* snz, double (*sred)[3 * CVL], int nl,
+    int m0, int L, double* __restrict__ cvq, A0 a0_of) {
+  const int tid = threadIdx.x, lane = tid & 63, wid = tid >> 6;
+  for (int j = tid; j < PMAX; j += 256) sxc[j] = j < p ? xcols[j] : xcols[0];
+  __syncthreads();
+  for (int j = tid; j < PMAX; j += 256) {
+    bool any = false;
+#pragma unroll
+    for (int m = 0; m < CVL; ++m) any |= sbeta[m][j] != 0.0;
+    snz[j] = any;
+  }
+  __syncthreads();
+  double bl[CVK][CVL];
+#pragma unroll
+  for (int k = 0; k < CVK; ++k)
+#pragma unroll
+    for (int m = 0; m < CVL; ++m) bl[k][m] = sbeta[m][k * 64 + lane];
+  int cl[CVK];
+#pragma unroll
+  for (int k = 0; k < CVK; ++k) cl[k] = sxc[k * 64 + lane];
+  double quad[CVL], lin[CVL], sx[CVL];
+#pragma unroll
+  for (int m = 0; m < CVL; ++m) { quad[m] = 0.0; lin[m] = 0.0; sx[m] = 0.0; }
+  if (wid == 0) {
+#pragma unroll
+    for (int k = 0; k < CVK; ++k) {
+      if (k * 64 + lane >= p) continue;
+      const double gy = Gh[(int64_t)cl[k] * P + yc], g1 = Gh[(int64_t)cl[k] * P + ones_col];
+#pragma unroll
+      for (int m = 0; m < CVL; ++m) {
+        lin[m] = fma(bl[k][m], gy, lin[m]);
+        sx[m] = fma(bl[k][m], g1, sx[m]);
+      }
+    }
+  }
+  auto next_row = [&](int a) {
+    while (a < p && !snz[a]) a += 4;
+    return a;
+  };
+  auto load_row = [&](int a, double* g) {
+    const double* Gr = Gh + (int64_t)sxc[a] * P;
+#pragma unroll
+    for (int k = 0; k < CVK; ++k) g[k] = (k * 64 + lane < p) ? Gr[cl[k]] : 0.0;
+  };
+  double gn[CVK];
+  int a = next_row(wid);
+  if (a < p) load_row(a, gn);
+  while (a < p) {
+    double g[CVK];
+#pragma unroll
+    for (int k = 0; k < CVK; ++k) g[k] = gn[k];
+    const int an = next_row(a + 4);
+    if (an < p) load_row(an, gn);
+#pragma unroll
+    for (int m = 0; m < CVL; ++m) {
+      double t = 0.0;
+#pragma unroll
+      for (int k = 0; k < CVK; ++k) t = fma(g[k], bl[k][m], t);
+      quad[m] = fma(sbeta[m][a], t, quad[m]);
+    }
+    a = an;
+  }
+#pragma unroll
+  for (int m = 0; m < CVL; ++m) {
+    quad[m] = wave_sum(quad[m]);
+    lin[m] = wave_sum(lin[m]);
+    sx[m] = wave_sum(sx[m]);
+  }
+  if (lane == 0)
+#pragma unroll
+    for (int m = 0; m < CVL; ++m) {
+      sred[wid][m] = quad[m];
+      sred[wid][CVL + m] = lin[m];
+      sred[wid][2 * CVL + m] = sx[m];
+    }
+  __syncthreads();
+  if (tid < CVL && m0 + tid < L) {
+    const int m = tid;
+    if (m0 + m >= nl) {
+      st_out<AGENT>(cvq + m0 + m, NAN);
+    } else {
+      const double qd = sred[0][m] + sred[1][m] + sred[2][m] + sred[3][m];
+      const double ln = sred[0][CVL + m], s1 = sred[0][2 * CVL + m];
+      const double a0 = a0_of(m);
+      const double n = Gh[(int64_t)ones_col * P + ones_col];
+      const double yy = Gh[(int64_t)yc * P + yc], sy = Gh[(int64_t)ones_col * P + yc];
+      const double sse = yy - 2.0 * a0 * sy - 2.0 * ln + n * a0 * a0 + 2.0 * a0 * s1 + qd;
+      st_out<AGENT>(cvq + m0 + m, sse / n);
+    }
+  }
+}
 
 __global__ __launch_bounds__(256) void enet_cvloss_gauss_kernel(
     const double* __restrict__ G, int P, const int* __restrict__ hold,
@@ -1444,93 +1732,9 @@
     const bool ok = j < p && m0 + m < nl;
     sbeta[m][j] = ok ? coef[((int64_t)q * L + m0 + m) * (p + 1) + 1 + j] : 0.0;
   }
-  for (int j = tid; j < PMAX; j += 256) sxc[j] = j < p ? xcols[j] : xcols[0];
-  __syncthreads();
-  for (int j = tid; j < PMAX; j += 256) {
-    bool any = false;
-#pragma unroll
-    for (int m = 0; m < CVL; ++m) any |= sbeta[m][j] != 0.0;
-    snz[j] = any;
-  }
-  __syncthreads();
-  double bl[CVK][CVL];
-#pragma unroll
-  for (int k = 0; k < CVK; ++k)
-#pragma unroll
-    for (int m = 0; m < CVL; ++m) bl[k][m] = sbeta[m][k * 64 + lane];
-  int cl[CVK];
-#pragma unroll
-  for (int k = 0; k < CVK; ++k) cl[k] = sxc[k * 64 + lane];
-  double quad[CVL], lin[CVL], sx[CVL];
-#pragma unroll
-  for (int m = 0; m < CVL; ++m) { quad[m] = 0.0; lin[m] = 0.0; sx[m] = 0.0; }
-  if (wid == 0) {
-#pragma unroll
-    for (int k = 0; k < CVK; ++k) {
-      if (k * 64 + lane >= p) continue;
-      const double gy = Gh[(int64_t)cl[k] * P + yc], g1 = Gh[(int64_t)cl[k] * P + ones_col];
-#pragma unroll
-      for (int m = 0; m < CVL; ++m) {
-        lin[m] = fma(bl[k][m], gy, lin[m]);
-        sx[m] = fma(bl[k][m], g1, sx[m]);
-      }
-    }
-  }
-  auto next_row = [&](int a) {
-    while (a < p && !snz[a]) a += 4;
-    return a;
-  };
-  auto load_row = [&](int a, double* g) {
-    const double* Gr = Gh + (int64_t)sxc[a] * P;
-#pragma unroll
-    for (int k = 0; k < CVK; ++k) g[k] = (k * 64 + lane < p) ? Gr[cl[k]] : 0.0;
-  };
-  double gn[CVK];
-  int a = next_row(wid);
-  if (a < p) load_row(a, gn);
-  while (a < p) {
-    double g[CVK];
-#pragma unroll
-    for (int k = 0; k < CVK; ++k) g[k] = gn[k];
-    const int an = next_row(a + 4);
-    if (an < p) load_row(an, gn);
-#pragma unroll
-    for (int m = 0; m < CVL; ++m) {
-      double t = 0.0;
-#pragma unroll
-      for (int k = 0; k < CVK; ++k) t = fma(g[k], bl[k][m], t);
-      quad[m] = fma(sbeta[m][a], t, quad[m]);
-    }
-    a = an;
-  }
-#pragma unroll
-  for (int m = 0; m < CVL; ++m) {
-    quad[m] = wave_sum(quad[m]);
-    lin[m] = wave_sum(lin[m]);
-    sx[m] = wave_sum(sx[m]);
-  }
-  if (lane == 0)
-#pragma unroll
-    for (int m = 0; m < CVL; ++m) {
-      sred[wid][m] = quad[m];
-      sred[wid][CVL + m] = lin[m];
-      sred[wid][2 * CVL + m] = sx[m];
-    }
-  __syncthreads();
-  if (tid < CVL && m0 + tid < L) {
-    const int m = tid;
-    if (m0 + m >= nl) {
-      cvraw[(int64_t)q * L + m0 + m] = NAN;
-    } else {
-      const double qd = sred[0][m] + sred[1][m] + sred[2][m] + sred[3][m];
-      const double ln = sred[0][CVL + m], s1 = sred[0][2 * CVL + m];
-      const double a0 = coef[((int64_t)q * L + m0 + m) * (p + 1)];
-      const double n = Gh[(int64_t)ones_col * P + ones_col];
-      const double yy = Gh[(int64_t)yc * P + yc], sy = Gh[(int64_t)ones_col * P + yc];
-      const double sse = yy - 2.0 * a0 * sy - 2.0 * ln + n * a0 * a0 + 2.0 * a0 * s1 + qd;
-      cvraw[(int64_t)q * L + m0 + m] = sse / n;
-    }
-  }
+  cvloss_chunk<false>(Gh, P, xcols, p, ones_col, yc, sbeta, sxc, snz, sred, nl, m0, L,
+                      cvraw + (int64_t)q * L,
+                      [&](int m) { return coef[((int64_t)q * L + m0 + m) * (p + 1)]; });
 }
 
 ATE_API int ate_enet_cvloss_gauss(const void* G, int P, const void* hold, const void* xcols, int p,
@@ -1554,6 +1758,81 @@
   return __syncthreads_or(bad) != 0;
 }
 
+__device__ __forceinline__ void cv_select_wave(
+    const double* __restrict__ cvraw, const int* __restrict__ fold_probs,
+    const double* __restrict__ nfold, int K, int f, const int* __restrict__ nlam_full, int L,
+    double* __restrict__ cvm, double* __restrict__ cvsd, int* __restrict__ sel, bool bad,
+    int lane, int& i_min, int& i_1se) {
+  i_min = 0;
+  i_1se = 0;
+  if (bad) {
+    for (int m = lane; m < L; m += 64) {
+      cvm[(int64_t)f * L + m] = NAN;
+      cvsd[(int64_t)f * L + m] = NAN;
+    }
+    if (lane == 0) { sel[2 * f] = 0; sel[2 * f + 1] = 0; }
+    return;
+  }
+  const int nl = nlam_full[f];
+  double wsum = 0.0;
+  for (int k = 0; k < K; ++k) wsum += nfold[f * K + k];
+  double mus[4], sds[4];
+  double best = INFINITY;
+  int imin = 0x7fffffff;
+#pragma unroll
+  for (int c = 0; c < 4; ++c) {
+    const int m = c * 64 + lane;
+    mus[c] = INFINITY;
+    sds[c] = 0.0;
+    if (m >= nl) {
+      if (m < L) {
+        cvm[(int64_t)f * L + m] = NAN;
+        cvsd[(int64_t)f * L + m] = NAN;
+      }
+      continue;
+    }
+    double mu = 0.0;
+    for (int k = 0; k < K; ++k) mu += nfold[f * K + k] * cvraw[(int64_t)fold_probs[f * K + k] * L + m];
+    mu /= wsum;
+    double var = 0.0;
+    for (int k = 0; k < K; ++k) {
+      double d = cvraw[(int64_t)fold_probs[f * K + k] * L + m] - mu;
+      var += nfold[f * K + k] * d * d;
+    }
+    const double sd = sqrt(var / wsum / (double)(K - 1));
+    cvm[(int64_t)f * L + m] = mu;
+    cvsd[(int64_t)f * L + m] = sd;
+    mus[c] = mu;
+    sds[c] = sd;
+    if (mu < best) { best = mu; imin = m; }
+  }
+#pragma unroll
+  for (int o = 32; o > 0; o >>= 1) {
+    const double ob = __shfl_xor(best, o, 64);
+    const int oi = __shfl_xor(imin, o, 64);
+    if (ob < best || (ob == best && oi < imin)) { best = ob; imin = oi; }
+  }
+  if (imin == 0x7fffffff) imin = 0;
+  const int oc = imin >> 6, ol = imin & 63;
+  double mine = 0.0;
+#pragma unroll
+  for (int c = 0; c < 4; ++c)
+    if (c == oc) mine = mus[c] + sds[c];
+  const double thr1 = __shfl(mine, ol, 64);
+  int i1 = imin;
+#pragma unroll
+  for (int c = 0; c < 4; ++c) {
+    const uint64_t b = __ballot(c * 64 + lane < nl && mus[c] <= thr1);
+    if (b) { i1 = c * 64 + __ffsll((unsigned long long)b) - 1; break; }
+  }
+  if (lane == 0) {
+    sel[2 * f] = imin;
+    sel[2 * f + 1] = i1;
+  }
+  i_min = imin;
+  i_1se = i1;
+}
+
 __global__ __launch_bounds__(64) void cv_select_kernel(
     const double* __restrict__ cvraw, const int* __restrict__ fold_probs,
     const double* __restrict__ nfold, int K, int nfull, const int* __restrict__ nlam_full, int L,
@@ -1562,70 +1841,9 @@
   const int f = blockIdx.x;
   const int lane = threadIdx.x;
   if (f >= nfull) return;
-  if (any_truncated(fnp, nfp)) {
-    for (int m = lane; m < L; m += 64) {
-      cvm[(int64_t)f * L + m] = NAN;
-      cvsd[(int64_t)f * L + m] = NAN;
-    }
-    if (lane == 0) { sel[2 * f] = 0; sel[2 * f + 1] = 0; }
-    return;
-  }
-  const int nl = nlam_full[f];
-  double wsum = 0.0;
-  for (int k = 0; k < K; ++k) wsum += nfold[f * K + k];
-  double mus[4], sds[4];
-  double best = INFINITY;
-  int imin = 0x7fffffff;
-#pragma unroll
-  for (int c = 0; c < 4; ++c) {
-    const int m = c * 64 + lane;
-    mus[c] = INFINITY;
-    sds[c] = 0.0;
-    if (m >= nl) {
-      if (m < L) {
-        cvm[(int64_t)f * L + m] = NAN;
-        cvsd[(int64_t)f * L + m] = NAN;
-      }
-      continue;
-    }
-    double mu = 0.0;
-    for (int k = 0; k < K; ++k) mu += nfold[f * K + k] * cvraw[(int64_t)fold_probs[f * K + k] * L + m];
-    mu /= wsum;
-    double var = 0.0;
-    for (int k = 0; k < K; ++k) {
-      double d = cvraw[(int64_t)fold_probs[f * K + k] * L + m] - mu;
-      var += nfold[f * K + k] * d * d;
-    }
-    const double sd = sqrt(var / wsum / (double)(K - 1));
-    cvm[(int64_t)f * L + m] = mu;
-    cvsd[(int64_t)f * L + m] = sd;
-    mus[c] = mu;
-    sds[c] = sd;
-    if (mu < best) { best = mu; imin = m; }
-  }
-#pragma unroll
-  for (int o = 32; o > 0; o >>= 1) {
-    const double ob = __shfl_xor(best, o, 64);
-    const int oi = __shfl_xor(imin, o, 64);
-    if (ob < best || (ob == best && oi < imin)) { best = ob; imin = oi; }
-  }
-  if (imin == 0x7fffffff) imin = 0;
-  const int oc = imin >> 6, ol = imin & 63;
-  double mine = 0.0;
-#pragma unroll
-  for (int c = 0; c < 4; ++c)
-    if (c == oc) mine = mus[c] + sds[c];
-  const double thr1 = __shfl(mine, ol, 64);
-  int i1 = imin;
-#pragma unroll
-  for (int c = 0; c < 4; ++c) {
-    const uint64_t b = __ballot(c * 64 + lane < nl && mus[c] <= thr1);
-    if (b) { i1 = c * 64 + __ffsll((unsigned long long)b) - 1; break; }
-  }
-  if (lane == 0) {
-    sel[2 * f] = imin;
-    sel[2 * f + 1] = i1;
-  }
+  int i0, i1;
+  cv_select_wave(cvraw, fold_probs, nfold, K, f, nlam_full, L, cvm, cvsd, sel,
+                 any_truncated(fnp, nfp), lane, i0, i1);
 }
 
 ATE_API int ate_cv_select(const void* cvraw, const void* fold_probs, const void* nfold, int K,
@@ -1661,3 +1879,133 @@
   ATE_CHECK_LAUNCH();
   return 0;
 }
+
+__global__ __launch_bounds__(256) void enet_cv_tail_kernel(
+    const double* __restrict__ G, int P, const int* __restrict__ hold,
+    const int* __restrict__ xcols, int p, int ones_col, const int* __restrict__ ycol_of_prob,
+    const double* __restrict__ apath, const EnetProblem* __restrict__ probs, int ny,
+    const int* __restrict__ nlam_out, const double* __restrict__ xm,
+    const double* __restrict__ xs, const unsigned char* __restrict__ ju,
+    const double* __restrict__ ym, const double* __restrict__ ys, int L, int nf, int nfp, int K,
+    const int* __restrict__ fold_probs, const double* __restrict__ nfold, double* coef,
+    double* cvraw, double* cvm, double* cvsd, int* sel, double* out_min, double* out_1se,
+    const int* __restrict__ fnp, int* done) {
+  const int tid = threadIdx.x, lane = tid & 63, wid = tid >> 6;
+  const int nch = (L + CVL - 1) / CVL, ncv = nfp * nch;
+  const int b = blockIdx.x;
+  __shared__ double sbeta[CVL][PMAX];
+  __shared__ int sxc[PMAX];
+  __shared__ unsigned char snz[PMAX];
+  __shared__ double sred[4][3 * CVL];
+  __shared__ double sw[CVL][2], sa0[CVL];
+  __shared__ int slast, ssel[2];
+  int f;
+  if (b < ncv) {
+    const int q = nf + b % nfp, m0 = (nch - 1 - b / nfp) * CVL;
+    const EnetProblem pr = probs[q];
+    f = pr.ulam_src;
+    ATE_DASSERT(f >= 0 && f < nf && pr.train >= 0 && pr.y >= 0 && pr.y < ny);
+    const int nl = nlam_out[q];
+    if (m0 >= nl) {
+      if (tid < CVL && m0 + tid < L) st_out<true>(cvraw + (int64_t)q * L + m0 + tid, NAN);
+    } else {
+      const double* Gh = G + (int64_t)hold[q] * P * P;
+      const int yc = ycol_of_prob[q];
+      const double ysq = ys[(int64_t)pr.train * ny + pr.y], ymq = ym[(int64_t)pr.train * ny + pr.y];
+      for (int e = tid; e < CVL * PMAX; e += 256) (&sbeta[0][0])[e] = 0.0;
+      __syncthreads();
+      const int half = tid >> 7, t = tid & 127;
+#pragma unroll
+      for (int r = 0; r < CVL / 2; ++r) {
+        const int m = 2 * r + half;
+        double acc = 0.0;
+        if (m0 + m < nl)
+          acc = coef_row_terms(apath + ((int64_t)q * L + m0 + m) * p, (int64_t)pr.train * p, p,
+                               ysq, xm, xs, ju, t, 128,
+                               [&](int j, double bj) { sbeta[m][j] = bj; });
+        acc = wave_sum(acc);
+        if (lane == 0) sw[m][wid & 1] = acc;
+      }
+      __syncthreads();
+      if (tid < CVL) {
+        double s = 0.0;
+        for (int w = 0; w < 2; ++w) s += sw[tid][w];
+        sa0[tid] = ymq - s;
+      }
+      cvloss_chunk<true>(Gh, P, xcols, p, ones_col, yc, sbeta, sxc, snz, sred, nl, m0, L,
+                         cvraw + (int64_t)q * L, [&](int m) { return sa0[m]; });
+    }
+  } else {
+    f = (b - ncv) / L;
+    const int m = (b - ncv) % L;
+    ATE_DASSERT(f < nf);
+    const EnetProblem pr = probs[f];
+    double* out = coef + ((int64_t)f * L + m) * (p + 1);
+    if (m >= nlam_out[f]) {
+      for (int j = tid; j <= p; j += 256) st_out<true>(out + j, NAN);
+    } else {
+      const double ysq = ys[(int64_t)pr.train * ny + pr.y], ymq = ym[(int64_t)pr.train * ny + pr.y];
+      double acc = 0.0;
+      if (tid < 128)
+        acc = coef_row_terms(apath + ((int64_t)f * L + m) * p, (int64_t)pr.train * p, p, ysq, xm,
+                             xs, ju, tid, 128,
+                             [&](int j, double bj) { st_out<true>(out + 1 + j, bj); });
+      acc = wave_sum(acc);
+      if (lane == 0 && wid < 2) sw[0][wid] = acc;
+      __syncthreads();
+      if (tid == 0) {
+        double s = 0.0;
+        for (int w = 0; w < 2; ++w) s += sw[0][w];
+        st_out<true>(out, ymq - s);
+      }
+    }
+  }
+  wait_stores();
+  __syncthreads();
+  if (tid == 0) {
+    const int total = L + K * nch;
+    const int old = __hip_atomic_fetch_add(done + f, 1, __ATOMIC_RELAXED, __HIP_MEMORY_SCOPE_AGENT);
+    ATE_DASSERT(old >= 0 && old < total);
+    slast = old == total - 1;
+  }
+  __syncthreads();
+  if (!slast) return;
+  __builtin_amdgcn_fence(__ATOMIC_ACQUIRE, "agent");
+  const bool bad = any_truncated(fnp, nfp);
+  if (wid == 0) {
+    int i0, i1;
+    cv_select_wave(cvraw, fold_probs, nfold, K, f, nlam_out, L, cvm, cvsd, sel, bad, lane, i0, i1);
+    if (lane == 0) { ssel[0] = i0; ssel[1] = i1; }
+  }
+  __syncthreads();
+  for (int which = 0; which < 2; ++which) {
+    double* out = which ? out_1se : out_min;
+    const int m = ssel[which];
+    ATE_DASSERT(m >= 0 && m < L);
+    for (int j = tid; j <= p; j += 256)
+      out[(int64_t)f * (p + 1) + j] = bad ? NAN : coef[((int64_t)f * L + m) * (p + 1) + j];
+  }
+}
+
+ATE_API int ate_enet_cv_tail(const void* G, int P, const void* hold, const void* xcols, int p,
+                             int ones_col, const void* ycol_of_prob, const void* apath,
+                             const void* probs, int ny, const void* nlam_out, const void* xm,
+                             const void* xs, const void* ju, const void* ym, const void* ys, int L,
+                             int nf, int nfp, int K, const void* fold_probs, const void* nfold,
+                             void* coef, void* cvraw, void* cvm, void* cvsd, void* sel,
+                             void* out_min, void* out_1se, const void* fold_npass, void* done,
+                             void* stream) {
+  if (p > PMAX || p < 1 || L > 256 || L < 1) return -1;
+  if (nf < 1 || K < 1 || nfp != nf * K) return -1;
+  const int nch = (L + CVL - 1) / CVL;
+  ATE_LAUNCH(enet_cv_tail_kernel, dim3(nfp * nch + nf * L), dim3(256), 0, (hipStream_t)stream,
+             (const double*)G, P, (const int*)hold, (const int*)xcols, p, ones_col,
+             (const int*)ycol_of_prob, (const double*)apath, (const EnetProblem*)probs, ny,
+             (const int*)nlam_out, (const double*)xm, (const double*)xs,
+             (const unsigned char*)ju, (const double*)ym, (const double*)ys, L, nf, nfp, K,
+             (const int*)fold_probs, (const double*)nfold, (double*)coef, (double*)cvraw,
+             (double*)cvm, (double*)cvsd, (int*)sel, (double*)out_min, (double*)out_1se,
+             (const int*)fold_npass, (int*)done);
+  ATE_CHECK_LAUNCH();
+  return 0;
+}
diff --git a/csrc/stats.hip b/csrc/stats.hip
--- a/csrc/stats.hip
+++ b/csrc/stats.hip
@@ -1,4 +1,5 @@
 #include "common.hpp"
+#include "dml_common.hpp"
 
 using namespace ate;
 
@@ -178,19 +179,7 @@
 };
 
 __global__ void dml_finalize_kernel(const double* __restrict__ m, int mode, double* __restrict__ res) {
-  double n = m[5];
-  double theta = m[0] / m[1];
-  double se;
-  if (mode == 0) {
-    double j = m[1] / n;
-    double psi2 = (m[2] - 2.0 * theta * m[3] + theta * theta * m[4]) / n;
-    se = sqrt(fmax(psi2, 0.0) / (j * j) / n);
-  } else {
-    double rss = m[6] - 2.0 * theta * m[0] + theta * theta * m[1];
-    se = sqrt(fmax(rss, 0.0) / (n - 1.0) / m[1]);
-  }
-  res[0] = theta;
-  res[1] = se;
+  dml_finalize_formula(m, mode, res);
 }
 
 ATE_API int ate_dml_moments(const void* yr, const void* wr, const void* valid, int64_t n,
```

Result: faster. 2.301 billion rows/s, median of 6 (+1.5%).
